# pcodec/pcodec

Measured on AMD Instinct MI355X. Metric: encode+decode GB/s (uncompressed) per chunk, u64/f64 2^18-elem, higher is better.
Workload: dtype u64

## Files before the change

### include/pco_gfx.h

```cpp
#ifndef PCO_GFX_H
#define PCO_GFX_H

#include <stddef.h>
#include <stdint.h>

#if defined(__cplusplus)
extern "C" {
#endif


#define PCO_TYPE_U32 1
#define PCO_TYPE_U64 2
#define PCO_TYPE_I32 3
#define PCO_TYPE_I64 4
#define PCO_TYPE_F32 5
#define PCO_TYPE_F64 6
#define PCO_TYPE_U16 7
#define PCO_TYPE_I16 8
#define PCO_TYPE_F16 9
#define PCO_TYPE_U8 10
#define PCO_TYPE_I8 11

typedef enum PcoError {
  PcoSuccess,
  PcoInvalidType,
  PcoCompressionError,
  PcoDecompressionError,
} PcoError;

typedef struct PcoChunkConfig {
  unsigned int compression_level;
  size_t max_page_n;
} PcoChunkConfig;

size_t pco_standalone_guarantee_file_size(size_t n, unsigned char dtype);

enum PcoError pco_standalone_simple_compress_into(const void* nums, size_t n, unsigned char dtype,
                                                  const struct PcoChunkConfig* config, void* dst,
                                                  size_t dst_cap, size_t* n_written);

enum PcoError pco_standalone_simple_decompress_into(const void* compressed, size_t compressed_len,
                                                    unsigned char dtype, void* dst, size_t dst_cap,
                                                    size_t* n_written);


enum PcoModeSpecKind {
  PCO_MODE_AUTO = 0,
  PCO_MODE_CLASSIC = 1,
  PCO_MODE_TRY_FLOAT_MULT = 2,
  PCO_MODE_TRY_FLOAT_QUANT = 3,
  PCO_MODE_TRY_INT_MULT = 4,
  PCO_MODE_TRY_DICT = 5,
};
enum PcoDeltaSpecKind {
  PCO_DELTA_AUTO = 0,
  PCO_DELTA_NOOP = 1,
  PCO_DELTA_TRY_CONSECUTIVE = 2,
  PCO_DELTA_TRY_LOOKBACK = 3,
  PCO_DELTA_TRY_CONV1 = 4,
};
typedef struct PcoChunkConfigEx {
  uint32_t compression_level;
  uint32_t mode_kind;
  double mode_f64;
  uint64_t mode_u64;
  uint32_t delta_kind;
  uint32_t delta_order;
  uint64_t max_page_n;
  uint32_t enable_8_bit;
  uint32_t flags;
} PcoChunkConfigEx;
#define PCO_GFX_CFG_STRICT_HISTOGRAM 1u
#define PCO_GFX_CFG_CONV1 2u
#define PCO_GFX_CFG_DICT 4u

enum PcoGfxStatus {
  PCO_GFX_OK = 0,
  PCO_GFX_CORRUPTION = 1,
  PCO_GFX_INSUFFICIENT_DATA = 2,
  PCO_GFX_INVALID_ARGUMENT = 3,
  PCO_GFX_UNSUPPORTED = 4,
  PCO_GFX_DEVICE_ERROR = 5,
};
int pco_gfx_last_status(void);
const char* pco_gfx_last_error(void);
int pco_gfx_device_count(void);

enum PcoError pco_gfx_simple_compress_into_ex(const void* nums, size_t n, unsigned char dtype,
                                              const PcoChunkConfigEx* config, int uniform_type,
                                              void* dst, size_t dst_cap, size_t* n_written);
enum PcoError pco_gfx_simple_compress_into_exact(const void* nums, size_t n, unsigned char dtype, const PcoChunkConfigEx* config,
                                                 int uniform_type, const size_t* page_sizes, size_t n_pages, void* dst,
                                                 size_t dst_cap, size_t* n_written);
size_t pco_gfx_guarantee_file_size(size_t n, unsigned char dtype, uint64_t max_page_n);
size_t pco_gfx_guarantee_chunk_size(size_t n, unsigned char dtype);


typedef struct PcoGfxEncodeTask {
  const void* src;
  uint64_t n;
  void* dst;
  uint64_t dst_cap;
  uint32_t dtype;
  uint32_t reserved;
} PcoGfxEncodeTask;

typedef struct PcoGfxDecodeTask {
  const void* src;
  uint64_t src_len;
  void* dst;
  uint64_t dst_cap;
  uint32_t dtype;
  uint32_t flags;
} PcoGfxDecodeTask;
#define PCO_GFX_TASK_HAS_FILE_HEADER 1u
#define PCO_GFX_TASK_WRAPPED_PAGE 2u
#define PCO_GFX_TASK_META_ONLY 4u
#define PCO_GFX_TASK_ONE_CHUNK 8u

typedef struct PcoGfxTaskResult {
  uint64_t n_out;
  uint64_t consumed;
  uint32_t status;
  uint32_t aux;
} PcoGfxTaskResult;

enum PcoError pco_gfx_compress_chunks(size_t n_tasks, const PcoGfxEncodeTask* tasks,
                                      const PcoChunkConfigEx* config, PcoGfxTaskResult* results,
                                      PcoGfxTaskResult* d_results, void* stream);
enum PcoError pco_gfx_decompress_chunks(size_t n_tasks, const PcoGfxDecodeTask* tasks,
                                        PcoGfxTaskResult* results, PcoGfxTaskResult* d_results,
                                        void* stream);

enum PcoError pco_gfx_compact_chunks(size_t n_tasks, const PcoGfxEncodeTask* tasks, const PcoGfxTaskResult* d_results, void* d_dst,
                                     uint64_t dst_cap, uint64_t dst_offset, uint64_t* d_offsets, uint64_t* total, void* stream);

size_t pco_gfx_write_standalone_header(void* dst, size_t dst_cap, uint64_t n_hint, unsigned char uniform_dtype);
size_t pco_gfx_write_standalone_footer(void* dst, size_t dst_cap);

void pco_gfx_release_workspace(void);
size_t pco_gfx_workspace_bytes(void);
unsigned long long pco_gfx_strict_histogram_fallbacks(void);
unsigned long long pco_gfx_trail_givebacks(void);
unsigned long long pco_gfx_trail_marked(void);

void pco_gfx_profile_begin(void);
int pco_gfx_profile_end(char* names, size_t names_cap, float* ms, int cap);

typedef struct PcoGfxChunkCompressor PcoGfxChunkCompressor;
typedef struct PcoGfxChunkDecompressor PcoGfxChunkDecompressor;

size_t pco_wrapped_write_header(void* dst, size_t dst_cap);
enum PcoError pco_wrapped_read_header(const void* src, size_t len, size_t* consumed,
                                      uint8_t* major, uint8_t* minor);
enum PcoError pco_chunk_compressor_new(const void* nums, size_t n, unsigned char dtype,
                                       const PcoChunkConfigEx* config,
                                       PcoGfxChunkCompressor** out);
enum PcoError pco_chunk_compressor_new_exact(const void* nums, size_t n, unsigned char dtype, const PcoChunkConfigEx* config,
                                             const size_t* page_sizes, size_t n_pages, PcoGfxChunkCompressor** out);
size_t pco_chunk_compressor_n_pages(const PcoGfxChunkCompressor*);
size_t pco_chunk_compressor_meta_size(const PcoGfxChunkCompressor*);
size_t pco_chunk_compressor_page_size(const PcoGfxChunkCompressor*, size_t page_idx);
size_t pco_chunk_compressor_page_n(const PcoGfxChunkCompressor*, size_t page_idx);
size_t pco_chunk_compressor_meta_size_hint(const PcoGfxChunkCompressor*);
size_t pco_chunk_compressor_page_size_hint(const PcoGfxChunkCompressor*, size_t page_idx);
enum PcoError pco_chunk_compressor_write_meta(const PcoGfxChunkCompressor*, void* dst, size_t dst_cap, size_t* n_written);
enum PcoError pco_chunk_compressor_write_page(const PcoGfxChunkCompressor*, size_t page_idx, void* dst, size_t dst_cap, size_t* n_written);
void pco_chunk_compressor_free(PcoGfxChunkCompressor*);

enum PcoError pco_chunk_decompressor_new(const void* src, size_t len, unsigned char dtype,
                                         uint8_t format_major, PcoGfxChunkDecompressor** out,
                                         size_t* consumed);
enum PcoError pco_chunk_decompressor_read_page(PcoGfxChunkDecompressor*, const void* src, size_t len,
                                               size_t page_n, void* dst, size_t dst_cap,
                                               size_t* n_processed, size_t* consumed);
void pco_chunk_decompressor_free(PcoGfxChunkDecompressor*);

typedef struct PcoGfxPageDecompressor PcoGfxPageDecompressor;
enum PcoError pco_page_decompressor_new(PcoGfxChunkDecompressor*, const void* src, size_t len, size_t page_n, PcoGfxPageDecompressor** out);
enum PcoError pco_page_decompressor_read(PcoGfxPageDecompressor*, void* dst, size_t dst_len, size_t* n_processed, int* finished);
size_t pco_page_decompressor_consumed(const PcoGfxPageDecompressor*);
void pco_page_decompressor_free(PcoGfxPageDecompressor*);

typedef struct PcoGfxPageInfo {
  uint64_t offset;
  uint64_t len;
  uint64_t n;
  uint32_t status;
  uint32_t aux;
} PcoGfxPageInfo;
size_t pco_gfx_wrapped_n_pages(size_t n, uint64_t max_page_n);
size_t pco_gfx_wrapped_chunk_cap(size_t n, unsigned char dtype, const PcoChunkConfigEx* config);
enum PcoError pco_gfx_compress_wrapped_chunks(size_t n_tasks, const PcoGfxEncodeTask* tasks, const PcoChunkConfigEx* config,
                                              PcoGfxPageInfo* infos, void* stream);

typedef struct PcoGfxWrappedTask {
  const void* src;
  uint64_t n;
  void* dst;
  uint64_t dst_cap;
  uint32_t dtype;
  uint32_t n_pages;
  const uint64_t* page_sizes;
} PcoGfxWrappedTask;
size_t pco_gfx_wrapped_chunk_cap_exact(const uint64_t* page_sizes, size_t n_pages, unsigned char dtype, const PcoChunkConfigEx* config);
enum PcoError pco_gfx_compress_wrapped_chunks_ex(size_t n_tasks, const PcoGfxWrappedTask* tasks, const PcoChunkConfigEx* config,
                                                 PcoGfxPageInfo* infos, PcoGfxPageInfo* d_infos, void* stream);
size_t pco_gfx_wrapped_scratch_estimate(size_t n_tasks, const PcoGfxWrappedTask* tasks, const PcoChunkConfigEx* config);
enum PcoError pco_gfx_compact_wrapped_chunks(size_t n_tasks, const PcoGfxWrappedTask* tasks, const PcoChunkConfigEx* config,
                                             const PcoGfxPageInfo* d_infos, uint32_t gap, void* d_dst, uint64_t dst_cap, uint64_t dst_offset,
                                             uint64_t* d_offsets, uint64_t* total, void* stream);

typedef struct PcoGfxPageTask {
  const void* meta;
  uint64_t meta_len;
  const void* page;
  uint64_t page_len;
  void* dst;
  uint64_t page_n;
  uint32_t dtype;
  uint32_t format_major;
} PcoGfxPageTask;
enum PcoError pco_gfx_decompress_pages(size_t n_tasks, const PcoGfxPageTask* tasks, PcoGfxTaskResult* results,
                                       PcoGfxTaskResult* d_results, void* stream);

typedef struct PcoGfxPageRangeTask {
  const void* meta;
  uint64_t meta_len;
  const void* page;
  uint64_t page_len;
  void* dst;
  uint64_t page_n;
  uint64_t first, count;
  uint32_t dtype;
  uint32_t format_major;
} PcoGfxPageRangeTask;
enum PcoError pco_gfx_decompress_page_ranges(size_t n_tasks, const PcoGfxPageRangeTask* tasks, PcoGfxTaskResult* results,
                                             PcoGfxTaskResult* d_results, void* stream);

typedef struct PcoGfxChunkMetaInfo {
  uint32_t mode_kind;
  uint32_t mode_k;
  uint64_t mode_base_latent;
  uint32_t delta_kind;
  uint32_t delta_order;
  uint32_t window_n_log, state_n_log;
  uint32_t secondary_uses_delta;
  uint32_t n_vars_parsed;
  uint32_t present[3], ans_size_log[3], n_bins[3];
  uint64_t meta_bytes;
} PcoGfxChunkMetaInfo;
enum PcoError pco_gfx_chunk_meta_info(const void* meta, size_t len, unsigned char dtype, uint8_t format_major, PcoGfxChunkMetaInfo* out);
enum PcoError pco_chunk_compressor_meta_info(const PcoGfxChunkCompressor*, unsigned char dtype, PcoGfxChunkMetaInfo* out);
enum PcoError pco_chunk_decompressor_meta_info(const PcoGfxChunkDecompressor*, PcoGfxChunkMetaInfo* out);
enum PcoError pco_gfx_chunk_meta_conv1(const void* meta, size_t len, unsigned char dtype, uint8_t format_major, uint32_t* quantization,
                                       int64_t* bias, int32_t* weights, uint32_t* order);
enum PcoError pco_gfx_chunk_meta_dict(const void* meta, size_t len, unsigned char dtype, uint8_t format_major, uint32_t* n_unique, void* values,
                                      size_t cap);

typedef struct PcoGfxComm PcoGfxComm;
enum PcoError pco_gfx_comm_unique_id(void* id128);
enum PcoError pco_gfx_comm_init(const void* id128, int n_ranks, int rank, PcoGfxComm** out);
void pco_gfx_comm_free(PcoGfxComm*);
int pco_gfx_comm_rank(const PcoGfxComm*);
int pco_gfx_comm_size(const PcoGfxComm*);
enum PcoError pco_gfx_gather_chunks(PcoGfxComm*, int root, const void* d_stream, uint64_t n_bytes, void* d_file, uint64_t file_cap,
                                    uint64_t file_offset, uint64_t* offsets, void* stream);
enum PcoError pco_gfx_scatter_chunks(PcoGfxComm*, int root, const void* d_file, uint64_t file_offset, const uint64_t* offsets,
                                     void* d_stream, uint64_t stream_cap, uint64_t* n_bytes, void* stream);

int pco_gfx_debug_float_screen(const void* values, size_t n, uint32_t dtype, uint32_t* out);
int64_t pco_gfx_debug_lookback_routes(uint8_t* out, size_t cap);

#if defined(__cplusplus)
}
#endif
#endif
```

### pcodec_amd/_lib.py

```python
import ctypes as C
import os

HERE = os.path.dirname(os.path.abspath(__file__))
LIB_PATH = os.environ.get("PCO_GFX_LIB", os.path.join(HERE, "libpco_gfx.so"))

PcoSuccess, PcoInvalidType, PcoCompressionError, PcoDecompressionError = range(4)
ST_OK, ST_CORRUPTION, ST_INSUFFICIENT_DATA, ST_INVALID_ARGUMENT, ST_UNSUPPORTED, ST_DEVICE_ERROR = range(6)
TASK_HAS_FILE_HEADER = 1

MODE_AUTO, MODE_CLASSIC, MODE_TRY_FLOAT_MULT, MODE_TRY_FLOAT_QUANT, MODE_TRY_INT_MULT, MODE_TRY_DICT = range(6)
DELTA_AUTO, DELTA_NOOP, DELTA_TRY_CONSECUTIVE, DELTA_TRY_LOOKBACK, DELTA_TRY_CONV1 = range(5)

CFG_STRICT_HISTOGRAM = 1
CFG_CONV1 = 2
CFG_DICT = 4

DTYPE_BYTE = {"uint32": 1, "uint64": 2, "int32": 3, "int64": 4, "float32": 5, "float64": 6,
              "uint16": 7, "int16": 8, "float16": 9, "uint8": 10, "int8": 11}
DTYPE_BYTES = {1: 4, 2: 8, 3: 4, 4: 8, 5: 4, 6: 8, 7: 2, 8: 2, 9: 2, 10: 1, 11: 1}


class PcoChunkConfig(C.Structure):
    _fields_ = [("compression_level", C.c_uint), ("max_page_n", C.c_size_t)]


class PcoChunkConfigEx(C.Structure):
    _fields_ = [("compression_level", C.c_uint32), ("mode_kind", C.c_uint32), ("mode_f64", C.c_double),
                ("mode_u64", C.c_uint64), ("delta_kind", C.c_uint32), ("delta_order", C.c_uint32),
                ("max_page_n", C.c_uint64), ("enable_8_bit", C.c_uint32), ("flags", C.c_uint32)]


class EncodeTask(C.Structure):
    _fields_ = [("src", C.c_void_p), ("n", C.c_uint64), ("dst", C.c_void_p), ("dst_cap", C.c_uint64),
                ("dtype", C.c_uint32), ("reserved", C.c_uint32)]


class DecodeTask(C.Structure):
    _fields_ = [("src", C.c_void_p), ("src_len", C.c_uint64), ("dst", C.c_void_p), ("dst_cap", C.c_uint64),
                ("dtype", C.c_uint32), ("flags", C.c_uint32)]


class TaskResult(C.Structure):
    _fields_ = [("n_out", C.c_uint64), ("consumed", C.c_uint64), ("status", C.c_uint32), ("aux", C.c_uint32)]


KIND_NAMES = {ST_CORRUPTION: "Corruption", ST_INSUFFICIENT_DATA: "InsufficientData", ST_INVALID_ARGUMENT: "InvalidArgument",
              ST_UNSUPPORTED: "Unsupported", ST_DEVICE_ERROR: "DeviceError"}


class PageInfo(C.Structure):
    _fields_ = [("offset", C.c_uint64), ("len", C.c_uint64), ("n", C.c_uint64), ("status", C.c_uint32), ("aux", C.c_uint32)]


class PageTask(C.Structure):
    _fields_ = [("meta", C.c_void_p), ("meta_len", C.c_uint64), ("page", C.c_void_p), ("page_len", C.c_uint64),
                ("dst", C.c_void_p), ("page_n", C.c_uint64), ("dtype", C.c_uint32), ("format_major", C.c_uint32)]


class PageRangeTask(C.Structure):
    _fields_ = [("meta", C.c_void_p), ("meta_len", C.c_uint64), ("page", C.c_void_p), ("page_len", C.c_uint64),
                ("dst", C.c_void_p), ("page_n", C.c_uint64), ("first", C.c_uint64), ("count", C.c_uint64),
                ("dtype", C.c_uint32), ("format_major", C.c_uint32)]


class WrappedTask(C.Structure):
    _fields_ = [("src", C.c_void_p), ("n", C.c_uint64), ("dst", C.c_void_p), ("dst_cap", C.c_uint64),
                ("dtype", C.c_uint32), ("n_pages", C.c_uint32), ("page_sizes", C.c_void_p)]


class PcoGfxError(RuntimeError):

    def __init__(self, code, status, msg):
        super().__init__(f"pco error: pco {KIND_NAMES.get(status, status)} error: {msg} (libpco_gfx code={code} status={status})")
        self.code, self.status = code, status


_lib = None


def lib():
    global _lib
    if _lib is None:
        if not os.path.exists(LIB_PATH):
            raise ImportError(f"{LIB_PATH} is missing: build it with `python -m pcodec_amd.build` (needs hipcc). "
                              "pcodec_amd has no CPU fallback.")
        try:
            import torch
        except Exception:
            pass
        L = C.CDLL(LIB_PATH)
        L.pco_gfx_last_error.restype = C.c_char_p
        L.pco_standalone_guarantee_file_size.restype = C.c_size_t
        L.pco_standalone_guarantee_file_size.argtypes = [C.c_size_t, C.c_ubyte]
        L.pco_gfx_guarantee_file_size.restype = C.c_size_t
        L.pco_gfx_guarantee_file_size.argtypes = [C.c_size_t, C.c_ubyte, C.c_uint64]
        L.pco_gfx_guarantee_chunk_size.restype = C.c_size_t
        L.pco_gfx_workspace_bytes.restype = C.c_size_t
        L.pco_gfx_workspace_bytes.argtypes = []
        L.pco_gfx_strict_histogram_fallbacks.restype = C.c_ulonglong
        L.pco_gfx_strict_histogram_fallbacks.argtypes = []
        L.pco_gfx_debug_lookback_routes.restype = C.c_int64
        L.pco_gfx_debug_lookback_routes.argtypes = [C.c_void_p, C.c_size_t]
        L.pco_gfx_trail_givebacks.restype = C.c_ulonglong
        L.pco_gfx_trail_givebacks.argtypes = []
        L.pco_gfx_trail_marked.restype = C.c_ulonglong
        L.pco_gfx_trail_marked.argtypes = []
        L.pco_gfx_guarantee_chunk_size.argtypes = [C.c_size_t, C.c_ubyte]
        L.pco_standalone_simple_compress_into.argtypes = [C.c_void_p, C.c_size_t, C.c_ubyte, C.c_void_p, C.c_void_p,
                                                          C.c_size_t, C.POINTER(C.c_size_t)]
        L.pco_standalone_simple_decompress_into.argtypes = [C.c_void_p, C.c_size_t, C.c_ubyte, C.c_void_p, C.c_size_t,
                                                            C.POINTER(C.c_size_t)]
        L.pco_gfx_simple_compress_into_ex.argtypes = [C.c_void_p, C.c_size_t, C.c_ubyte, C.c_void_p, C.c_int,
                                                      C.c_void_p, C.c_size_t, C.POINTER(C.c_size_t)]
        L.pco_gfx_compress_chunks.argtypes = [C.c_size_t, C.c_void_p, C.c_void_p, C.c_void_p, C.c_void_p, C.c_void_p]
        L.pco_gfx_decompress_chunks.argtypes = [C.c_size_t, C.c_void_p, C.c_void_p, C.c_void_p, C.c_void_p]
        L.pco_gfx_write_standalone_header.restype = C.c_size_t
        L.pco_gfx_write_standalone_header.argtypes = [C.c_void_p, C.c_size_t, C.c_uint64, C.c_ubyte]
        L.pco_gfx_write_standalone_footer.restype = C.c_size_t
        L.pco_gfx_write_standalone_footer.argtypes = [C.c_void_p, C.c_size_t]
        L.pco_wrapped_write_header.restype = C.c_size_t
        L.pco_wrapped_write_header.argtypes = [C.c_void_p, C.c_size_t]
        L.pco_gfx_wrapped_n_pages.restype = C.c_size_t
        L.pco_gfx_wrapped_n_pages.argtypes = [C.c_size_t, C.c_uint64]
        L.pco_gfx_wrapped_chunk_cap.restype = C.c_size_t
        L.pco_gfx_wrapped_chunk_cap.argtypes = [C.c_size_t, C.c_ubyte, C.c_void_p]
        L.pco_gfx_compress_wrapped_chunks.argtypes = [C.c_size_t, C.c_void_p, C.c_void_p, C.c_void_p, C.c_void_p]
        L.pco_gfx_decompress_pages.argtypes = [C.c_size_t, C.c_void_p, C.c_void_p, C.c_void_p, C.c_void_p]
        L.pco_gfx_decompress_page_ranges.argtypes = [C.c_size_t, C.c_void_p, C.c_void_p, C.c_void_p, C.c_void_p]
        L.pco_gfx_wrapped_chunk_cap_exact.restype = C.c_size_t
        L.pco_gfx_wrapped_chunk_cap_exact.argtypes = [C.c_void_p, C.c_size_t, C.c_ubyte, C.c_void_p]
        L.pco_gfx_compress_wrapped_chunks_ex.argtypes = [C.c_size_t, C.c_void_p, C.c_void_p, C.c_void_p, C.c_void_p, C.c_void_p]
        L.pco_gfx_wrapped_scratch_estimate.restype = C.c_size_t
        L.pco_gfx_wrapped_scratch_estimate.argtypes = [C.c_size_t, C.c_void_p, C.c_void_p]
        L.pco_gfx_compact_wrapped_chunks.argtypes = [C.c_size_t, C.c_void_p, C.c_void_p, C.c_void_p, C.c_uint32, C.c_void_p, C.c_uint64, C.c_uint64,
                                                     C.c_void_p, C.c_void_p, C.c_void_p]
        _lib = L
    return _lib


def check(code):
    if code != PcoSuccess:
        L = lib()
        raise PcoGfxError(code, L.pco_gfx_last_status(), (L.pco_gfx_last_error() or b"").decode())


def make_config(level=8, mode=MODE_AUTO, mode_f64=0.0, mode_u64=0, delta=DELTA_AUTO, delta_order=0, max_page_n=0,
                enable_8_bit=False, strict_histogram=False, conv1=False, dict=False):
    return PcoChunkConfigEx(level, mode, mode_f64, mode_u64, delta, delta_order, max_page_n, 1 if enable_8_bit else 0,
                            (CFG_STRICT_HISTOGRAM if strict_histogram else 0) | (CFG_CONV1 if conv1 else 0) | (CFG_DICT if dict else 0))


def chunk_meta_conv1(meta, dtype_byte, format_major=4):
    buf = (C.c_uint8 * max(len(meta), 1)).from_buffer_copy(bytes(meta) or b"\0")
    q, b, order, w = C.c_uint32(), C.c_int64(), C.c_uint32(), (C.c_int32 * 32)()
    rc = lib().pco_gfx_chunk_meta_conv1(buf, C.c_size_t(len(meta)), C.c_ubyte(dtype_byte), C.c_uint8(format_major), C.byref(q), C.byref(b), w,
                                        C.byref(order))
    if rc != 0:
        raise PcoGfxError(rc, lib().pco_gfx_last_status(), lib().pco_gfx_last_error().decode())
    return None if order.value == 0 else (q.value, b.value, list(w[:order.value]))


def chunk_meta_dict(meta, dtype_byte, format_major=4):
    import numpy as np
    buf = (C.c_uint8 * max(len(meta), 1)).from_buffer_copy(bytes(meta) or b"\0")
    width = {1: 4, 2: 8, 3: 4, 4: 8, 5: 4, 6: 8, 7: 2, 8: 2, 9: 2, 10: 1, 11: 1}[dtype_byte]
    cap = max(len(meta) // width, 1)
    out = np.zeros(cap, dtype={1: np.uint8, 2: np.uint16, 4: np.uint32, 8: np.uint64}[width])
    k = C.c_uint32()
    rc = lib().pco_gfx_chunk_meta_dict(buf, C.c_size_t(len(meta)), C.c_ubyte(dtype_byte), C.c_uint8(format_major), C.byref(k),
                                       out.ctypes.data_as(C.c_void_p), C.c_size_t(cap))
    if rc != 0:
        raise PcoGfxError(rc, lib().pco_gfx_last_status(), lib().pco_gfx_last_error().decode())
    return None if k.value == 0 else out[:k.value].copy()
```

### pcodec_amd/csrc/decode_fast.hip

```cpp
#include "decode_kernel.hip"

namespace pcogfx {

constexpr uint32_t kGrpWinOff = 0;
constexpr uint32_t kGrpVarOff = 448;
constexpr uint32_t kGrpTblOff = 640;
template <uint32_t KQ> struct WalkCfg {
  static constexpr uint32_t kGrpBytes = KQ == 8 ? 4912u : 9904u;
  static constexpr uint32_t kGrpTblBytes = kGrpBytes - kGrpTblOff;
  static constexpr uint32_t kWalkTmpOff = KQ * kGrpBytes;
  static constexpr uint32_t kWalkTmpObOff = kWalkTmpOff + 1056;
  static constexpr uint32_t kWalkLdsBytes = kWalkTmpObOff + 256;
  static constexpr uint32_t kRetryStatus = KQ == 8 ? 101u : 100u;
  static_assert(kGrpBytes % 16 == 0, "chunk slices must stay 16-byte aligned");
  static_assert(kWalkLdsBytes < 65536, "walk entries hold 16-bit LDS addresses");
};
template <uint32_t KQ> __device__ __forceinline__ uint8_t PCO_LDS* walk_lds() { return lds_base() + uni((uint32_t)(threadIdx.x >> 6)) * WalkCfg<KQ>::kWalkLdsBytes; }
__device__ __forceinline__ uint32_t walk_block_id() { return blockIdx.x * (blockDim.x >> 6) + uni((uint32_t)(threadIdx.x >> 6)); }
constexpr uint32_t kTrailDead = 0xffffffffu;
constexpr uint32_t kTrailDoneWord = 8;
constexpr uint32_t kTrailProgressStride = 32;
constexpr bool kTrailDefer = true;
constexpr uint32_t kTrailMaxBins = 64;
constexpr uint32_t kFastMaxBins = 256;
// ... 63 lines not shown
  if (n_bins == 0) { if (lane == 0) entries[0] = make_wentry(0, 0, 0, 0); wave_sync_lds(); return true; }
  if (carry != T) { status = PCO_GFX_CORRUPTION; return false; }
  wave_sync_lds();
  uint32_t stride = (3 * T) / 5; if ((stride & 1) == 0) stride += 1;
  for (uint32_t t = lane; t < T; t += 64) {
    uint32_t lo = 0, hi = n_bins;
    while (hi - lo > 1) { const uint32_t mid = (lo + hi) >> 1; if (cum[mid] <= t) lo = mid; else hi = mid; }
    entries[(stride * t) & (T - 1)] = lo;
  }
  wave_sync_lds();
  for (uint32_t b0 = 0; b0 < n_bins; b0 += 64) {
    const uint32_t b = b0 + lane;
    uint32_t w = 0;
    if (b < n_bins) w = cum[b + 1] - cum[b];
    wave_sync_lds();
    if (b < n_bins) cum[b] = w;
    wave_sync_lds();
  }
  const uint32_t sym_bits = 32 - clz_u32(n_bins - 1 > 0 ? n_bins - 1 : 1);
  for (uint32_t i0 = 0; i0 < T; i0 += 64) {
    const uint32_t i = i0 + lane;
    const bool act = i < T;
    const uint32_t s = act ? entries[i] : 0xffffffffu;
    uint64_t m = __ballot(act);
    for (uint32_t bit = 0; bit < sym_bits; bit++) { const uint64_t bm = __ballot((s >> bit) & 1); m &= ((s >> bit) & 1) ? bm : ~bm; }
    const uint64_t lt = ((uint64_t)1 << lane) - 1;
    const uint32_t rank = __popcll(m & lt), gcount = __popcll(m);
    const uint32_t basec = act ? cum[s] : 0;
    wave_sync_lds();
    if (act && rank == 0) cum[s] = basec + gcount;
    wave_sync_lds();
    if (act) { const uint32_t x_s = basec + rank; const uint32_t btr = clz_u32(x_s) - clz_u32(T); entries[i] = make_wentry((x_s << btr) - T, s, btr, obs[s]); }
  }
  wave_sync_lds();
  return true;
}

template <class LV, uint32_t KQ>
__device__ __noinline__ bool fast_build_var(uint32_t q, uint32_t vi, MetaReader& mr, uint8_t PCO_GLOBAL* bins_out, uint32_t& status) { return fast_build_var_impl<LV, KQ>(q, vi, mr, bins_out, status); }

struct FrontOut {
  uint32_t status, n, mode_kind;
  uint64_t bitpos;
  uint32_t states[3][4];
  uint64_t moments[2][2];
};

template <class L, uint32_t KQ, bool kInline, bool kRange = false>
__device__ __forceinline__ void fast_front_impl(const PcoGfxDecodeTask& task, uint32_t q, DecPlan PCO_GLOBAL* plan, uint8_t PCO_GLOBAL* bins_out, FrontOut& out,
                                                gcptr_u8 meta_p, uint64_t meta_len) {
  constexpr uint32_t kGrpBytes = WalkCfg<KQ>::kGrpBytes, kGrpTblBytes = WalkCfg<KQ>::kGrpTblBytes;
  const uint32_t lane = lane_id();
  gcptr_u8 src = (gcptr_u8)task.src;
  const uint64_t src_len = uni((uint64_t)task.src_len);
  const uint32_t dtype = uni(task.dtype), flags = uni(task.flags);
  const uint64_t dst_cap = uni((uint64_t)task.dst_cap);
  constexpr uint32_t LB = LBits<L>::v;
  const bool wrapped = (flags & PCO_GFX_TASK_WRAPPED_PAGE) != 0;
  MetaReader mr{src, src_len, 0};
  if (wrapped && meta_p != nullptr) mr = MetaReader{meta_p, meta_len, 0};
  uint32_t status = PCO_GFX_OK, format_major = 4, uniform_type = 0;
  out.status = PCO_GFX_OK; out.n = 0; out.bitpos = 0;
  for (int v = 0; v < 3; v++) for (int j = 0; j < 4; j++) out.states[v][j] = 0;
  out.mode_kind = kClassic;
  VarInfo PCO_LDS* vinfo = (VarInfo PCO_LDS*)(walk_lds<KQ>() + q * kGrpBytes + kGrpVarOff);
  auto fail = [&](uint32_t s) { if (wrapped && s != kStatusRetryK4) s = kStatusRetryLegacy; out.status = s; if (lane == 0) { plan->status = s; plan->consumed = mr.bit >> 3; plan->n = 0; plan->fused = 0; plan->more = 0; } };
  out.moments[0][0] = out.moments[0][1] = out.moments[1][0] = out.moments[1][1] = 0;
  if (dtype_bits(dtype) != (int)LB) { fail(PCO_GFX_INVALID_ARGUMENT); return; }
  if (flags & PCO_GFX_TASK_META_ONLY) { fail(kStatusRetryLegacy); return; }
  uint32_t n = 0;
  if (wrapped) {
    format_major = (flags >> 8) & 0xffu;
    if (dst_cap == 0 || dst_cap > kMaxEntries || format_major > 4) { fail(kStatusRetryLegacy); return; }
    n = (uint32_t)dst_cap;
  } else
  if (flags & PCO_GFX_TASK_HAS_FILE_HEADER) {
    const uint32_t magic = (uint32_t)mr.read(32);
    if (!mr.in_bounds()) status = PCO_GFX_INSUFFICIENT_DATA; else if (magic != 0x216f6370u) status = PCO_GFX_CORRUPTION;
    if (!status) {
      const uint32_t sv = (uint32_t)mr.read(8);
      if (sv < 2) mr.bit -= 8;
      else {
        if (sv >= 3) { const uint32_t ub = (uint32_t)mr.read(8); if (ub != 0) { if (dtype_bits(ub) == 0) status = PCO_GFX_CORRUPTION; uniform_type = ub; } }
        if (!status) { const uint32_t power = 1 + (uint32_t)mr.read(kBitsVarintPower); mr.read(power); if (!mr.drain_empty_byte() && mr.in_bounds()) status = PCO_GFX_CORRUPTION; }
      }
      if (!status && !mr.in_bounds()) status = PCO_GFX_INSUFFICIENT_DATA;
      if (!status && sv > 3) status = PCO_GFX_CORRUPTION;
      if (!status) {
        format_major = (uint32_t)mr.read(8);
        if (format_major >= 4) mr.read(8);
        if (format_major > 4) status = PCO_GFX_CORRUPTION; else if (!mr.in_bounds()) status = PCO_GFX_INSUFFICIENT_DATA;
      }
    }
    if (status) { fail(status); return; }
  } else if (src_len == 0) { fail(kStatusRetryLegacy); return; }
  else if ((flags & PCO_GFX_TASK_ONE_CHUNK) && ((flags >> 8) & 0xffu) != 0) format_major = (flags >> 8) & 0xffu;
  if (!wrapped) {
    const uint32_t tb = (uint32_t)mr.read(8);
    if (!mr.in_bounds()) { fail(PCO_GFX_INSUFFICIENT_DATA); return; }
    if (tb == 0) { fail(kStatusRetryLegacy); return; }
    if ((uniform_type && uniform_type != tb) || tb != dtype) { fail(PCO_GFX_CORRUPTION); return; }
    n = (uint32_t)mr.read(kBitsNEntries) + 1;
    if (!mr.in_bounds()) { fail(PCO_GFX_INSUFFICIENT_DATA); return; }
    if (n > dst_cap) { fail(PCO_GFX_INVALID_ARGUMENT); return; }
  }
  const uint32_t num_kind = dtype_kind(dtype);
  const uint32_t mode_kind = (uint32_t)mr.read(kBitsModeVariant);
  L mode_base = 0; uint32_t mode_k = 0;
  if (mode_kind == kIntMult) { if (format_major == 0) { fail(PCO_GFX_CORRUPTION); return; } mode_base = (L)mr.read(LB); }
  else if (mode_kind == kFloatMult) mode_base = (L)mr.read(LB);
  else if (mode_kind == kFloatQuant) mode_k = (uint32_t)mr.read(kBitsQuantK);
  else if (mode_kind == kDict) { fail(mr.in_bounds() ? kStatusRetryLegacy : PCO_GFX_INSUFFICIENT_DATA); return; }
  else if (mode_kind != kClassic) { fail(mr.in_bounds() ? PCO_GFX_CORRUPTION : PCO_GFX_INSUFFICIENT_DATA); return; }
  if (!mr.in_bounds()) { fail(PCO_GFX_INSUFFICIENT_DATA); return; }
  uint32_t dkind = kDeltaNone, dorder = 0, wlog = 0, slog = 0; bool sec_uses_delta = false;
  if (format_major < 3) { dorder = (uint32_t)mr.read(kBitsDeltaOrder); if (dorder) dkind = kDeltaConsecutive; }
  else {
    const uint32_t variant = (uint32_t)mr.read(kBitsDeltaVariant);
    if (variant == 1) { dorder = (uint32_t)mr.read(kBitsDeltaOrder); if (dorder == 0) { fail(PCO_GFX_CORRUPTION); return; } dkind = kDeltaConsecutive; sec_uses_delta = mr.read(1) != 0; }
    else if (variant == 2) {
      wlog = 1 + (uint32_t)mr.read(kBitsLookbackWindowLog); slog = (uint32_t)mr.read(kBitsLookbackStateLog);
      if (wlog > kMaxLookbackWindowLog || slog > wlog) { fail(PCO_GFX_CORRUPTION); return; }
      dkind = kDeltaLookback; sec_uses_delta = mr.read(1) != 0;
    } else if (variant == 3) { fail(mr.in_bounds() ? kStatusRetryLegacy : PCO_GFX_INSUFFICIENT_DATA); return; }
    else if (variant != 0) { fail(PCO_GFX_CORRUPTION); return; }
  }
  if (!mr.in_bounds()) { fail(PCO_GFX_INSUFFICIENT_DATA); return; }
  const uint32_t present[3] = {dkind == kDeltaLookback ? 1u : 0u, 1u, (mode_kind == kIntMult || mode_kind == kFloatMult || mode_kind == kFloatQuant) ? 1u : 0u};
  uint32_t total_tbl = 0; bool too_big = false;
  {
    MetaReader peek = mr;
#pragma unroll
    for (int vi = 0; vi < 3; vi++) {
      VarInfo v{};
      v.present = present[vi]; v.latent_bits = vi == 0 ? 32u : LB;
      if (vi == 1 || (vi == 2 && sec_uses_delta)) { v.delta_kind = dkind; v.delta_order = dorder; v.window_n_log = wlog; v.state_n_log = slog; }
      if (present[vi]) {
        const uint32_t a = (uint32_t)peek.read(kBitsAnsSizeLog), nb = (uint32_t)peek.read(kBitsNBins);
        if (!peek.in_bounds()) { fail(PCO_GFX_INSUFFICIENT_DATA); return; }
        if ((1u << a) < nb || (nb == 1 && a > 0) || a > kMaxAnsBits) { fail(PCO_GFX_CORRUPTION); return; }
        v.ans_size_log = a; v.n_bins = nb;
        v.off_nodes = total_tbl; v.off_lower = 0; v.off_ob = total_tbl + (4u << a);
        total_tbl += (4u << a) + 8u;
        if (nb > kFastMaxBins || a > 12) too_big = true;
        peek.bit += (uint64_t)nb * (a + v.latent_bits + offset_bits_bits(v.latent_bits));
      }
      if (lane == 0) { uint32_t PCO_LDS* p = (uint32_t PCO_LDS*)(vinfo + vi); const uint32_t* qq = (const uint32_t*)&v; for (int w = 0; w < 16; w++) p[w] = qq[w]; }
    }
  }
  wave_sync_lds();
  if (too_big || total_tbl > WalkCfg<4>::kGrpTblBytes) { fail(kStatusRetryLegacy); return; }
  if (total_tbl > kGrpTblBytes) { fail(WalkCfg<KQ>::kRetryStatus); return; }
  if (dkind == kDeltaLookback && (mode_kind != kClassic || sec_uses_delta)) { fail(kStatusRetryLegacy); return; }
  if constexpr (kRange) { if (dkind == kDeltaLookback) { fail(kStatusRetryLegacy); return; } }
#pragma unroll
  for (int vi = 0; vi < 3; vi++) {
    if (!present[vi]) continue;
    mr.bit += kBitsAnsSizeLog + kBitsNBins;
    bool ok;
    if constexpr (kInline) ok = vi == 0 ? fast_build_var_impl<uint32_t, KQ>(q, vi, mr, bins_out, status) : fast_build_var_impl<L, KQ>(q, vi, mr, bins_out, status);
    else ok = vi == 0 ? fast_build_var<uint32_t, KQ>(q, vi, mr, bins_out, status) : fast_build_var<L, KQ>(q, vi, mr, bins_out, status);
    if (!ok) { fail(status); return; }
  }
  if (!mr.drain_empty_byte()) { if (mr.in_bounds()) { fail(PCO_GFX_CORRUPTION); return; } }
  if (!mr.in_bounds()) { fail(PCO_GFX_INSUFFICIENT_DATA); return; }
  if (wrapped && meta_p != nullptr) mr = MetaReader{src, src_len, 0};
  if (dkind == kDeltaLookback) {
    const uint32_t nb0 = uni(vinfo[0].n_bins);
    const uint64_t PCO_GLOBAL* lw = (const uint64_t PCO_GLOBAL*)bins_out;
    uint32_t bad = 0;
    __builtin_amdgcn_fence(__ATOMIC_ACQ_REL, "workgroup");
    for (uint32_t b = lane; b < nb0; b += 64) { const uint64_t x = __hip_atomic_load(&lw[b], __ATOMIC_RELAXED, __HIP_MEMORY_SCOPE_AGENT); if (x < 1 || x > (1ull << wlog)) bad = 1; }
    if (uni(wave_or_u32(bad))) { fail(PCO_GFX_CORRUPTION); return; }
  }
  {
    bool valid = true;
    if (mode_kind == kIntMult) valid = num_kind != kFloat && mode_base > 0;
    else if (mode_kind == kFloatQuant) { const uint32_t prec = LB == 64 ? 52 : (LB == 32 ? 23 : 10); valid = num_kind == kFloat && mode_k > 0 && mode_k <= prec; }
    else if (mode_kind == kFloatMult) {
      if (num_kind != kFloat) valid = false;
      else if constexpr (sizeof(L) >= 4) { typedef typename FloatOf<L>::F F; const F b = bits_to_float(from_latent_ordered<L>(mode_base, kFloat)); valid = isfinite(b) && b != (F)0; }
      else if constexpr (sizeof(L) == 2) { const uint32_t hb = (uint32_t)from_latent_ordered<L>(mode_base, kFloat); valid = (hb & 0x7c00u) != 0x7c00u && (hb & 0x7fffu) != 0; }
      else valid = false;
    }
    if (!valid) { fail(PCO_GFX_CORRUPTION); return; }
  }
  uint32_t nlps[3];
#pragma unroll
  for (int vi = 0; vi < 3; vi++) {
    const uint32_t dk = uni(vinfo[vi].delta_kind);
    nlps[vi] = dk == kDeltaConsecutive ? uni(vinfo[vi].delta_order) : (dk == kDeltaLookback ? (1u << uni(vinfo[vi].state_n_log)) : 0u);
  }
  L PCO_GLOBAL* dst = (L PCO_GLOBAL*)task.dst;
#pragma unroll
  for (int vi = 0; vi < 3; vi++) {
    if (!present[vi]) continue;
    const uint32_t lbits = vi == 0 ? 32u : LB;
    const uint32_t dk = uni(vinfo[vi].delta_kind);
    for (uint32_t i = 0; i < nlps[vi]; i++) {
      const L x = (L)mr.read(lbits);
      if (dk == kDeltaConsecutive) { if (lane == 0 && i < 8) plan->moments[vi == 2 ? 1 : 0][i] = (uint64_t)x; if (i < 2) out.moments[vi == 2 ? 1 : 0][i] = (uint64_t)x; }
      else if (vi == 1 && i < n && mr.in_bounds()) { if (lane == 0) dst[i] = from_latent_ordered<L>(x, num_kind); }
    }
    const uint32_t asl = uni(vinfo[vi].ans_size_log);
    for (uint32_t j = 0; j < 4; j++) out.states[vi][j] = (uint32_t)mr.read(asl);
  }
  if (!mr.drain_empty_byte()) { if (mr.in_bounds()) { fail(PCO_GFX_CORRUPTION); return; } }
  if (!mr.in_bounds()) { fail(PCO_GFX_INSUFFICIENT_DATA); return; }
  const uint32_t n_in_body = n > nlps[1] ? n - nlps[1] : 0;
  if (n_in_body > 0) for (int vi = 0; vi < 3; vi++) if (present[vi] && uni(vinfo[vi].n_bins) == 0) { fail(PCO_GFX_CORRUPTION); return; }
  out.mode_kind = mode_kind;
  if (lane == 0) {
    plan->status = PCO_GFX_OK; plan->n = n; plan->mode_kind = mode_kind; plan->mode_k = mode_k; plan->mode_base = (uint64_t)mode_base;
    plan->num_kind = num_kind; plan->dtype = dtype; plan->window_n_log = wlog; plan->state_n_log = slog; plan->consumed = 0; plan->fused = 0; plan->more = 0;
    for (int vi = 0; vi < 3; vi++) {
      plan->present[vi] = present[vi]; plan->n_bins[vi] = vinfo[vi].n_bins; plan->max_ob[vi] = vinfo[vi].max_ob;
      plan->delta_kind[vi] = vinfo[vi].delta_kind; plan->delta_order[vi] = vinfo[vi].delta_order; plan->nlps[vi] = nlps[vi];
    }
  }
  out.n = n; out.bitpos = mr.bit;
}

template <class L, uint32_t KQ>
__device__ __noinline__ void fast_front(const PcoGfxDecodeTask& task, uint32_t q, DecPlan PCO_GLOBAL* plan, uint8_t PCO_GLOBAL* bins_out, FrontOut& out, gcptr_u8 meta_p, uint64_t meta_len) { fast_front_impl<L, KQ, false>(task, q, plan, bins_out, out, meta_p, meta_len); }
template <class L, uint32_t KQ>
__device__ __noinline__ void fast_front_range(const PcoGfxDecodeTask& task, uint32_t q, DecPlan PCO_GLOBAL* plan, uint8_t PCO_GLOBAL* bins_out, FrontOut& out, gcptr_u8 meta_p, uint64_t meta_len) { fast_front_impl<L, KQ, false, true>(task, q, plan, bins_out, out, meta_p, meta_len); }

struct WalkRegs {
  uint32_t saddr;
  uint32_t e;
  uint32_t bitaddr;
  uint32_t d0, d1, d2;
  uint32_t obsum, symacc;
};

__device__ __forceinline__ void walk_window(WalkRegs& r, uint32_t tot) {
  r.bitaddr += tot;
  const uint32_t PCO_LDS* w = (const uint32_t PCO_LDS*)(uintptr_t)((r.bitaddr >> 3) & ~3u);
  r.d0 = w[0]; r.d1 = w[1]; r.d2 = w[2];
}

template <bool kAgent>
__device__ __forceinline__ void store_syms(uint8_t PCO_GLOBAL* p, uint32_t __attribute__((ext_vector_type(4))) acc) {
  typedef uint32_t u32x4 __attribute__((ext_vector_type(4)));
  if constexpr (kAgent) {
    __asm__ volatile("global_store_dwordx4 %0, %1, off sc1" : : "v"(p), "v"(acc) : "memory");
  } else *(u32x4 PCO_GLOBAL*)p = acc;
}

struct QuadMasks { uint32_t m1, m2, m3, c63; };

template <int K, bool kTail>
__device__ __forceinline__ void walk_step(WalkRegs& r, const QuadMasks& m, uint32_t tbl_addr, bool chain_on) {
  uint32_t e = r.e;
  if (kTail) e = chain_on ? e : 0u;
  const uint32_t p = ((uint32_t)__builtin_amdgcn_update_dpp(0, (int)e, 0x111, 0xf, 0xf, true) & m.m1) +
                     ((uint32_t)__builtin_amdgcn_update_dpp(0, (int)e, 0x112, 0xf, 0xf, true) & m.m2) +
                     ((uint32_t)__builtin_amdgcn_update_dpp(0, (int)e, 0x113, 0xf, 0xf, true) & m.m3);
  const uint32_t x0 = __builtin_amdgcn_alignbit(r.d1, r.d0, r.bitaddr), x1 = __builtin_amdgcn_alignbit(r.d2, r.d1, r.bitaddr);
  const uint64_t xs = (((uint64_t)x1 << 32) | x0) >> (p & 63u);
  const uint32_t v = __builtin_amdgcn_ubfe((uint32_t)xs, 0u, e);
  const uint32_t next = tbl_addr + (((e >> 21) + v) << 2);
  if (kTail) r.saddr = chain_on ? next : r.saddr; else r.saddr = next;
  r.e = *(const uint32_t PCO_LDS*)(uintptr_t)r.saddr;
  __builtin_amdgcn_sched_barrier(0);
  const uint32_t t = p + e;
  walk_window(r, (uint32_t)__builtin_amdgcn_update_dpp(0, (int)t, 0xFF, 0xf, 0xf, true) & m.c63);
  if (K == 0) r.symacc = __builtin_amdgcn_ubfe(e, 13u, 8u); else r.symacc |= __builtin_amdgcn_ubfe(e, 13u, 8u) << (8 * K);
  r.obsum += __builtin_amdgcn_ubfe(e, 6u, 7u);
  __builtin_amdgcn_sched_barrier(0);
}

__device__ __forceinline__ uint32_t block_trail_kinds(const PcoGfxDecodeTask* tasks, const uint32_t* task_ids, uint32_t n_ids, uint32_t wb, const MetaRef* metas) {
  const uint32_t lane = lane_id(), bi = wb * 8 + (lane & 7u);
  bool one = false, two = false;
  if (lane < 8 && bi < n_ids) {
    const uint32_t ti = task_ids ? task_ids[bi] : bi;
    const PcoGfxDecodeTask t = tasks[ti];
    const bool wrapped = (t.flags & PCO_GFX_TASK_WRAPPED_PAGE) != 0;
    const uint32_t fmt = wrapped ? (t.flags >> 8) & 0xffu : ((t.flags & PCO_GFX_TASK_ONE_CHUNK) && ((t.flags >> 8) & 0xffu) ? (t.flags >> 8) & 0xffu : 4u);
    gcptr_u8 mp = (gcptr_u8)t.src + 4; uint64_t mlen = t.src_len >= 4 ? t.src_len - 4 : 0;
    if (wrapped) { if (metas != nullptr && metas[ti].p != nullptr) { mp = (gcptr_u8)metas[ti].p; mlen = metas[ti].len; } else { mp = (gcptr_u8)t.src; mlen = t.src_len; } }
    if ((t.flags & (PCO_GFX_TASK_META_ONLY | PCO_GFX_TASK_HAS_FILE_HEADER)) == 0 && mlen >= 20 && fmt >= 3 && fmt <= 4) {
      const uint64_t w = load_u64_le(mp);
      const uint32_t mode = (uint32_t)w & 15u;
      if (mode == kClassic) {
        const uint32_t dv = (uint32_t)(w >> 4) & 15u;
        const uint32_t n_bins = (uint32_t)(w >> (dv == kDeltaConsecutive ? 16 : 12)) & 0x7fffu;
        one = (dv == kDeltaNone || dv == kDeltaConsecutive) && n_bins > 1 && n_bins <= kTrailMaxBins;
      } else if (mode == kIntMult || mode == kFloatMult || mode == kFloatQuant) {
        const uint32_t at = 4u + (mode == kFloatQuant ? kBitsQuantK : (uint32_t)dtype_bits(t.dtype));
        const uint64_t w2 = load_u64_le(mp + (at >> 3));
        const uint32_t dv = (uint32_t)(w2 >> (at & 7u)) & 15u;
        two = dv == kDeltaNone || dv == kDeltaConsecutive;
      }
    }
  }
  return (uni((uint32_t)__any(one)) ? 1u : 0u) | (uni((uint32_t)__any(two)) ? 2u : 0u);
}
__device__ __forceinline__ bool block_has_trail_candidate(const PcoGfxDecodeTask* tasks, const uint32_t* task_ids, uint32_t n_ids, uint32_t wb, const MetaRef* metas) {
  return block_trail_kinds(tasks, task_ids, n_ids, wb, metas) != 0;
}

template <class L, uint32_t kWQ, bool kTrail, bool kRange = false>
__device__ __forceinline__ void dec_walk_body(const PcoGfxDecodeTask* tasks, const uint32_t* task_ids, uint32_t n_ids, DecPlan* plans,
                                              uint8_t* bins_area, uint8_t* sym_area, uint64_t sym_stride, uint64_t* offpos_area, uint64_t offpos_stride,
                                              uint32_t accept_status, PcoGfxTaskResult* results, uint32_t* progress, const MetaRef* metas,
                                              const RangeRef* ranges = nullptr) {
  static_assert(!kTrail || !kRange, "range tasks never take the publishing walker");
  static_assert(!kTrail || kWQ == 8, "the trailing expanders follow the eight-chunk walker");
  const uint32_t wb = walk_block_id();
  if ((uint64_t)wb * kWQ >= n_ids) return;
  constexpr uint32_t kGrpBytes = WalkCfg<kWQ>::kGrpBytes;
  if constexpr (kTrail) __builtin_amdgcn_s_setprio(3);
  const uint32_t lane = lane_id();
  const uint32_t slot = lane >> 2, j = lane & 3;
  if constexpr (kTrail) {
    if (!block_has_trail_candidate(tasks, task_ids, n_ids, wb, metas)) {
      if (lane < 8) __hip_atomic_store(progress + (uint64_t)wb * kTrailProgressStride + lane, kTrailDead, __ATOMIC_RELAXED, __HIP_MEMORY_SCOPE_AGENT);
      return;
    }
  } else if constexpr (kWQ == 8) {
    if (progress != nullptr && accept_status == 0 && block_has_trail_candidate(tasks, task_ids, n_ids, wb, metas)) return;
  }
  uint32_t my_ti = 0xffffffffu, my_active = 0, my_front_ok = 0, my_n = 0, my_flags = 0, my_mode = kClassic;
  uint32_t my_bend = 0xffffffffu;
  uint32_t st0 = 0, st1 = 0, st2 = 0;
  uint64_t my_bitpos = 0, my_len = 0;
  uint64_t my_mom[2][2] = {{0, 0}, {0, 0}};
  gcptr_u8 my_src = nullptr;
  for (uint32_t q = 0; q < kWQ; q++) {
    const uint32_t bi = wb * kWQ + q;
    if (bi >= n_ids) break;
    const uint32_t ti = task_ids ? task_ids[bi] : bi;
    if (accept_status != 0 && uni(((const DecPlan PCO_GLOBAL*)plans + ti)->status) != accept_status) continue;
    if constexpr (kRange) {
      if (uni(ranges[ti].count) == 0) { if (lane == 0) { DecPlan PCO_GLOBAL* pl = (DecPlan PCO_GLOBAL*)plans + ti; pl->status = kStatusEmptyRange; pl->consumed = 0; pl->n = 0; pl->fused = 0; pl->more = 0; } continue; }
    }
    const PcoGfxDecodeTask task = tasks[ti];
    FrontOut fo;
    gcptr_u8 meta_p = metas != nullptr ? (gcptr_u8)metas[ti].p : (gcptr_u8) nullptr;
    const uint64_t meta_len = metas != nullptr ? uni((uint64_t)metas[ti].len) : 0;
    if constexpr (kRange) fast_front_range<L, kWQ>(task, q, (DecPlan PCO_GLOBAL*)plans + ti, (uint8_t PCO_GLOBAL*)bins_area + (uint64_t)ti * kBinsAreaPerTask, fo, meta_p, meta_len);
    else if constexpr (kTrail) fast_front_impl<L, kWQ, true>(task, q, (DecPlan PCO_GLOBAL*)plans + ti, (uint8_t PCO_GLOBAL*)bins_area + (uint64_t)ti * kBinsAreaPerTask, fo, meta_p, meta_len);
    else fast_front<L, kWQ>(task, q, (DecPlan PCO_GLOBAL*)plans + ti, (uint8_t PCO_GLOBAL*)bins_area + (uint64_t)ti * kBinsAreaPerTask, fo, meta_p, meta_len);
    if (slot == q) {
      my_ti = ti; my_active = fo.status == PCO_GFX_OK ? 1u : 0u; my_front_ok = my_active; my_n = fo.n; my_bitpos = fo.bitpos; my_mode = fo.mode_kind;
      my_len = task.src_len; my_flags = task.flags; my_src = (gcptr_u8)task.src;
      if constexpr (kRange) my_bend = (uint32_t)range_end_batch(ranges[ti].first, ranges[ti].count);
      my_mom[0][0] = fo.moments[0][0]; my_mom[0][1] = fo.moments[0][1]; my_mom[1][0] = fo.moments[1][0]; my_mom[1][1] = fo.moments[1][1];
      st0 = j == 0 ? fo.states[0][0] : (j == 1 ? fo.states[0][1] : (j == 2 ? fo.states[0][2] : fo.states[0][3]));
      st1 = j == 0 ? fo.states[1][0] : (j == 1 ? fo.states[1][1] : (j == 2 ? fo.states[1][2] : fo.states[1][3]));
      st2 = j == 0 ? fo.states[2][0] : (j == 1 ? fo.states[2][1] : (j == 2 ? fo.states[2][2] : fo.states[2][3]));
    }
    wave_sync_lds();
  }
  const uint32_t slice = (slot < kWQ ? slot : 0u) * kGrpBytes;
  uint8_t PCO_LDS* gbase = walk_lds<kWQ>() + slice;
  const uint32_t lds0 = (uint32_t)(uintptr_t)walk_lds<kWQ>();
  uint64_t PCO_LDS* win = (uint64_t PCO_LDS*)(gbase + kGrpWinOff);
  VarInfo PCO_LDS* vinfo = (VarInfo PCO_LDS*)(gbase + kGrpVarOff);
  uint32_t n_rem = my_n, batch = 0, cur_v = 0, status = PCO_GFX_OK, present_mask = 0, nlps1 = 0;
  if (my_active) {
    present_mask = (vinfo[0].present ? 1u : 0u) | 2u | (vinfo[2].present ? 4u : 0u);
    nlps1 = vinfo[1].delta_kind == kDeltaConsecutive ? vinfo[1].delta_order : (vinfo[1].delta_kind == kDeltaLookback ? (1u << vinfo[1].state_n_log) : 0u);
    cur_v = (present_mask & 1u) ? 0u : 1u;
    if (n_rem == 0) my_active = 0;
    st0 = lds0 + slice + kGrpTblOff + vinfo[0].off_nodes + 4u * st0;
    st1 = lds0 + slice + kGrpTblOff + vinfo[1].off_nodes + 4u * st1;
    st2 = lds0 + slice + kGrpTblOff + vinfo[2].off_nodes + 4u * st2;
  }
  bool my_fused = false;
  uint32_t my_fused_kind = 0;
  uint32_t PCO_GLOBAL* my_progress = nullptr;
  if constexpr (kTrail) {
    if (my_active && slot < kWQ) {
      const bool prim_ok = vinfo[0].present == 0 && vinfo[1].n_bins >= 1 && vinfo[1].n_bins <= kTrailMaxBins && vinfo[1].max_ob <= 16 &&
                           (vinfo[1].delta_kind == kDeltaConsecutive ? vinfo[1].delta_order <= 2 : vinfo[1].delta_kind == kDeltaNone);
      if (vinfo[2].present == 0) { if (prim_ok && my_mode == kClassic && vinfo[1].n_bins > 1) my_fused_kind = 1; }
      else if (prim_ok && (my_mode == kIntMult || my_mode == kFloatMult || my_mode == kFloatQuant) && vinfo[2].n_bins >= 1 && vinfo[2].n_bins <= kTrailMaxBins &&
               vinfo[2].max_ob <= 16 && vinfo[2].delta_kind == kDeltaNone && (vinfo[1].n_bins > 1 || vinfo[2].n_bins > 1)) my_fused_kind = 2;
      my_fused = my_fused_kind != 0;
    }
    if (slot < kWQ) my_progress = (uint32_t PCO_GLOBAL*)progress + (uint64_t)wb * kTrailProgressStride + slot;
    if (j == 0 && my_fused) ((DecPlan PCO_GLOBAL*)plans + my_ti)->fused = my_fused_kind;
    __builtin_amdgcn_fence(__ATOMIC_RELEASE, "agent");
    if (j == 0 && slot < kWQ) __hip_atomic_store((uint32_t*)my_progress, my_fused ? 1u : kTrailDead, __ATOMIC_RELAXED, __HIP_MEMORY_SCOPE_AGENT);
  }

  typedef uint32_t u32x4 __attribute__((ext_vector_type(4)));
  QuadMasks qm = {j >= 1 ? ~0u : 0u, j >= 2 ? ~0u : 0u, j >= 3 ? ~0u : 0u, 63u};
  asm volatile("" : "+v"(qm.m1), "+v"(qm.m2), "+v"(qm.m3), "+v"(qm.c63));
  u32x4 d_acc[4] = {{0u, 0u, 0u, 0u}, {0u, 0u, 0u, 0u}, {0u, 0u, 0u, 0u}, {0u, 0u, 0u, 0u}};
  uint32_t d_ngrp = 0, issued_batches = 0; uint8_t PCO_GLOBAL* d_sym_out = nullptr;
  uint64_t d_off_val = 0; uint64_t* d_off_ptr = nullptr;
  auto flush_deferred = [&]() {
#pragma unroll
    for (int g = 0; g < 4; g++) if ((uint32_t)g < d_ngrp) store_syms<true>(d_sym_out + 64 * g, d_acc[g]);
    d_ngrp = 0;
    if (d_off_ptr) __hip_atomic_store(d_off_ptr, d_off_val, __ATOMIC_RELAXED, __HIP_MEMORY_SCOPE_AGENT);
    d_off_ptr = nullptr;
  };
  uint64_t touch_prev = my_bitpos >> 3; uint32_t touch_r0 = 0, touch_r1 = 0;
  while (__any(my_active != 0)) {
    uint32_t cnt = 0, nb = 0, asl = 0, off_ob = 0, off_nodes = 0;
    bool walk = false;
    if (my_active) {
      const VarInfo PCO_LDS* vi = vinfo + cur_v;
      nb = vi->n_bins; asl = vi->ans_size_log; off_ob = vi->off_ob; off_nodes = vi->off_nodes;
      const uint32_t batch_n = n_rem < kBatchN ? n_rem : kBatchN;
      if (cur_v == 0) { const uint32_t lim = n_rem > nlps1 ? n_rem - nlps1 : 0; cnt = lim < batch_n ? lim : batch_n; }
      else {
        const uint32_t nl = cur_v == 1 ? nlps1 : (vi->delta_kind == kDeltaConsecutive ? vi->delta_order : (vi->delta_kind == kDeltaLookback ? (1u << vi->state_n_log) : 0u));
        const uint32_t rem = n_rem > nl ? n_rem - nl : 0; cnt = rem < kBatchN ? rem : kBatchN;
      }
      walk = cnt > 0 && nb > 1;
    }
    const uint64_t q0 = my_bitpos >> 6;
    WalkRegs r;
    r.saddr = cur_v == 0 ? st0 : (cur_v == 1 ? st1 : st2);
    const uint32_t win_addr = lds0 + slice + kGrpWinOff, rel0 = (uint32_t)(my_bitpos & 63);
    r.bitaddr = 8u * win_addr + rel0; r.obsum = 0; r.symacc = 0; r.e = 0; r.d0 = r.d1 = r.d2 = 0;
    if (walk) {
      const uint32_t nq = ((((rel0 + cnt * asl + 63u) >> 6) + 3u) + 1u) & ~1u;
      uint64_t lo[7], hi[7];
      if ((q0 + nq) * 8 <= my_len + 16) {
#pragma unroll
        for (int k = 0; k < 7; k++) {
          const uint32_t qi = 2 * j + 8 * k, qc = qi < nq ? qi : nq - 2;
          lo[k] = load_u64_le(my_src + (q0 + qc) * 8); hi[k] = load_u64_le(my_src + (q0 + qc) * 8 + 8);
        }
      } else {
#pragma unroll
        for (int k = 0; k < 7; k++) {
          const uint32_t qi = 2 * j + 8 * k;
          lo[k] = 0; hi[k] = 0;
          if (qi < nq) { lo[k] = load_u64_le_safe(my_src, (q0 + qi) * 8, my_len + 16); hi[k] = load_u64_le_safe(my_src, (q0 + qi + 1) * 8, my_len + 16); }
        }
      }
#pragma unroll
      for (int k = 0; k < 7; k++) { const uint32_t qi = 2 * j + 8 * k; if (qi < nq) { win[qi] = lo[k]; win[qi + 1] = hi[k]; } }
    }
    wave_sync_lds();
    if constexpr (kTrail) {
      __asm__ volatile("s_waitcnt vmcnt(0)" ::: "memory");
      if (my_fused && j == 0 && status == PCO_GFX_OK) __hip_atomic_store((uint32_t*)my_progress, 1u + issued_batches, __ATOMIC_RELAXED, __HIP_MEMORY_SCOPE_AGENT);
      if constexpr (kTrailDefer) { flush_deferred(); issued_batches = batch; }
      else issued_batches = batch;
    }
    ((uint32_t PCO_LDS*)(walk_lds<kWQ>() + WalkCfg<kWQ>::kWalkTmpOff))[lane] = touch_r0 ^ touch_r1;
    if (walk) {
      const uint64_t cur = q0 * 8, pred = cur + (cur - touch_prev);
      touch_prev = cur;
      const uint64_t line0 = (pred & ~(uint64_t)127) - (pred >= 128 ? 128u : 0u);
      const uint64_t a0 = line0 + 128u * j, a1 = a0 + 512u;
      touch_r0 = load_u32_le(my_src + (a0 + 4 <= my_len ? a0 : 0));
      touch_r1 = load_u32_le(my_src + (a1 + 4 <= my_len ? a1 : 0));
    }
    const uint32_t obs_addr = lds0 + slice + kGrpTblOff + off_ob, tbl_addr = lds0 + slice + kGrpTblOff + off_nodes;
    uint8_t PCO_GLOBAL* sym_out = (uint8_t PCO_GLOBAL*)sym_area + ((uint64_t)(my_ti == 0xffffffffu ? 0u : my_ti) * 3 + cur_v) * sym_stride + (uint64_t)batch * kBatchN + 16 * j;
    if (walk) {
      r.e = *(const uint32_t PCO_LDS*)(uintptr_t)r.saddr;
      walk_window(r, 0u);
      constexpr bool defer = kTrail && kTrailDefer;
      if constexpr (defer) d_sym_out = sym_out;
      if (__all(!walk || cnt == kBatchN)) {
#pragma unroll
        for (uint32_t grp = 0; grp < 4; grp++) {
          u32x4 acc;
#pragma unroll
          for (int b = 0; b < 4; b++) {
            walk_step<0, false>(r, qm, tbl_addr, true);
            walk_step<1, false>(r, qm, tbl_addr, true);
            walk_step<2, false>(r, qm, tbl_addr, true);
            walk_step<3, false>(r, qm, tbl_addr, true);
            acc[b] = r.symacc;
          }
          if constexpr (defer) d_acc[grp] = acc; else store_syms<kTrail>(sym_out + 64 * grp, acc);
        }
        if constexpr (defer) d_ngrp = 4;
      } else {
        const uint32_t steps = (cnt + 3) >> 2;
        if constexpr (defer) d_ngrp = (steps + 15) >> 4;
#pragma unroll
        for (uint32_t grp = 0; grp < 4; grp++) {
          if (grp * 16 >= steps) break;
          u32x4 acc = {0u, 0u, 0u, 0u};
#pragma unroll
          for (int b = 0; b < 4; b++) {
            const uint32_t g = grp * 16 + b * 4;
            if (g < steps) {
              r.symacc = 0;
              if (g + 0 < steps) walk_step<0, true>(r, qm, tbl_addr, 4 * (g + 0) + j < cnt);
              if (g + 1 < steps) walk_step<1, true>(r, qm, tbl_addr, 4 * (g + 1) + j < cnt);
              if (g + 2 < steps) walk_step<2, true>(r, qm, tbl_addr, 4 * (g + 2) + j < cnt);
              if (g + 3 < steps) walk_step<3, true>(r, qm, tbl_addr, 4 * (g + 3) + j < cnt);
              acc[b] = r.symacc;
            }
          }
          if constexpr (defer) d_acc[grp] = acc; else store_syms<kTrail>(sym_out + 64 * grp, acc);
        }
      }
      if (cur_v == 0) st0 = r.saddr; else if (cur_v == 1) st1 = r.saddr; else st2 = r.saddr;
    }
    if (my_active) {
      uint32_t obq = r.obsum;
      obq += (uint32_t)__builtin_amdgcn_update_dpp(0, (int)obq, 0xB1, 0xf, 0xf, false);
      obq += (uint32_t)__builtin_amdgcn_update_dpp(0, (int)obq, 0x4E, 0xf, 0xf, false);
      const uint64_t ans_end = walk ? (q0 << 6) + (r.bitaddr - 8u * win_addr) : my_bitpos;
      uint64_t ob_total = 0;
      if (cnt > 0) ob_total = walk ? (uint64_t)obq : (nb == 1 ? (uint64_t)cnt * *(const uint8_t PCO_LDS*)(uintptr_t)obs_addr : 0ull);
      if (cnt > 0 && j == 0) {
        uint64_t* op = offpos_area + ((uint64_t)my_ti * 3 + cur_v) * offpos_stride + batch;
        if constexpr (kTrail && kTrailDefer) { d_off_ptr = op; d_off_val = ans_end; }
        else if constexpr (kTrail) __hip_atomic_store(op, ans_end, __ATOMIC_RELAXED, __HIP_MEMORY_SCOPE_AGENT);
        else *op = ans_end;
      }
      my_bitpos = ans_end + ob_total;
      if (my_bitpos > my_len * 8) { status = PCO_GFX_INSUFFICIENT_DATA; my_active = 0; }
      uint32_t nv = cur_v + 1;
      while (nv < 3 && !((present_mask >> nv) & 1u)) nv++;
      if (nv >= 3) {
        const uint32_t batch_n = n_rem < kBatchN ? n_rem : kBatchN;
        n_rem -= batch_n; batch++;
        nv = (present_mask & 1u) ? 0u : 1u;
        if (n_rem == 0) my_active = 0;
        if constexpr (kRange) { if (batch >= my_bend) my_active = 0; }
      }
      cur_v = nv;
    }
    wave_sync_lds();
  }
  if constexpr (kTrail) {
    flush_deferred();
    __asm__ volatile("s_waitcnt vmcnt(0)" ::: "memory");
    if (my_fused && j == 0) __hip_atomic_store((uint32_t*)my_progress, status == PCO_GFX_OK ? 1u + batch : kTrailDead, __ATOMIC_RELAXED, __HIP_MEMORY_SCOPE_AGENT);
  }
  if (my_ti != 0xffffffffu && j == 0 && slot < kWQ) {
    DecPlan PCO_GLOBAL* plan = (DecPlan PCO_GLOBAL*)plans + my_ti;
    if (my_front_ok) {
      uint64_t bit = my_bitpos;
      bool open_end = false;
      if constexpr (kRange) open_end = status == PCO_GFX_OK && n_rem != 0;
      if (status == PCO_GFX_OK && !open_end) {
        const uint32_t sh = (uint32_t)(bit & 7);
        if (sh) { const uint64_t byte = bit >> 3; const uint32_t b = byte < my_len ? my_src[byte] : 0u; if ((b >> sh) != 0) status = PCO_GFX_CORRUPTION; bit += 8 - sh; }
        if (bit > my_len * 8) status = PCO_GFX_INSUFFICIENT_DATA;
      }
      if ((my_flags & PCO_GFX_TASK_WRAPPED_PAGE) && status != PCO_GFX_OK) status = kStatusRetryLegacy;
      if (status == PCO_GFX_OK) {
        uint64_t byte = bit >> 3;
        if (my_flags & PCO_GFX_TASK_WRAPPED_PAGE) { }
        else if (my_flags & PCO_GFX_TASK_ONE_CHUNK) {
          if (byte < my_len && my_src[byte] != 0) plan->more = 1u;
          else if (byte < my_len) { byte += 1; plan->more = 2u; }
          else if (my_flags & PCO_GFX_TASK_HAS_FILE_HEADER) status = PCO_GFX_INSUFFICIENT_DATA;
        } else if (my_flags & PCO_GFX_TASK_HAS_FILE_HEADER) {
          if (byte >= my_len) status = PCO_GFX_INSUFFICIENT_DATA;
          else if (my_src[byte] != 0) status = kStatusRetryLegacy;
          else byte += 1;
        } else if (byte < my_len) status = kStatusRetryLegacy;
        plan->consumed = open_end ? 0 : byte;
      }
      plan->status = status;
      if constexpr (kTrail) {
        if (my_fused && status != kStatusRetryLegacy) {
          PcoGfxTaskResult r; r.n_out = status == PCO_GFX_OK ? my_n : 0; r.consumed = plan->consumed; r.status = status; r.aux = plan->more;
          results[my_ti] = r;
        }
      }
    }
  }
}

template <class L, uint32_t kWQ>
__global__ __launch_bounds__(256) void dec_walk_kernel(const PcoGfxDecodeTask* tasks, const uint32_t* task_ids, uint32_t n_ids, DecPlan* plans,
                                                      uint8_t* bins_area, uint8_t* sym_area, uint64_t sym_stride, uint64_t* offpos_area, uint64_t offpos_stride,
                                                      uint32_t accept_status, PcoGfxTaskResult* results, uint32_t* split, const MetaRef* metas) {
  dec_walk_body<L, kWQ, false>(tasks, task_ids, n_ids, plans, bins_area, sym_area, sym_stride, offpos_area, offpos_stride, accept_status, results, split, metas);
}
#define PCO_TRAIL_WALK_ATTR __attribute__((amdgpu_waves_per_eu(4, 4)))
template <class L>
__global__ __launch_bounds__(256) PCO_TRAIL_WALK_ATTR void dec_walk_trail_kernel(const PcoGfxDecodeTask* tasks, const uint32_t* task_ids, uint32_t n_ids, DecPlan* plans,
                                                      uint8_t* bins_area, uint8_t* sym_area, uint64_t sym_stride, uint64_t* offpos_area, uint64_t offpos_stride,
                                                      PcoGfxTaskResult* results, uint32_t* progress, const MetaRef* metas) {
  dec_walk_body<L, 8, true>(tasks, task_ids, n_ids, plans, bins_area, sym_area, sym_stride, offpos_area, offpos_stride, 0u, results, progress, metas);
}

__device__ __forceinline__ void store_u64_batch(unsigned long long PCO_GLOBAL* batch_base, const unsigned long long (&x)[4]) {
  typedef uint32_t u32x4 __attribute__((ext_vector_type(4)));
  const uint32_t lane = lane_id();
  const uint32_t from = 4u * (((lane & 1u) << 5) + (lane >> 1));
  const uint32_t a[4] = {(uint32_t)x[0], (uint32_t)(x[0] >> 32), (uint32_t)x[1], (uint32_t)(x[1] >> 32)};
  const uint32_t b[4] = {(uint32_t)x[2], (uint32_t)(x[2] >> 32), (uint32_t)x[3], (uint32_t)(x[3] >> 32)};
  u32x4 s1, s2;
#pragma unroll
  for (int j = 0; j < 4; j++) {
    const auto r = __builtin_amdgcn_permlane32_swap(a[j], b[j], false, false);
    s1[j] = (uint32_t)__builtin_amdgcn_ds_bpermute((int)from, (int)r[0]); s2[j] = (uint32_t)__builtin_amdgcn_ds_bpermute((int)from, (int)r[1]);
  }
  u32x4 PCO_GLOBAL* o = (u32x4 PCO_GLOBAL*)batch_base + lane;
  __builtin_nontemporal_store(s1, o); __builtin_nontemporal_store(s2, o + 64);
}

constexpr uint32_t kExpWaves = 4;
constexpr uint32_t kExpLowOff = 0;
constexpr uint32_t kExpObOff = 3 * 2048;
constexpr uint32_t kExpMomOff = kExpObOff + 768;
constexpr uint32_t kExpTurnOff = kExpMomOff + 128;
constexpr uint32_t kExpWaveOff = kExpTurnOff + 16;
constexpr uint32_t kExpWaveBytes = 4096;
constexpr uint32_t kExpLdsBytes = kExpWaveOff + kExpWaves * kExpWaveBytes;
constexpr uint32_t kExpRing = 8;
constexpr uint32_t kExpRingOff = kExpLdsBytes;
constexpr uint32_t kExpLbLdsBytes = kExpRingOff + kExpRing * 256 * 8;

struct ExpPre { uint32_t syms; uint32_t sec[8]; };
constexpr uint32_t kExpStgDwords = 528;

__device__ __forceinline__ void expand_prefetch(ExpPre& pre, gcptr_u8 src, uint64_t src_len, uint64_t start_bit, uint32_t need_bits,
                                                const uint8_t PCO_GLOBAL* syms, uint32_t cnt, bool single_bin) {
  const uint32_t lane = lane_id();
  typedef uint32_t u32x4 __attribute__((ext_vector_type(4)));
  typedef u32x4 __attribute__((aligned(1))) u32x4_unaligned;
  pre.syms = (!single_bin && 64 * (lane >> 4) < cnt) ? *(const uint32_t PCO_GLOBAL*)(syms + 4 * lane) : 0u;
  const uint64_t byte0 = (start_bit >> 5) * 4;
  const uint32_t need_bytes = need_bits == 0 ? 0u : (((uint32_t)(start_bit & 31) + need_bits + 31u) / 32u) * 4u + 8u;
  const uint32_t off = 32 * lane;
#pragma unroll
  for (int k = 0; k < 8; k++) pre.sec[k] = 0;
  if (off < need_bytes) {
    if (byte0 + off + 32 <= src_len + 16) {
      const u32x4 a = *(const u32x4_unaligned PCO_GLOBAL*)(src + byte0 + off), b = *(const u32x4_unaligned PCO_GLOBAL*)(src + byte0 + off + 16);
      pre.sec[0] = a.x; pre.sec[1] = a.y; pre.sec[2] = a.z; pre.sec[3] = a.w; pre.sec[4] = b.x; pre.sec[5] = b.y; pre.sec[6] = b.z; pre.sec[7] = b.w;
    } else {
#pragma unroll
      for (int k = 0; k < 4; k++) { const uint64_t w = load_u64_le_safe(src, byte0 + off + 8 * k, src_len + 16); pre.sec[2 * k] = (uint32_t)w; pre.sec[2 * k + 1] = (uint32_t)(w >> 32); }
    }
  }
}

template <class LV>
__device__ __forceinline__ void expand_item(const ExpPre& pre, uint32_t PCO_LDS* stg, gcptr_u8 src, uint64_t src_len, uint64_t start_bit, uint32_t need_bits, uint32_t cnt,
                                            const uint64_t PCO_LDS* lowers, const uint8_t PCO_LDS* obs, bool single_bin, uint32_t max_ob, LV out[4]) {
  const uint32_t lane = lane_id();
  typedef uint32_t u32x4 __attribute__((ext_vector_type(4)));
  if (need_bits != 0) {
    const uint32_t need_bytes = (((uint32_t)(start_bit & 31) + need_bits + 31u) / 32u) * 4u + 8u;
    if (32 * lane < need_bytes) {
      u32x4 a, b; a.x = pre.sec[0]; a.y = pre.sec[1]; a.z = pre.sec[2]; a.w = pre.sec[3]; b.x = pre.sec[4]; b.y = pre.sec[5]; b.z = pre.sec[6]; b.w = pre.sec[7];
      *(u32x4 PCO_LDS*)(stg + 8 * lane) = a; *(u32x4 PCO_LDS*)(stg + 8 * lane + 4) = b;
    }
    if (need_bytes > 2048 && lane < 2) {
      const uint64_t w = load_u64_le_safe(src, (start_bit >> 5) * 4 + 2048 + 8 * lane, src_len + 16);
      stg[512 + 2 * lane] = (uint32_t)w; stg[513 + 2 * lane] = (uint32_t)(w >> 32);
    }
  }
  wave_sync_lds();
  const uint32_t mine = (uint32_t)__builtin_amdgcn_ds_bpermute((int)(4u * ((lane & 48u) + 4u * (lane & 3u) + ((lane >> 2) & 3u))), (int)pre.syms);
  const uint32_t syms = single_bin ? 0u : quad_transpose_u8(mine, lane & 3);
  uint32_t ob[4]; LV low[4]; uint32_t t = 0;
#pragma unroll
  for (int k = 0; k < 4; k++) {
    const bool act = 4 * lane + k < cnt;
    const uint32_t s = (syms >> (8 * k)) & 0xffu;
    ob[k] = act ? (uint32_t)obs[s] : 0u;
    low[k] = act ? (LV)lowers[s] : (LV)0;
    t += ob[k];
  }
  const uint32_t incl = wave_incl_scan(t);
  uint32_t r = (uint32_t)(start_bit & 31) + incl - t;
  if (need_bits != 0 && max_ob <= 16) {
    const uint32_t d = r >> 5;
    const uint32_t w0 = stg[d], w1 = stg[d + 1], w2 = stg[d + 2];
    uint64_t v64 = (uint64_t)__builtin_amdgcn_alignbit(w1, w0, r) | ((uint64_t)__builtin_amdgcn_alignbit(w2, w1, r) << 32);
#pragma unroll
    for (int k = 0; k < 4; k++) {
      out[k] = (LV)(low[k] + (LV)__builtin_amdgcn_ubfe((uint32_t)v64, 0u, ob[k]));
      v64 >>= ob[k];
    }
    wave_sync_lds();
    return;
  }
#pragma unroll
  for (int k = 0; k < 4; k++) {
    LV val = 0;
    if (need_bits != 0) {
      const uint32_t d = r >> 5;
      const uint32_t w0 = stg[d], w1 = stg[d + 1];
      if constexpr (sizeof(LV) == 8) {
        const uint32_t w2 = stg[d + 2];
        const uint64_t v64 = (uint64_t)__builtin_amdgcn_alignbit(w1, w0, r) | ((uint64_t)__builtin_amdgcn_alignbit(w2, w1, r) << 32);
        val = ob[k] >= 64 ? v64 : (v64 & (((uint64_t)1 << ob[k]) - 1));
      } else {
        val = (LV)__builtin_amdgcn_ubfe(__builtin_amdgcn_alignbit(w1, w0, r), 0u, ob[k]);
        if (ob[k] >= 32) val = (LV)__builtin_amdgcn_alignbit(w1, w0, r);
      }
    }
    out[k] = (LV)(low[k] + val);
    r += ob[k];
  }
  wave_sync_lds();
}

template <class L, bool kLb, bool kRange>
__device__ __forceinline__ void dec_expand_body(const PcoGfxDecodeTask* tasks, PcoGfxTaskResult* results, const uint32_t* task_ids, uint32_t n_ids,
                                                const DecPlan* plans, const uint8_t* bins_area, const uint8_t* sym_area, uint64_t sym_stride,
                                                const uint64_t* offpos_area, uint64_t offpos_stride,
                                                const uint32_t* progress , uint32_t* givebacks,
                                                const RangeRef* ranges) {
  static_assert(!(kLb && kRange), "lookback ranges are decoded into scratch");
  const uint32_t lane = lane_id(), tid = threadIdx.x, wave = tid >> 6;
  uint8_t PCO_LDS* smem = lds_base();
  for (uint32_t bi = blockIdx.x; bi < n_ids; bi += gridDim.x) {
    const uint32_t ti = task_ids ? task_ids[bi] : bi;
    const DecPlan PCO_GLOBAL* plan = (const DecPlan PCO_GLOBAL*)plans + ti;
    const uint32_t pstatus = uni(plan->status);
    if constexpr (kRange) {
      if (pstatus == kStatusRetryLegacy || pstatus == kStatusEmptyRange) {
        if (tid == 0) { PcoGfxTaskResult r; r.n_out = 0; r.consumed = 0; r.status = pstatus == kStatusEmptyRange ? (uint32_t)PCO_GFX_OK : pstatus; r.aux = 0; results[ti] = r; }
        continue;
      }
    }
    if (pstatus == kStatusRetryLegacy) continue;
    if (uni(plan->fused)) {
      const bool done = progress != nullptr && uni(progress[(uint64_t)(bi >> 3) * kTrailProgressStride + kTrailDoneWord + (bi & 7u)]) != 0;
      if (!kLb && tid == 0 && givebacks != nullptr) atomicAdd(givebacks + 1, 1u);
      if (done) continue;
      if (!kLb && tid == 0 && givebacks != nullptr && pstatus == PCO_GFX_OK) atomicAdd(givebacks, 1u);
    }
    if ((uni(plan->delta_kind[1]) == kDeltaLookback) != kLb) continue;
    if (pstatus != PCO_GFX_OK) {
      if (tid == 0) { PcoGfxTaskResult r; r.n_out = 0; r.consumed = plan->consumed; r.status = pstatus; r.aux = 0; results[ti] = r; }
      continue;
    }
    const PcoGfxDecodeTask task = tasks[ti];
    gcptr_u8 src = (gcptr_u8)task.src;
    const uint64_t src_len = uni((uint64_t)task.src_len);
    L PCO_GLOBAL* dst = (L PCO_GLOBAL*)task.dst;
    const uint32_t n = uni(plan->n), mode_kind = uni(plan->mode_kind), mode_k = uni(plan->mode_k), num_kind = uni(plan->num_kind);
    const L mode_base = (L)uni((uint64_t)plan->mode_base);
    uint32_t present[3], n_bins[3], max_ob[3], dk[3], dord[3], nlps[3];
#pragma unroll
    for (int v = 0; v < 3; v++) {
      present[v] = uni(plan->present[v]); n_bins[v] = uni(plan->n_bins[v]); max_ob[v] = uni(plan->max_ob[v]);
      dk[v] = uni(plan->delta_kind[v]); dord[v] = uni(plan->delta_order[v]); nlps[v] = uni(plan->nlps[v]);
    }
    const uint32_t window_n_log = uni(plan->window_n_log);
    const uint32_t state_n = dk[1] == kDeltaLookback ? nlps[1] : 0u;
    uint64_t PCO_LDS* lowers = (uint64_t PCO_LDS*)(smem + kExpLowOff);
    uint8_t PCO_LDS* obs = smem + kExpObOff;
    uint64_t PCO_LDS* mom64 = (uint64_t PCO_LDS*)(smem + kExpMomOff);
    uint32_t PCO_LDS* turn = (uint32_t PCO_LDS*)(smem + kExpTurnOff);
    uint8_t PCO_LDS* wsm = smem + kExpWaveOff + wave * kExpWaveBytes;
    uint32_t PCO_LDS* dlat = (uint32_t PCO_LDS*)wsm;
    L PCO_LDS* scratch = (L PCO_LDS*)(wsm + 1024);
    uint32_t PCO_LDS* parent = (uint32_t PCO_LDS*)(wsm + 3072);
    uint32_t PCO_LDS* stg = (uint32_t PCO_LDS*)(wsm + 1024);
    L PCO_LDS* moments0 = (L PCO_LDS*)mom64; L PCO_LDS* moments1 = (L PCO_LDS*)(mom64 + 8);
    L PCO_LDS* hring = (L PCO_LDS*)(smem + kExpRingOff);
    __syncthreads();
    const uint8_t PCO_GLOBAL* bins = (const uint8_t PCO_GLOBAL*)bins_area + (uint64_t)ti * kBinsAreaPerTask;
#pragma unroll
    for (int v = 0; v < 3; v++) {
      if (!present[v]) continue;
      const uint64_t PCO_GLOBAL* gl = (const uint64_t PCO_GLOBAL*)(bins + (uint64_t)v * kBinsAreaPerVar);
      const uint8_t PCO_GLOBAL* go = bins + (uint64_t)v * kBinsAreaPerVar + kFastMaxBins * 8;
      for (uint32_t b = tid; b < n_bins[v]; b += 256) { lowers[v * 256 + b] = gl[b]; obs[v * 256 + b] = go[b]; }
    }
    if (tid < 8) { moments0[tid] = (L)plan->moments[0][tid]; moments1[tid] = (L)plan->moments[1][tid]; }
    if (tid == 0) { turn[0] = 0; turn[1] = 0; }
    __syncthreads();
    const bool ordered = dk[1] != kDeltaNone || (present[2] && dk[2] == kDeltaConsecutive);
    uint32_t n_batches = (n + kBatchN - 1) / kBatchN;
    uint64_t r_first = 0, r_end = 0;
    uint32_t b_begin = 0;
    if constexpr (kRange) {
      r_first = uni(ranges[ti].first); r_end = r_first + uni(ranges[ti].count);
      const uint32_t b_end = (uint32_t)range_end_batch(r_first, r_end - r_first);
      n_batches = b_end < n_batches ? b_end : n_batches;
      b_begin = ordered ? 0u : (uint32_t)(r_first >> 8);
    }
    uint32_t lb_oob = 0;
    auto cnt_of = [&](uint32_t batch, int v) -> uint32_t {
      const uint32_t n_remaining = n - batch * kBatchN;
      const uint32_t batch_n = n_remaining < kBatchN ? n_remaining : kBatchN;
      if (v == 0) { const uint32_t lim = n_remaining > nlps[1] ? n_remaining - nlps[1] : 0; return lim < batch_n ? lim : batch_n; }
      const uint32_t rem = n_remaining > nlps[v] ? n_remaining - nlps[v] : 0; return rem < kBatchN ? rem : kBatchN;
    };
    const int other = present[0] ? 0 : 2;
    const bool has_other = present[0] || present[2];
    const uint32_t wave_u = kRange ? b_begin + ((uni(wave) + kExpWaves - (b_begin & (kExpWaves - 1))) & (kExpWaves - 1)) : uni(wave);
    ExpPre pre[2], nxt[2];
    uint64_t st_cur[2] = {0, 0}, st_nxt[2] = {0, 0}, st_raw[2] = {0, 0};
    auto var_of = [&](int slot) -> int { return slot == 1 ? 1 : other; };
    auto issue_starts = [&](uint32_t batch, uint64_t (&st)[2]) {
#pragma unroll
      for (int sl = 0; sl < 2; sl++) {
        const int v = var_of(sl);
        st[sl] = ((sl == 1 || has_other) && batch < n_batches && cnt_of(batch, v) > 0) ? offpos_area[((uint64_t)ti * 3 + v) * offpos_stride + batch] : 0ull;
      }
    };
    auto prefetch = [&](uint32_t batch, const uint64_t (&st)[2], ExpPre (&dstp)[2]) {
#pragma unroll
      for (int sl = 0; sl < 2; sl++) {
        const int v = var_of(sl);
        if (sl == 0 && !has_other) continue;
        const uint32_t cnt = cnt_of(batch, v);
        if (cnt == 0) continue;
        const uint8_t PCO_GLOBAL* syms = (const uint8_t PCO_GLOBAL*)sym_area + ((uint64_t)ti * 3 + v) * sym_stride + (uint64_t)batch * kBatchN;
        expand_prefetch(dstp[sl], src, src_len, st[sl], cnt * max_ob[v], syms, cnt, n_bins[v] <= 1);
      }
    };
    if (wave_u < n_batches) {
      issue_starts(wave_u, st_cur); issue_starts(wave_u + kExpWaves, st_nxt);
      for (int sl = 0; sl < 2; sl++) { st_cur[sl] = uni(st_cur[sl]); st_nxt[sl] = uni(st_nxt[sl]); }
      prefetch(wave_u, st_cur, pre);
    }
    for (uint32_t batch = wave_u; batch < n_batches; batch += kExpWaves) {
      const uint32_t j0 = batch * kBatchN, n_remaining = n - j0;
      const uint32_t batch_n = n_remaining < kBatchN ? n_remaining : kBatchN;
      L prim[4] = {0, 0, 0, 0}, sec[4] = {0, 0, 0, 0};
      uint32_t prim_cnt = 0;
      issue_starts(batch + 2 * kExpWaves, st_raw);
      if (batch + kExpWaves < n_batches) prefetch(batch + kExpWaves, st_nxt, nxt);
#pragma unroll
      for (int sl = 0; sl < 2; sl++) {
        if (sl == 0 && !has_other) continue;
        const int v = var_of(sl);
        const uint32_t cnt = cnt_of(batch, v);
        if (cnt == 0) continue;
        const bool single_bin = n_bins[v] <= 1;
        if (v == 0) {
          uint32_t tmp[4];
          if (max_ob[0] != 0 || !single_bin) expand_item<uint32_t>(pre[0], stg, src, src_len, st_cur[0], cnt * max_ob[0], cnt, lowers, obs, single_bin, max_ob[0], tmp);
          else { const uint32_t l0 = (uint32_t)lowers[0]; for (int k = 0; k < 4; k++) tmp[k] = l0; }
          for (int k = 0; k < 4; k++) dlat[4 * lane + k] = 4 * lane + k < cnt ? tmp[k] : 0u;
        } else {
          L tmp[4];
          if (max_ob[v] != 0 || !single_bin) expand_item<L>(pre[sl], stg, src, src_len, st_cur[sl], cnt * max_ob[v], cnt, lowers + v * 256, obs + v * 256, single_bin, max_ob[v], tmp);
          else { const L l0 = (L)lowers[v * 256]; for (int k = 0; k < 4; k++) tmp[k] = 4 * lane + k < cnt ? l0 : (L)0; }
          if (v == 1) { for (int k = 0; k < 4; k++) prim[k] = tmp[k]; prim_cnt = cnt; } else { for (int k = 0; k < 4; k++) sec[k] = tmp[k]; }
        }
      }
#pragma unroll
      for (int sl = 0; sl < 2; sl++) { pre[sl] = nxt[sl]; st_cur[sl] = st_nxt[sl]; st_nxt[sl] = uni(st_raw[sl]); }
      L far_val[4] = {0, 0, 0, 0};
      if constexpr (kLb) {
        wave_sync_lds();
#pragma unroll
        for (int k = 0; k < 4; k++) {
          const uint32_t i = 4 * lane + k;
          const uint32_t lb = i < prim_cnt ? dlat[i] : 0u;
          const int64_t q = (int64_t)(state_n + j0 + i) - (int64_t)lb;
          const bool far = lb > i && lb <= (1u << window_n_log) && q >= 0 && (q < (int64_t)state_n || batch - (uint32_t)((q - state_n) >> 8) >= kExpRing);
          if (far) far_val[k] = to_latent_ordered<L>(__hip_atomic_load(&dst[q], __ATOMIC_RELAXED, __HIP_MEMORY_SCOPE_AGENT), num_kind);
        }
      }
      if (ordered) {
        while (__hip_atomic_load((uint32_t*)turn, __ATOMIC_RELAXED, __HIP_MEMORY_SCOPE_WORKGROUP) != batch) __builtin_amdgcn_s_sleep(1);
        __builtin_amdgcn_fence(__ATOMIC_ACQUIRE, "workgroup");
        if (dk[1] == kDeltaConsecutive) consecutive_decode<L>(prim, dord[1], moments0);
        if (present[2] && dk[2] == kDeltaConsecutive) consecutive_decode<L>(sec, dord[2], moments1);
        if constexpr (kLb) {
          __builtin_amdgcn_wave_barrier();
          const uint32_t window_n = 1u << window_n_log;
          const uint64_t kbase = (uint64_t)j0;
          for (int k = 0; k < 4; k++) {
            const uint32_t i = 4 * lane + k;
            L val = (L)(prim[k] + lmid<L>());
            uint32_t par = 0xffffffffu;
            if (i < prim_cnt) {
              uint32_t lb = dlat[i];
              if (lb > window_n) { lb_oob = 1; lb = 1; val = (L)(prim[k] + lmid<L>()); }
              if (lb == 0) { }
              else if (lb <= i) par = i - lb;
              else {
                const int64_t q = (int64_t)(state_n + kbase + i) - (int64_t)lb;
                if (q >= 0) {
                  const bool ring_hit = q >= (int64_t)state_n && batch - (uint32_t)((q - state_n) >> 8) < kExpRing;
                  if (ring_hit) val = (L)(val + hring[(uint32_t)(q - state_n) & (kExpRing * 256 - 1)]);
                  else if (dlat[i] <= window_n) val = (L)(val + far_val[k]);
                  else val = (L)(val + to_latent_ordered<L>(__hip_atomic_load(&dst[q], __ATOMIC_RELAXED, __HIP_MEMORY_SCOPE_AGENT), num_kind));
                }
              }
            }
            scratch[i] = val; parent[i] = par;
          }
          wave_sync_lds();
// ... 129 lines not shown
```

### pcodec_amd/csrc/decode_kernel.hip

```cpp
#pragma once
#include <type_traits>

#include "pco_dev.h"

namespace pcogfx {

#define PCO_LDS __attribute__((address_space(3)))
template <bool kLds, class T> using tptr = std::conditional_t<kLds, T PCO_LDS*, T PCO_GLOBAL*>;

struct MetaRef { const void* p; uint64_t len; };
struct RangeRef { uint64_t first, count; };
__host__ __device__ inline uint64_t range_end_batch(uint64_t first, uint64_t count) { return (first + count + 255) >> 8; }

struct VarInfo {
  uint32_t present, latent_bits, ans_size_log, n_bins, max_ob;
  uint32_t delta_kind, delta_order, window_n_log, state_n_log;
  uint32_t off_nodes, off_lower, off_ob, off_cum;
  uint32_t pad[3];
};
static_assert(sizeof(VarInfo) == 64, "VarInfo");

constexpr uint32_t kLdsWinOff = 0;
constexpr uint32_t kLdsSymOff = 544;
constexpr uint32_t kLdsMomOff = kLdsSymOff + 512;
constexpr uint32_t kLdsVarOff = kLdsMomOff + 128;
constexpr uint32_t kLdsDlatOff = kLdsVarOff + 192;
constexpr uint32_t kLdsScratchOff = kLdsDlatOff + 1024;
constexpr uint32_t kLdsParentOff = kLdsScratchOff + 2048;
constexpr uint32_t kLdsFixed = kLdsParentOff + 1024;
static_assert(kLdsFixed % 16 == 0, "LDS carve must stay 16-byte aligned");
constexpr uint64_t kTblWsBytesPerVar = (4ull << kMaxAnsBits) + (1ull << kMaxAnsBits) * (8 + 1 + 4) + 256;
constexpr uint64_t kTblWsBytes = 3 * kTblWsBytesPerVar;

__device__ __forceinline__ uint8_t PCO_LDS* lds_base() {
  extern __shared__ __attribute__((aligned(16))) uint8_t pco_lds[];
  return (uint8_t PCO_LDS*)pco_lds;
}
__device__ __forceinline__ void wave_sync_lds() {
  __builtin_amdgcn_fence(__ATOMIC_RELEASE, "workgroup");
  __builtin_amdgcn_wave_barrier();
}

__device__ __forceinline__ uint32_t var_table_bytes(uint32_t ans_size_log, uint32_t n_bins, uint32_t latent_bytes) {
  uint32_t b = (4u << ans_size_log);
  b += ((n_bins * latent_bytes + 7u) & ~7u);
  b += ((n_bins + 7u) & ~7u);
  b += (((n_bins + 1) * 4u + 7u) & ~7u);
  return b;
}

__device__ __forceinline__ uint32_t make_node(uint32_t base, uint32_t btr, uint32_t sym) { return base | (btr << 14) | (sym << 18); }

template <class LV, bool kLds>
__device__ __noinline__ bool build_var_tables(tptr<kLds, uint8_t> tbl, uint32_t vi, MetaReader& mr, uint32_t& status) {
  const uint32_t lane = lane_id();
  VarInfo PCO_LDS* vinfo = (VarInfo PCO_LDS*)(lds_base() + kLdsVarOff) + vi;
  const uint32_t asl = uni(vinfo->ans_size_log), n_bins = uni(vinfo->n_bins), latent_bits = uni(vinfo->latent_bits);
  const uint32_t T = 1u << asl;
  tptr<kLds, uint32_t> nodes = (tptr<kLds, uint32_t>)(tbl + uni(vinfo->off_nodes));
  tptr<kLds, LV> lowers = (tptr<kLds, LV>)(tbl + uni(vinfo->off_lower));
  tptr<kLds, uint8_t> obs = tbl + uni(vinfo->off_ob);
  tptr<kLds, uint32_t> cum = (tptr<kLds, uint32_t>)(tbl + uni(vinfo->off_cum));
  const uint32_t obb = offset_bits_bits(latent_bits);
  const uint32_t bin_bits = asl + latent_bits + obb;
  const uint64_t bins_start = mr.bit;
  uint32_t bad = 0, max_ob = 0, carry = 0;
  for (uint32_t b0 = 0; b0 < n_bins; b0 += 64) {
    const uint32_t b = b0 + lane;
    uint32_t w = 0;
    if (b < n_bins) {
      const uint64_t at = bins_start + (uint64_t)b * bin_bits;
      w = (uint32_t)mr.peek(at, asl) + 1;
      const uint64_t lower = mr.peek(at + asl, latent_bits);
      const uint32_t ob = (uint32_t)mr.peek(at + asl + latent_bits, obb);
      if (ob > latent_bits) bad = 1;
      lowers[b] = (LV)lower; obs[b] = (uint8_t)ob;
      max_ob = max_ob > ob ? max_ob : ob;
    }
    const uint32_t incl = wave_incl_scan(w);
    if (b < n_bins) cum[b] = carry + incl - w;
    carry += wave_last(incl);
  }
  if (lane == 0) { cum[n_bins] = carry; }
  mr.bit = bins_start + (uint64_t)n_bins * bin_bits;
  max_ob = uni(wave_max_u32(max_ob));
  if (lane == 0) vinfo->max_ob = max_ob;
  if (!mr.in_bounds()) { status = PCO_GFX_INSUFFICIENT_DATA; return false; }
  if (uni(wave_or_u32(bad))) { status = PCO_GFX_CORRUPTION; return false; }
  if (n_bins == 0) {
    if (lane == 0) nodes[0] = make_node(0, 0, 0);
    wave_sync_lds();
    return true;
  }
  if (carry != T) { status = PCO_GFX_CORRUPTION; return false; }
  wave_sync_lds();
  uint32_t stride = (3 * T) / 5; if ((stride & 1) == 0) stride += 1;
  for (uint32_t t = lane; t < T; t += 64) {
    uint32_t lo = 0, hi = n_bins;
    while (hi - lo > 1) { const uint32_t mid = (lo + hi) >> 1; if (cum[mid] <= t) lo = mid; else hi = mid; }
    nodes[(stride * t) & (T - 1)] = lo;
  }
  wave_sync_lds();
  for (uint32_t b0 = 0; b0 < n_bins; b0 += 64) {
    const uint32_t b = b0 + lane;
    uint32_t w = 0;
    if (b < n_bins) w = cum[b + 1] - cum[b];
    wave_sync_lds();
    if (b < n_bins) cum[b] = w;
    wave_sync_lds();
  }
  const uint32_t sym_bits = 32 - clz_u32(n_bins - 1 > 0 ? n_bins - 1 : 1);
  for (uint32_t i0 = 0; i0 < T; i0 += 64) {
    const uint32_t i = i0 + lane;
    const bool act = i < T;
    const uint32_t s = act ? nodes[i] : 0xffffffffu;
    uint64_t m = __ballot(act);
    for (uint32_t bit = 0; bit < sym_bits; bit++) {
      const uint64_t bm = __ballot((s >> bit) & 1);
      m &= ((s >> bit) & 1) ? bm : ~bm;
    }
    const uint64_t lt = ((uint64_t)1 << lane) - 1;
    const uint32_t rank = __popcll(m & lt), gcount = __popcll(m);
    const uint32_t basec = act ? cum[s] : 0;
    wave_sync_lds();
    if (act && rank == 0) cum[s] = basec + gcount;
    wave_sync_lds();
    if (act) {
      const uint32_t x_s = basec + rank;
      const uint32_t btr = clz_u32(x_s) - clz_u32(T);
      nodes[i] = make_node((x_s << btr) - T, btr, s);
    }
  }
  wave_sync_lds();
  return true;
}

template <bool kLds>
__device__ __forceinline__ uint64_t walk_ans(gcptr_u8 src, uint64_t src_len, uint64_t bitpos, uint32_t cnt,
                                              tptr<kLds, uint32_t> nodes, uint32_t& st) {
  const uint32_t lane = lane_id();
  uint32_t PCO_LDS* win = (uint32_t PCO_LDS*)(lds_base() + kLdsWinOff);
  uint16_t PCO_LDS* sym_stage = (uint16_t PCO_LDS*)(lds_base() + kLdsSymOff);
  const uint64_t dw0 = bitpos >> 5;
  {
    const uint64_t w = load_u64_le_safe(src, dw0 * 4 + (uint64_t)lane * 8, src_len + 16);
    win[2 * lane] = (uint32_t)w; win[2 * lane + 1] = (uint32_t)(w >> 32);
    if (lane < 4) {
      const uint64_t w2 = load_u64_le_safe(src, dw0 * 4 + 512 + (uint64_t)lane * 8, src_len + 16);
      win[128 + 2 * lane] = (uint32_t)w2; win[128 + 2 * lane + 1] = (uint32_t)(w2 >> 32);
    }
  }
  wave_sync_lds();
  uint32_t rel = (uint32_t)(bitpos & 31);
  if (lane < 4) {
    const uint32_t steps = (cnt + 3) >> 2;
    for (uint32_t g = 0; g < steps; g++) {
      const bool act = 4 * g + lane < cnt;
      const uint32_t node = nodes[st];
      const uint32_t d = rel >> 5;
      const uint32_t w0 = win[d], w1 = win[d + 1], w2 = win[d + 2], w3 = win[d + 3];
      const uint32_t btr = act ? ((node >> 14) & 15u) : 0u;
      uint32_t p1 = (uint32_t)__builtin_amdgcn_mov_dpp((int)btr, 0x90 , 0xf, 0xf, false);
      p1 = lane >= 1 ? p1 : 0;
      uint32_t incl = btr + p1;
      uint32_t p2 = (uint32_t)__builtin_amdgcn_mov_dpp((int)incl, 0x40 , 0xf, 0xf, false);
      p2 = lane >= 2 ? p2 : 0;
      incl += p2;
      const uint32_t excl = incl - btr;
      const uint32_t tot = (uint32_t)__builtin_amdgcn_mov_dpp((int)incl, 0xff , 0xf, 0xf, false);
      const uint32_t sh = (rel & 31) + excl;
      const uint32_t sel = sh >> 5;
      const uint32_t lo = sel == 0 ? w0 : (sel == 1 ? w1 : w2);
      const uint32_t hi = sel == 0 ? w1 : (sel == 1 ? w2 : w3);
      const uint32_t bits = __builtin_amdgcn_alignbit(hi, lo, sh & 31);
      const uint32_t val = bits & ((1u << btr) - 1u);
      if (act) {
        sym_stage[4 * g + lane] = (uint16_t)(node >> 18);
        st = (node & 0x3fffu) + val;
      }
      rel += tot;
    }
  }
  const uint32_t rel_end = uni(rel);
  wave_sync_lds();
  return (dw0 << 5) + rel_end;
}

template <class LV, bool kLds>
__device__ __forceinline__ uint64_t unpack_offsets(gcptr_u8 src, uint64_t src_len, uint64_t bitpos, uint32_t cnt,
                                                    tptr<kLds, LV> lowers, tptr<kLds, uint8_t> obs, bool single_bin, LV out[4]) {
  const uint32_t lane = lane_id();
  uint16_t PCO_LDS* sym_stage = (uint16_t PCO_LDS*)(lds_base() + kLdsSymOff);
  uint32_t ob[4]; LV low[4];
#pragma unroll
  for (int k = 0; k < 4; k++) {
    const uint32_t i = 4 * lane + k;
    const bool act = i < cnt;
    const uint32_t s = (single_bin || !act) ? 0u : (uint32_t)sym_stage[i];
    ob[k] = act ? (uint32_t)obs[s] : 0u;
    low[k] = act ? lowers[s] : (LV)0;
  }
  const uint32_t t = ob[0] + ob[1] + ob[2] + ob[3];
  const uint32_t incl = wave_incl_scan(t);
  const uint32_t total = wave_last(incl);
  uint64_t b = bitpos + (incl - t);
#pragma unroll
  for (int k = 0; k < 4; k++) {
    uint64_t val = 0;
    if (ob[k] != 0) {
      const uint64_t byte = b >> 3; const uint32_t sh = (uint32_t)(b & 7);
      val = load_u64_le_safe(src, byte, src_len + 16) >> sh;
      if (sh + ob[k] > 64) val |= load_u64_le_safe(src, byte + 8, src_len + 16) << (64 - sh);
      if (ob[k] < 64) val &= ((uint64_t)1 << ob[k]) - 1;
    }
    out[k] = (LV)(low[k] + (LV)val);
    b += ob[k];
  }
  return bitpos + total;
}

template <class L>
__device__ __forceinline__ void consecutive_decode(L x[4], uint32_t order, L PCO_LDS* moments) {
  const uint32_t lane = lane_id();
#pragma unroll
  for (int k = 0; k < 4; k++) x[k] = (L)(x[k] + lmid<L>());
  for (uint32_t m = order; m-- > 0;) {
    const L mom = moments[m];
    const L e1 = x[0], e2 = (L)(e1 + x[1]), e3 = (L)(e2 + x[2]), t = (L)(e3 + x[3]);
    const L incl = wave_incl_scan(t);
    const L base = (L)(mom + (L)(incl - t));
    x[0] = base; x[1] = (L)(base + e1); x[2] = (L)(base + e2); x[3] = (L)(base + e3);
    const L total = wave_last(incl);
    wave_sync_lds();
    if (lane == 0) moments[m] = (L)(mom + total);
    wave_sync_lds();
  }
}

template <class L>
__device__ __forceinline__ L join_one(uint32_t mode_kind, uint32_t num_kind, L base_latent, uint32_t k, L p, L s) {
  switch (mode_kind) {
    case kClassic: return from_latent_ordered<L>(p, num_kind);
    case kIntMult: return from_latent_ordered<L>((L)((L)(p * base_latent) + s), num_kind);
    case kFloatQuant: {
      const L sign_cutoff = (L)(lmid<L>() >> k);
      const L lowmax = (L)(((L)1 << k) - 1);
      const L low = p >= sign_cutoff ? s : (L)(lowmax - s);
      return from_latent_ordered<L>((L)((L)(p << k) + low), kFloat);
    }
    default: {
      if constexpr (sizeof(L) >= 4) {
        typedef typename FloatOf<L>::F F;
        const F base = bits_to_float(from_latent_ordered<L>(base_latent, kFloat));
        const F unadjusted = int_float_from_latent<L>(p) * base;
        const L l = (L)(to_latent_ordered<L>(float_to_bits(unadjusted), kFloat) + s + lmid<L>());
        return from_latent_ordered<L>(l, kFloat);
      } else if constexpr (sizeof(L) == 2) {
        const uint32_t base = (uint32_t)from_latent_ordered<L>(base_latent, kFloat);
        const uint32_t unadjusted = half_mul(half_int_float_from_latent((uint32_t)p), base);
        const L l = (L)(to_latent_ordered<L>((L)unadjusted, kFloat) + s + lmid<L>());
        return from_latent_ordered<L>(l, kFloat);
      } else return 0;
    }
  }
}

struct PageParams {
  uint32_t mode_kind, mode_k, num_kind, n;
  uint64_t mode_base;
  uint64_t dict_byte; uint32_t dict_n;
  uint32_t conv_order, conv_quant;
  void PCO_GLOBAL* sec_hist;
  gcptr_u8 dict_src = nullptr;
  uint32_t limit = 0;
  uint32_t* progress = nullptr;
};
constexpr uint32_t kLdsConvOff = kLdsParentOff;

template <class L>
__device__ __forceinline__ void conv1_decode(L x[4], uint32_t dst_n, uint32_t order, uint32_t quant) {
  const uint32_t lane = lane_id();
  uint32_t PCO_LDS* res = (uint32_t PCO_LDS*)(lds_base() + kLdsScratchOff);
  const int64_t PCO_LDS* cw = (const int64_t PCO_LDS*)(lds_base() + kLdsConvOff);
  constexpr int kConvBits = LBits<L>::v == 32 ? 64 : 2 * (int)LBits<L>::v;
  auto wrap = [&](uint64_t v) -> int64_t { return kConvBits == 64 ? (int64_t)v : (int64_t)(v << (64 - kConvBits)) >> (64 - kConvBits); };
#pragma unroll
  for (int k = 0; k < 4; k++) res[order + 4 * lane + k] = (uint32_t)(L)(x[k] + lmid<L>());
  wave_sync_lds();
  if (lane == 0) {
    const int64_t bias = wrap((uint64_t)cw[0]);
    for (uint32_t i = 0; i < dst_n; i++) {
      uint64_t sum = (uint64_t)bias;
      for (uint32_t k = 0; k < order; k++) sum += (uint64_t)wrap((uint64_t)cw[1 + k]) * (uint64_t)res[i + k];
      int64_t sc = wrap(sum);
      if (sc < 0) sc = 0;
      res[order + i] = (uint32_t)(L)((L)res[order + i] + (L)(uint64_t)(sc >> quant));
    }
  }
  wave_sync_lds();
#pragma unroll
  for (int k = 0; k < 4; k++) x[k] = (L)res[4 * lane + k];
  wave_sync_lds();
  if (lane == 0) for (uint32_t j = 0; j < order; j++) res[j] = res[dst_n + j];
  wave_sync_lds();
}

template <class L, bool kLds, bool kRange = false>
__device__ __noinline__ void decode_page_body(gcptr_u8 src, uint64_t src_len, MetaReader& mr, tptr<kLds, uint8_t> tbl,
                                             const PageParams& pp, L PCO_GLOBAL* dst, uint32_t& status) {
  const uint32_t lane = lane_id();
  uint8_t PCO_LDS* smem = lds_base();
  uint64_t PCO_LDS* mom64 = (uint64_t PCO_LDS*)(smem + kLdsMomOff);
  uint32_t PCO_LDS* dlat = (uint32_t PCO_LDS*)(smem + kLdsDlatOff);
  L PCO_LDS* scratch = (L PCO_LDS*)(smem + kLdsScratchOff);
  uint32_t PCO_LDS* parent = (uint32_t PCO_LDS*)(smem + kLdsParentOff);
  VarInfo PCO_LDS* vinfo = (VarInfo PCO_LDS*)(smem + kLdsVarOff);
  L PCO_LDS* moments0 = (L PCO_LDS*)(mom64);
  L PCO_LDS* moments1 = (L PCO_LDS*)(mom64 + 8);
  const uint32_t mode_kind = pp.mode_kind, mode_k = pp.mode_k, num_kind = pp.num_kind, n = pp.n;
  const L mode_base = (L)pp.mode_base;

// ... 581 lines not shown
```

### pcodec_amd/csrc/pco_gfx.hip

```cpp
#include "pco_host.h"
#include "pco_half.h"

#include <algorithm>
#include <atomic>
#include <chrono>
#include <thread>
#include <mutex>
#include <condition_variable>
#include <functional>
#include <sched.h>
#include <pthread.h>
#include <sys/syscall.h>
#include <unistd.h>
#include <cstdlib>
#include <cstring>
#include <memory>
#include <unordered_map>

#include "pco_auto_host.inc"
#include "decode_kernel.hip"
#include "decode_trail.hip"
#include "encode_kernels.hip"
#include "encode_lookback.hip"
#include "encode_conv1.hip"
#include "encode_dict.hip"
#include "encode_hist_select.hip"
#include "encode_hist_literal.hip"
#include "auto_mode_kernels.hip"
#include "encode_fast.hip"
#include "encode_walkseg.hip"
#include "encode_walkpack.hip"
#include "stream_kernels.hip"
#include "stream_wrapped.hip"

namespace pcogfx {

static thread_local HostError g_err{PCO_GFX_OK, ""};
void set_error(int status, const std::string& msg) { g_err.status = status; g_err.msg = msg; }
void clear_error() { g_err.status = PCO_GFX_OK; g_err.msg.clear(); }

struct WorkspaceHolder {
  std::unordered_map<int, std::unique_ptr<Workspace>> by_device;
  ~WorkspaceHolder() {
    const bool worker = (long)syscall(SYS_gettid) != (long)getpid();
    for (auto& kv : by_device) {
      if (worker) { int cur = 0; const bool sw = hipGetDevice(&cur) == hipSuccess && cur != kv.first && hipSetDevice(kv.first) == hipSuccess; kv.second->release_all(); if (kv.second->last_event) (void)hipEventDestroy(kv.second->last_event); if (sw) (void)hipSetDevice(cur); }
      else (void)kv.second.release();
    }
  }
};
static thread_local WorkspaceHolder g_ws_holder;
Workspace& workspace() {
  int dev = 0;
  hipError_t e = hipGetDevice(&dev);
  if (e != hipSuccess) throw HostError{PCO_GFX_DEVICE_ERROR, std::string("no HIP device: ") + hipGetErrorString(e)};
  std::unique_ptr<Workspace>& slot = g_ws_holder.by_device[dev];
  if (!slot) { slot.reset(new Workspace()); slot->device = dev; }
  return *slot;
}

static void require_device() {
  int n = 0;
  hipError_t e = hipGetDeviceCount(&n);
  if (e != hipSuccess || n <= 0)
    throw HostError{PCO_GFX_DEVICE_ERROR, "libpco_gfx: no MI355X/HIP device visible; this library has no CPU fallback"};
}

static size_t baseline_meta_max_size(int latent_bits) {
  const size_t delta_max_bits = 4 + 5 + 5 + 64 + 32 * 32;
  const size_t var_bits = kBitsAnsSizeLog + kBitsNBins + (0 + (size_t)latent_bits + offset_bits_bits(latent_bits));
  return (kBitsModeVariant + delta_max_bits + var_bits + 7) / 8;
}
size_t guarantee_wrapped_chunk_size(int latent_bits, size_t n) { return baseline_meta_max_size(latent_bits) + (n * (size_t)latent_bits + 7) / 8; }
size_t guarantee_standalone_chunk_size(int latent_bits, size_t n) { return 1 + 3 + guarantee_wrapped_chunk_size(latent_bits, n); }
size_t guarantee_standalone_header_size() { return 4 + 1 + (kBitsVarintPower + 64 + 8 + 7) / 8 + 2; }
bool n_per_page(uint64_t max_page_n, size_t n, std::vector<size_t>& out) {
  out.clear();
  if (max_page_n == 0) max_page_n = 1u << 18;
  if (n == 0) return true;
  size_t n_pages = (n + max_page_n - 1) / max_page_n;
  size_t low = n / n_pages, r = n % n_pages;
  out.assign(n_pages, low);
  for (size_t i = 0; i < r; i++) out[i] = low + 1;
  return true;
}

static PcoError fail_with(const HostError& e, PcoError code) { set_error(e.status, e.msg); return code; }

struct KernelProfile {
  bool on = false;
  struct Rec { const char* name; hipEvent_t a, b; };
  std::vector<Rec> recs;
  std::vector<hipEvent_t> pool;
  bool take(hipEvent_t& e) { if (!pool.empty()) { e = pool.back(); pool.pop_back(); return true; } return hipEventCreate(&e) == hipSuccess; }
  void give(hipEvent_t e) { pool.push_back(e); }
};
static thread_local KernelProfile g_prof;
struct ScopedKernelTimer {
  hipStream_t s; hipEvent_t b{}; bool live = false;
  ScopedKernelTimer(const char* name, hipStream_t stream) : s(stream) {
    if (!g_prof.on) return;
    hipEvent_t a;
    if (!g_prof.take(a)) return;
    if (!g_prof.take(b)) { g_prof.give(a); return; }
    (void)hipEventRecord(a, s);
    g_prof.recs.push_back({name, a, b}); live = true;
  }
  ~ScopedKernelTimer() { if (live) (void)hipEventRecord(b, s); }
};
hipEvent_t profile_span_begin(const char* name, hipStream_t stream) {
  if (!g_prof.on) return nullptr;
  hipEvent_t a, b;
  if (!g_prof.take(a)) return nullptr;
  if (!g_prof.take(b)) { g_prof.give(a); return nullptr; }
  (void)hipEventRecord(a, stream);
  g_prof.recs.push_back({name, a, b});
  return b;
}
#define PCO_TIMED_LAUNCH(name, stream, ...) do { ScopedKernelTimer _t(name, stream); hipLaunchKernelGGL(__VA_ARGS__); } while (0)

static uint32_t g_decode_lds_bytes = 16 * 1024;
static bool g_decode_trail = env_not_zero("PCO_GFX_DEC_TRAIL");
static char g_trail_debug = env_char("PCO_GFX_TRAIL_DEBUG");
static bool g_trail_always = env_first_is("PCO_GFX_DEC_TRAIL", '2');

static void ensure_side_stream(Workspace& ws) {
  if (!ws.side_stream) PCO_HIP_CHECK(hipStreamCreateWithFlags(&ws.side_stream, hipStreamNonBlocking));
  if (!ws.side_stream2) PCO_HIP_CHECK(hipStreamCreateWithFlags(&ws.side_stream2, hipStreamNonBlocking));
  if (!ws.join_event2) PCO_HIP_CHECK(hipEventCreateWithFlags(&ws.join_event2, hipEventDisableTiming));
  if (!ws.fork_event) PCO_HIP_CHECK(hipEventCreateWithFlags(&ws.fork_event, hipEventDisableTiming));
  if (!ws.join_event) PCO_HIP_CHECK(hipEventCreateWithFlags(&ws.join_event, hipEventDisableTiming));
  if (!ws.n_cus) { hipDeviceProp_t prop; PCO_HIP_CHECK(hipGetDeviceProperties(&prop, ws.device)); ws.n_cus = prop.multiProcessorCount > 0 ? prop.multiProcessorCount : 256; }
}

static void launch_decode(size_t n_tasks, const PcoGfxDecodeTask* tasks, PcoGfxTaskResult* results,
                          PcoGfxTaskResult* d_results_user, hipStream_t stream, const MetaRef* metas = nullptr) {
  if (n_tasks == 0) return;
  Workspace& ws = workspace();
  std::vector<uint32_t> ids[4];
  bool any_bad = false;
  for (size_t i = 0; i < n_tasks; i++) {
    const int b = dtype_bits(tasks[i].dtype);
    if (b == 64) ids[0].push_back((uint32_t)i); else if (b == 32) ids[1].push_back((uint32_t)i); else if (b == 16) ids[2].push_back((uint32_t)i); else if (b == 8) ids[3].push_back((uint32_t)i); else any_bad = true;
  }
  if (any_bad) throw HostError{PCO_GFX_INVALID_ARGUMENT, "decode: invalid number type"};
  const size_t task_bytes = n_tasks * sizeof(PcoGfxDecodeTask);
  const size_t ids_off = (task_bytes + 15) & ~(size_t)15, metas_off = (ids_off + n_tasks * sizeof(uint32_t) + 15) & ~(size_t)15;
  uint8_t* d_base = (uint8_t*)ws.tasks.ensure(metas_off + (metas ? n_tasks * sizeof(MetaRef) : 0) + 64);
  PcoGfxDecodeTask* d_tasks = (PcoGfxDecodeTask*)d_base;
  uint32_t* d_ids = (uint32_t*)(d_base + ids_off);
  const MetaRef* d_metas = nullptr;
  if (metas) { PCO_HIP_CHECK(hipMemcpyAsync(d_base + metas_off, metas, n_tasks * sizeof(MetaRef), hipMemcpyHostToDevice, stream)); d_metas = (const MetaRef*)(d_base + metas_off); }
  PcoGfxTaskResult* d_results = d_results_user ? d_results_user : (PcoGfxTaskResult*)ws.results.ensure(n_tasks * sizeof(PcoGfxTaskResult));
  PCO_HIP_CHECK(hipMemcpyAsync(d_tasks, tasks, task_bytes, hipMemcpyHostToDevice, stream));
  const bool mixed = (ids[0].size() != n_tasks) && (ids[1].size() != n_tasks) && (ids[2].size() != n_tasks) && (ids[3].size() != n_tasks);
  std::vector<uint32_t> flat;
  size_t id_off[4] = {0, 0, 0, 0};
  if (mixed) {
    for (int g = 0; g < 4; g++) { id_off[g] = flat.size(); flat.insert(flat.end(), ids[g].begin(), ids[g].end()); }
    PCO_HIP_CHECK(hipMemcpyAsync(d_ids, flat.data(), flat.size() * sizeof(uint32_t), hipMemcpyHostToDevice, stream));
  }
  const uint32_t budget = g_decode_lds_bytes - kLdsFixed;
  size_t max_grid = 0;
  constexpr size_t kGeneralGrid = 4096;
  for (int g = 0; g < 4; g++) max_grid = std::max(max_grid, std::min<size_t>(ids[g].size(), kGeneralGrid));
  uint8_t* tbl = results ? nullptr : (uint8_t*)ws.tbl_ws.ensure(max_grid * kTblWsBytes);
  uint64_t max_cap = 0; bool plain = true;
  for (size_t i = 0; i < n_tasks; i++) { max_cap = std::max<uint64_t>(max_cap, tasks[i].dst_cap); if (tasks[i].flags & PCO_GFX_TASK_META_ONLY) plain = false; }
  const uint64_t sym_stride = ((max_cap + 255) & ~(uint64_t)255) + 256, offpos_stride = sym_stride / 256 + 2;
  const bool fast = plain && n_tasks * 3 * sym_stride <= ((size_t)48 << 30);
  DecPlan* d_plans = nullptr; uint8_t* d_bins = nullptr; uint8_t* d_sym = nullptr; uint64_t* d_offpos = nullptr;
  if (fast) {
    d_plans = (DecPlan*)ws.dec_plans.ensure(n_tasks * sizeof(DecPlan));
    d_bins = (uint8_t*)ws.dec_bins.ensure(n_tasks * kBinsAreaPerTask);
    d_sym = (uint8_t*)ws.dec_sym.ensure(n_tasks * 3 * sym_stride + 64);
    d_offpos = (uint64_t*)ws.dec_offpos.ensure(n_tasks * 3 * offpos_stride * 8);
  }
  const uint32_t need_hist = results ? kStatusNeedHist : (uint32_t)PCO_GFX_UNSUPPORTED;
  for (int g = 0; g < 4; g++) {
    if (ids[g].empty()) continue;
    const uint32_t cnt = (uint32_t)ids[g].size();
    const uint32_t grid = (uint32_t)std::min<size_t>(cnt, kGeneralGrid);
    const uint32_t* idp = mixed ? d_ids + id_off[g] : nullptr;
    const uint32_t* filt = fast ? (const uint32_t*)d_plans : nullptr;
    const uint32_t fstride = (uint32_t)(sizeof(DecPlan) / 4);
    if (fast) {
      const uint32_t n_wb = (cnt + 7) / 8;
      uint32_t* d_progress = nullptr;
      uint32_t* d_givebacks = nullptr;
      constexpr uint32_t kTrailMinChunks = 1024;
      const bool use_trail = g_decode_trail && (cnt >= kTrailMinChunks || g_trail_debug != '\0' || g_trail_always);
      if (use_trail) {
        ensure_side_stream(ws);
        d_progress = (uint32_t*)ws.dec_progress.ensure((size_t)n_wb * kTrailProgressStride * sizeof(uint32_t));
        PCO_HIP_CHECK(hipMemsetAsync(d_progress, 0, (size_t)n_wb * kTrailProgressStride * sizeof(uint32_t), stream));
        if (!ws.dec_stats.p) { ws.dec_stats.ensure(256); PCO_HIP_CHECK(hipMemsetAsync(ws.dec_stats.p, 0, 256, stream)); }
        d_givebacks = (uint32_t*)ws.dec_stats.p;
      }
      const uint32_t trail_grid = use_trail ? std::min<uint32_t>(n_wb, (uint32_t)ws.n_cus * 4u) : 0u;
#define PCO_FAST_DECODE(L, name)                                                                                                                          \
      {                                                                                                                                                   \
        static const bool _walk_ok = hipFuncSetAttribute((const void*)dec_walk_kernel<L, 8>, hipFuncAttributeMaxDynamicSharedMemorySize, (int)(4 * WalkCfg<8>::kWalkLdsBytes)) == hipSuccess && \
                                     hipFuncSetAttribute((const void*)dec_walk_kernel<L, 4>, hipFuncAttributeMaxDynamicSharedMemorySize, (int)(4 * WalkCfg<4>::kWalkLdsBytes)) == hipSuccess;   \
        if (!_walk_ok) throw HostError{PCO_GFX_DEVICE_ERROR, "cannot reserve LDS for dec_walk_kernel"};                                                   \
      }                                                                                                                                                   \
      if (use_trail) {                                                                                                                                    \
        ScopedKernelTimer _span("dec_walk+trail<" name ">", stream);                                                                                      \
        if (g_trail_debug == 'd') {    \
          hipLaunchKernelGGL((dec_trail_kernel<L, false>), dim3(trail_grid), dim3(64 * kTrailWaves), 0, stream, d_tasks, idp, cnt, d_plans, d_bins, d_sym, sym_stride, d_offpos, offpos_stride, d_progress, n_wb, d_metas); \
          hipLaunchKernelGGL((dec_trail_kernel<L, true>), dim3(trail_grid), dim3(64 * kTrailWaves), 0, stream, d_tasks, idp, cnt, d_plans, d_bins, d_sym, sym_stride, d_offpos, offpos_stride, d_progress, n_wb, d_metas);  \
        }                                                                                                                                                 \
        PCO_HIP_CHECK(hipEventRecord(ws.fork_event, stream));                                                                                             \
                              \
        static const bool _quad_ok = hipFuncSetAttribute((const void*)dec_walk_trail_kernel<L>, hipFuncAttributeMaxDynamicSharedMemorySize, (int)(4 * WalkCfg<8>::kWalkLdsBytes)) == hipSuccess; \
        if (!_quad_ok) throw HostError{PCO_GFX_DEVICE_ERROR, "cannot reserve LDS for dec_walk_trail_kernel"};                                             \
        PCO_TIMED_LAUNCH("~dec_walk_kernel<" name ">", stream, (dec_walk_trail_kernel<L>), dim3((n_wb + 3) / 4), dim3(256), 4 * WalkCfg<8>::kWalkLdsBytes, stream, \
                         d_tasks, idp, cnt, d_plans, d_bins, d_sym, sym_stride, d_offpos, offpos_stride, d_results, d_progress, d_metas);                 \
                  \
        PCO_HIP_CHECK(hipStreamWaitEvent(ws.side_stream2, ws.fork_event, 0));                                                                             \
        PCO_TIMED_LAUNCH("~dec_walk_kernel(rest)<" name ">", ws.side_stream2, (dec_walk_kernel<L, 8>), dim3((n_wb + 3) / 4), dim3(256), 4 * WalkCfg<8>::kWalkLdsBytes, ws.side_stream2, \
                         d_tasks, idp, cnt, d_plans, d_bins, d_sym, sym_stride, d_offpos, offpos_stride, 0u, d_results, d_progress, d_metas);             \
        PCO_HIP_CHECK(hipEventRecord(ws.join_event2, ws.side_stream2));                                                                                   \
        hipStream_t ts = g_trail_debug == 's' ? stream : ws.side_stream;                                                                                  \
        PCO_HIP_CHECK(hipStreamWaitEvent(ws.side_stream, ws.fork_event, 0));                                                                              \
                                                                 \
        if (g_trail_debug != 'n' && g_trail_debug != 'd') PCO_TIMED_LAUNCH("~dec_trail_kernel<" name ">", ts, (dec_trail_kernel<L, false>), dim3(trail_grid), dim3(64 * kTrailWaves), 0, ts, \
                         d_tasks, idp, cnt, d_plans, d_bins, d_sym, sym_stride, d_offpos, offpos_stride, d_progress, n_wb, d_metas);                               \
        if (g_trail_debug != 'n' && g_trail_debug != 'd') PCO_TIMED_LAUNCH("~dec_trail2_kernel<" name ">", ts, (dec_trail_kernel<L, true>), dim3(trail_grid), dim3(64 * kTrailWaves), 0, ts, \
                         d_tasks, idp, cnt, d_plans, d_bins, d_sym, sym_stride, d_offpos, offpos_stride, d_progress, n_wb, d_metas);                               \
        PCO_HIP_CHECK(hipEventRecord(ws.join_event, ws.side_stream));                                                                                     \
        PCO_HIP_CHECK(hipStreamWaitEvent(stream, ws.join_event, 0));                                                                                      \
        PCO_HIP_CHECK(hipStreamWaitEvent(stream, ws.join_event2, 0));                                                                                     \
      } else PCO_TIMED_LAUNCH("dec_walk_kernel<" name ">", stream, (dec_walk_kernel<L, 8>), dim3((n_wb + 3) / 4), dim3(256), 4 * WalkCfg<8>::kWalkLdsBytes, stream, \
                       d_tasks, idp, cnt, d_plans, d_bins, d_sym, sym_stride, d_offpos, offpos_stride, 0u, d_results, (uint32_t*)nullptr, d_metas);       \
      PCO_TIMED_LAUNCH("dec_walk4_kernel<" name ">", stream, (dec_walk_kernel<L, 4>), dim3((cnt + 15) / 16), dim3(256), 4 * WalkCfg<4>::kWalkLdsBytes, stream, \
                       d_tasks, idp, cnt, d_plans, d_bins, d_sym, sym_stride, d_offpos, offpos_stride, kStatusRetryK4, d_results, (uint32_t*)nullptr, d_metas); \
      PCO_TIMED_LAUNCH("dec_expand_kernel<" name ">", stream, (dec_expand_kernel<L, false>), dim3(grid), dim3(256), kExpLdsBytes, stream,               \
                       d_tasks, d_results, idp, cnt, d_plans, d_bins, d_sym, sym_stride, d_offpos, offpos_stride, (const uint32_t*)d_progress, d_givebacks);    \
      PCO_TIMED_LAUNCH("dec_expand_lb_kernel<" name ">", stream, (dec_expand_kernel<L, true>), dim3(grid), dim3(256), kExpLbLdsBytes, stream,           \
                       d_tasks, d_results, idp, cnt, d_plans, d_bins, d_sym, sym_stride, d_offpos, offpos_stride, (const uint32_t*)d_progress, d_givebacks);
      if (g == 0) { PCO_FAST_DECODE(uint64_t, "u64") } else if (g == 1) { PCO_FAST_DECODE(uint32_t, "u32") } else if (g == 2) { PCO_FAST_DECODE(uint16_t, "u16") } else { PCO_FAST_DECODE(uint8_t, "u8") }
#undef PCO_FAST_DECODE
    }
    if (g == 0) PCO_TIMED_LAUNCH("pco_decode_kernel<u64>", stream, pco_decode_kernel<uint64_t>, dim3(grid), dim3(64), g_decode_lds_bytes, stream, d_tasks, d_results, idp, cnt, budget, tbl, filt, fstride, kStatusRetryLegacy, (uint8_t*)nullptr, (const uint64_t*)nullptr, need_hist, d_metas);
    else if (g == 1) PCO_TIMED_LAUNCH("pco_decode_kernel<u32>", stream, pco_decode_kernel<uint32_t>, dim3(grid), dim3(64), g_decode_lds_bytes, stream, d_tasks, d_results, idp, cnt, budget, tbl, filt, fstride, kStatusRetryLegacy, (uint8_t*)nullptr, (const uint64_t*)nullptr, need_hist, d_metas);
    else if (g == 2) PCO_TIMED_LAUNCH("pco_decode_kernel<u16>", stream, pco_decode_kernel<uint16_t>, dim3(grid), dim3(64), g_decode_lds_bytes, stream, d_tasks, d_results, idp, cnt, budget, tbl, filt, fstride, kStatusRetryLegacy, (uint8_t*)nullptr, (const uint64_t*)nullptr, need_hist, d_metas);
    else PCO_TIMED_LAUNCH("pco_decode_kernel<u8>", stream, pco_decode_kernel<uint8_t>, dim3(grid), dim3(64), g_decode_lds_bytes, stream, d_tasks, d_results, idp, cnt, budget, tbl, filt, fstride, kStatusRetryLegacy, (uint8_t*)nullptr, (const uint64_t*)nullptr, need_hist, d_metas);
    PCO_HIP_CHECK(hipGetLastError());
  }
  if (results) {
    PCO_HIP_CHECK(hipMemcpyAsync(results, d_results, n_tasks * sizeof(PcoGfxTaskResult), hipMemcpyDeviceToHost, stream));
    PCO_HIP_CHECK(hipStreamSynchronize(stream));
    std::vector<uint32_t> again[4]; size_t n_again = 0;
    for (size_t i = 0; i < n_tasks; i++) if (results[i].status == kStatusNeedHist) {
      const int b = dtype_bits(tasks[i].dtype);
      again[b == 64 ? 0 : (b == 32 ? 1 : (b == 16 ? 2 : 3))].push_back((uint32_t)i); n_again++;
    }
    if (n_again) {
      std::vector<uint32_t> flat_ids; std::vector<uint64_t> offs; uint64_t hist_bytes = 0;
      size_t goff[4];
      for (int g = 0; g < 4; g++) { goff[g] = flat_ids.size(); for (uint32_t i : again[g]) { flat_ids.push_back(i); offs.push_back(hist_bytes); hist_bytes += ((tasks[i].dst_cap * (uint64_t)(dtype_bits(tasks[i].dtype) / 8)) + 255) & ~(uint64_t)255; } }
      uint8_t* d_hist = (uint8_t*)ws.dec_hist.ensure(hist_bytes + n_again * 12 + 256);
      uint64_t* d_hoff = (uint64_t*)(d_hist + ((hist_bytes + 15) & ~(uint64_t)15));
      uint32_t* d_again = (uint32_t*)(d_hoff + n_again);
      PCO_HIP_CHECK(hipMemcpyAsync(d_hoff, offs.data(), n_again * 8, hipMemcpyHostToDevice, stream));
      PCO_HIP_CHECK(hipMemcpyAsync(d_again, flat_ids.data(), n_again * 4, hipMemcpyHostToDevice, stream));
      uint8_t* tbl2 = (uint8_t*)ws.tbl_ws.ensure(std::min<size_t>(n_again, kGeneralGrid) * kTblWsBytes);
      for (int g = 0; g < 4; g++) {
        if (again[g].empty()) continue;
        const uint32_t cnt = (uint32_t)again[g].size(), grid = (uint32_t)std::min<size_t>(cnt, kGeneralGrid);
        const uint32_t* idp = d_again + goff[g]; const uint64_t* hop = d_hoff + goff[g];
        if (g == 0) PCO_TIMED_LAUNCH("pco_decode_kernel<u64>", stream, pco_decode_kernel<uint64_t>, dim3(grid), dim3(64), g_decode_lds_bytes, stream, d_tasks, d_results, idp, cnt, budget, tbl2, (const uint32_t*)nullptr, 0u, 0u, d_hist, hop, (uint32_t)PCO_GFX_UNSUPPORTED, d_metas);
        else if (g == 1) PCO_TIMED_LAUNCH("pco_decode_kernel<u32>", stream, pco_decode_kernel<uint32_t>, dim3(grid), dim3(64), g_decode_lds_bytes, stream, d_tasks, d_results, idp, cnt, budget, tbl2, (const uint32_t*)nullptr, 0u, 0u, d_hist, hop, (uint32_t)PCO_GFX_UNSUPPORTED, d_metas);
        else if (g == 2) PCO_TIMED_LAUNCH("pco_decode_kernel<u16>", stream, pco_decode_kernel<uint16_t>, dim3(grid), dim3(64), g_decode_lds_bytes, stream, d_tasks, d_results, idp, cnt, budget, tbl2, (const uint32_t*)nullptr, 0u, 0u, d_hist, hop, (uint32_t)PCO_GFX_UNSUPPORTED, d_metas);
        else PCO_TIMED_LAUNCH("pco_decode_kernel<u8>", stream, pco_decode_kernel<uint8_t>, dim3(grid), dim3(64), g_decode_lds_bytes, stream, d_tasks, d_results, idp, cnt, budget, tbl2, (const uint32_t*)nullptr, 0u, 0u, d_hist, hop, (uint32_t)PCO_GFX_UNSUPPORTED, d_metas);
      }
      PCO_HIP_CHECK(hipGetLastError());
      PCO_HIP_CHECK(hipMemcpyAsync(results, d_results, n_tasks * sizeof(PcoGfxTaskResult), hipMemcpyDeviceToHost, stream));
      PCO_HIP_CHECK(hipStreamSynchronize(stream));
    }
  }
}

}

using namespace pcogfx;

extern "C" {

int pco_gfx_last_status(void) { return g_err.status; }
const char* pco_gfx_last_error(void) { return g_err.msg.c_str(); }
int pco_gfx_device_count(void) { int n = 0; if (hipGetDeviceCount(&n) != hipSuccess) return 0; return n; }
void pco_gfx_release_workspace(void) {
  try { Workspace& w = workspace(); if (w.has_last && w.last_event) (void)hipEventSynchronize(w.last_event); w.release_all(); } catch (...) {}
}

size_t pco_gfx_workspace_bytes(void) {
  try {
    static const bool trace = std::getenv("PCO_GFX_TRACE") != nullptr;
    if (trace) fprintf(stderr, "[pco_gfx trace] workspace: %s\n", workspace().device_report().c_str());
    return workspace().device_bytes();
  } catch (...) { return 0; }
}

static unsigned long long trail_stat(int which) {
  try {
    Workspace& w = workspace();
    const unsigned long long acc = which == 0 ? w.acc_givebacks : w.acc_marked;
    if (!w.dec_stats.p) return acc;
    if (w.has_last && w.last_event) (void)hipEventSynchronize(w.last_event);
    uint32_t v[2] = {0, 0};
    if (hipMemcpy(v, w.dec_stats.p, 8, hipMemcpyDeviceToHost) != hipSuccess) return acc;
    return acc + v[which];
  } catch (...) { return 0; }
}
unsigned long long pco_gfx_trail_givebacks(void) { return trail_stat(0); }
unsigned long long pco_gfx_trail_marked(void) { return trail_stat(1); }
unsigned long long pco_gfx_strict_histogram_fallbacks(void) {
  try {
    Workspace& w = workspace();
    if (!w.enc_strict.p) return w.acc_strict;
    if (w.has_last && w.last_event) (void)hipEventSynchronize(w.last_event);
    uint32_t v = 0;
    if (hipMemcpy(&v, w.enc_strict.p, 4, hipMemcpyDeviceToHost) != hipSuccess) return w.acc_strict;
    return w.acc_strict + v;
  } catch (...) { return 0; }
}

void pco_gfx_profile_begin(void) {
  for (auto& r : g_prof.recs) { g_prof.give(r.a); g_prof.give(r.b); }
  g_prof.recs.clear(); g_prof.on = true;
}
int pco_gfx_profile_end(char* names, size_t names_cap, float* ms, int cap) {
  g_prof.on = false;
  int n = 0; size_t pos = 0;
  for (auto& r : g_prof.recs) {
    float t = 0.f;
    (void)hipEventSynchronize(r.b);
    (void)hipEventElapsedTime(&t, r.a, r.b);
    if (n < cap) {
      const size_t len = std::strlen(r.name) + 1;
      if (names && pos + len <= names_cap) { std::memcpy(names + pos, r.name, len); pos += len; }
      if (ms) ms[n] = t;
      n++;
    }
    g_prof.give(r.a); g_prof.give(r.b);
  }
  g_prof.recs.clear();
  return n;
}

size_t pco_gfx_guarantee_file_size(size_t n, unsigned char dtype, uint64_t max_page_n) {
  const int bits = dtype_bits(dtype);
  if (!bits) return 0;
  std::vector<size_t> pages;
  n_per_page(max_page_n, n, pages);
  size_t res = guarantee_standalone_header_size() + 1;
  for (size_t p : pages) res += guarantee_standalone_chunk_size(bits, p);
  return res;
}
size_t pco_standalone_guarantee_file_size(size_t n, unsigned char dtype) { return pco_gfx_guarantee_file_size(n, dtype, 0); }
size_t pco_gfx_guarantee_chunk_size(size_t n, unsigned char dtype) {
  const int bits = dtype_bits(dtype);
  return bits ? guarantee_standalone_chunk_size(bits, n) : 0;
}

size_t pco_gfx_write_standalone_header(void* dst, size_t dst_cap, uint64_t n_hint, unsigned char uniform_dtype) {
  HostBitWriter w;
  w.write(0x216f6370u, 32); w.write(3, 8); w.write(uniform_dtype, 8);
  const uint32_t power = n_hint == 0 ? 1 : (64 - (uint32_t)__builtin_clzll(n_hint));
  w.write(power - 1, kBitsVarintPower); w.write(n_hint, power); w.finish_byte();
  w.write(4, 8); w.write(1, 8);
  if (w.bytes() > dst_cap) return 0;
  std::memcpy(dst, w.buf.data(), w.bytes());
  return w.bytes();
}
size_t pco_gfx_write_standalone_footer(void* dst, size_t dst_cap) {
  if (dst_cap < 1) return 0;
  *(uint8_t*)dst = 0;
  return 1;
}
size_t pco_wrapped_write_header(void* dst, size_t dst_cap) {
  if (dst_cap < 2) return 0;
  ((uint8_t*)dst)[0] = 4; ((uint8_t*)dst)[1] = 1;
  return 2;
}
enum PcoError pco_wrapped_read_header(const void* src, size_t len, size_t* consumed, uint8_t* major, uint8_t* minor) {
  clear_error();
  const uint8_t* p = (const uint8_t*)src;
  if (len < 1) { set_error(PCO_GFX_INSUFFICIENT_DATA, "empty header"); return PcoDecompressionError; }
  uint8_t mj = p[0], mn = 0; size_t used = 1;
  if (mj >= 4) { if (len < 2) { set_error(PCO_GFX_INSUFFICIENT_DATA, "short header"); return PcoDecompressionError; } mn = p[1]; used = 2; }
  if (mj > 4) { set_error(PCO_GFX_CORRUPTION, "file's format version definitely cannot be decompressed"); return PcoDecompressionError; }
  if (consumed) *consumed = used; if (major) *major = mj; if (minor) *minor = mn;
  return PcoSuccess;
}

enum PcoError pco_gfx_decompress_chunks(size_t n_tasks, const PcoGfxDecodeTask* tasks, PcoGfxTaskResult* results,
                                        PcoGfxTaskResult* d_results, void* stream) {
  clear_error();
  try {
    require_device();
    { WorkspaceUse use(workspace(), (hipStream_t)stream); launch_decode(n_tasks, tasks, results, d_results, (hipStream_t)stream); }
    if (results) for (size_t i = 0; i < n_tasks; i++) if (results[i].status != PCO_GFX_OK) {
      set_error((int)results[i].status, "decode task " + std::to_string(i) + " failed");
      return PcoDecompressionError;
    }
    return PcoSuccess;
  } catch (const HostError& e) { return fail_with(e, PcoDecompressionError); }
}

enum PcoError pco_gfx_decompress_pages(size_t n_tasks, const PcoGfxPageTask* tasks, PcoGfxTaskResult* results, PcoGfxTaskResult* d_results, void* stream) {
  clear_error();
  try {
    require_device();
    std::vector<PcoGfxDecodeTask> dt(n_tasks); std::vector<MetaRef> refs(n_tasks);
    for (size_t i = 0; i < n_tasks; i++) {
      const PcoGfxPageTask& t = tasks[i];
      if (t.format_major > 4) throw HostError{PCO_GFX_CORRUPTION, "page task " + std::to_string(i) + ": the file's format version definitely cannot be decompressed"};
      if (t.meta == nullptr || t.page == nullptr) throw HostError{PCO_GFX_INVALID_ARGUMENT, "page task " + std::to_string(i) + ": null ChunkMeta or page"};
      dt[i] = PcoGfxDecodeTask{t.page, t.page_len, t.dst, t.page_n, t.dtype, PCO_GFX_TASK_WRAPPED_PAGE | (t.format_major << 8)};
      refs[i] = MetaRef{t.meta, t.meta_len};
    }
    { WorkspaceUse use(workspace(), (hipStream_t)stream); launch_decode(n_tasks, dt.data(), results, d_results, (hipStream_t)stream, refs.data()); }
    if (results) for (size_t i = 0; i < n_tasks; i++) if (results[i].status != PCO_GFX_OK) {
      set_error((int)results[i].status, "page task " + std::to_string(i) + " failed");
      return PcoDecompressionError;
    }
    return PcoSuccess;
  } catch (const HostError& e) { return fail_with(e, PcoDecompressionError); }
}

enum PcoError pco_gfx_compact_chunks(size_t n_tasks, const PcoGfxEncodeTask* tasks, const PcoGfxTaskResult* d_results, void* d_dst,
                                     uint64_t dst_cap, uint64_t dst_offset, uint64_t* d_offsets, uint64_t* total, void* stream_) {
  clear_error();
  try {
    require_device();
    hipStream_t stream = (hipStream_t)stream_;
    if (!d_results || !d_offsets || (!d_dst && dst_cap)) throw HostError{PCO_GFX_INVALID_ARGUMENT, "compact: null device array"};
    if (n_tasks >= (1ull << 31)) throw HostError{PCO_GFX_INVALID_ARGUMENT, "compact: too many chunks"};
    Workspace& ws = workspace();
    WorkspaceUse use(ws, stream);
    uint8_t* d_base = (uint8_t*)ws.compact_tasks.ensure(n_tasks * sizeof(PcoGfxEncodeTask) + 64);
    uint32_t* d_over = (uint32_t*)d_base; PcoGfxEncodeTask* d_tasks = (PcoGfxEncodeTask*)(d_base + 64);
    uint64_t max_cap = 0;
    for (size_t i = 0; i < n_tasks; i++) max_cap = std::max<uint64_t>(max_cap, tasks[i].dst_cap);
    if (n_tasks) PCO_HIP_CHECK(hipMemcpyAsync(d_tasks, tasks, n_tasks * sizeof(PcoGfxEncodeTask), hipMemcpyHostToDevice, stream));
    PCO_TIMED_LAUNCH("compact_scan_kernel", stream, compact_scan_kernel, dim3(1), dim3(1024), 0, stream, d_results, (uint32_t)n_tasks, dst_offset, dst_cap, d_offsets, d_over);
    if (n_tasks) {
      const uint64_t slice = 64 * 1024;
      const uint32_t slices = (uint32_t)std::max<uint64_t>(1, (max_cap + slice - 1) / slice);
      if ((uint64_t)slices * n_tasks >= (1ull << 31)) throw HostError{PCO_GFX_INVALID_ARGUMENT, "compact: too many chunks for one call"};
      PCO_TIMED_LAUNCH("compact_copy_kernel", stream, compact_copy_kernel, dim3((uint32_t)(slices * n_tasks)), dim3(256), 0, stream, d_tasks, d_results, d_offsets, (uint8_t*)d_dst, d_over, (uint32_t)n_tasks, slice, slices);
    }
    PCO_HIP_CHECK(hipGetLastError());
    if (total) {
      uint32_t over = 0;
      PCO_HIP_CHECK(hipMemcpyAsync(total, d_offsets + n_tasks, 8, hipMemcpyDeviceToHost, stream));
      PCO_HIP_CHECK(hipMemcpyAsync(&over, d_over, 4, hipMemcpyDeviceToHost, stream));
      PCO_HIP_CHECK(hipStreamSynchronize(stream));
      if (over) throw HostError{PCO_GFX_INVALID_ARGUMENT, "compact: destination too small"};
    }
    return PcoSuccess;
  } catch (const HostError& e) { return fail_with(e, PcoCompressionError); }
}

static bool parse_standalone_header_host(const uint8_t* p, size_t len, unsigned char dtype, size_t& off, uint32_t& fmt_major) {
  if (len < 6 || p[0] != 'p' || p[1] != 'c' || p[2] != 'o' || p[3] != '!') return false;
  const uint32_t sv = p[4];
  if (sv < 2 || sv > 3) return false;
  size_t pos = 5;
  if (sv >= 3) { const uint32_t uniform = p[pos++]; if (uniform != 0 && uniform != dtype) return false; }
  if (pos + 9 > len) return false;
  uint64_t bits = 0; for (int i = 0; i < 9 && i < 8; i++) bits |= (uint64_t)p[pos + i] << (8 * i);
  const uint32_t power = 1 + (uint32_t)(bits & 63u);
  const uint32_t vbits = kBitsVarintPower + power, vbytes = (vbits + 7) / 8;
  if (vbits & 7) {
    const uint32_t last = p[pos + vbytes - 1];
    if ((last >> (vbits & 7)) != 0) return false;
  }
  pos += vbytes;
  if (pos >= len) return false;
  fmt_major = p[pos++];
  if (fmt_major > 4) return false;
  if (fmt_major >= 4) pos++;
  if (pos > len) return false;
  off = pos;
  return true;
}

enum PcoError pco_standalone_simple_decompress_into(const void* compressed, size_t compressed_len, unsigned char dtype,
                                                    void* dst, size_t dst_cap, size_t* n_written) {
  clear_error();
  const int bits = dtype_bits(dtype);
  if (!bits) { set_error(PCO_GFX_INVALID_ARGUMENT, "invalid dtype"); return PcoInvalidType; }
  try {
    require_device();
    Workspace& ws = workspace();
    WorkspaceUse use(ws, 0);
    uint8_t* d_in = (uint8_t*)ws.io_in.ensure(compressed_len + 64);
    const size_t esz = (size_t)(bits / 8), out_bytes = dst_cap * esz;
    uint8_t* d_out = (uint8_t*)ws.io_out.ensure(out_bytes + 64);
    PCO_HIP_CHECK(hipMemsetAsync(d_in + compressed_len, 0, 64, 0));
    if (compressed_len) PCO_HIP_CHECK(hipMemcpyAsync(d_in, compressed, compressed_len, hipMemcpyHostToDevice, 0));
    size_t off = 0, done = 0; uint32_t fmt_major = 4;
    const bool by_chunk = parse_standalone_header_host((const uint8_t*)compressed, compressed_len, dtype, off, fmt_major);
    if (!by_chunk) {
      PcoGfxDecodeTask task{d_in, compressed_len, d_out, dst_cap, dtype, PCO_GFX_TASK_HAS_FILE_HEADER};
      PcoGfxTaskResult res{};
      launch_decode(1, &task, &res, nullptr, 0);
      if (res.status != PCO_GFX_OK) {
        set_error((int)res.status, "decompression failed");
        return PcoDecompressionError;
      }
      done = res.n_out;
    } else {
      for (;;) {
        if (off >= compressed_len) { set_error(PCO_GFX_INSUFFICIENT_DATA, "decompression failed: the file ends without its terminator"); return PcoDecompressionError; }
        if (((const uint8_t*)compressed)[off] == 0) break;
        PcoGfxDecodeTask task{d_in + off, compressed_len - off, d_out + done * esz, std::min<size_t>(dst_cap - done, kMaxEntries), dtype, PCO_GFX_TASK_ONE_CHUNK | (fmt_major << 8)};
        PcoGfxTaskResult res{};
        launch_decode(1, &task, &res, nullptr, 0);
        if (res.status != PCO_GFX_OK) { set_error((int)res.status, "decompression failed"); return PcoDecompressionError; }
        done += res.n_out; off += res.consumed;
        if (res.aux & 1u) { if (res.consumed == 0) break; continue; }
        if (!(res.aux & 2u)) { set_error(PCO_GFX_INSUFFICIENT_DATA, "decompression failed: the file ends without its terminator"); return PcoDecompressionError; }
        break;
      }
    }
    if (done) PCO_HIP_CHECK(hipMemcpy(dst, d_out, done * esz, hipMemcpyDeviceToHost));
    if (n_written) *n_written = done;
    return PcoSuccess;
  } catch (const HostError& e) { return fail_with(e, PcoDecompressionError); }
}

}

#include "pco_gfx_encode_api.inc"
#include "pco_gfx_comm.inc"

extern "C" int pco_gfx_debug_float_screen(const void* values, size_t n, uint32_t dtype, uint32_t* out) {
  using namespace pcogfx;
  if (n == 0 || n > kAutoCap || dtype_kind(dtype) != kFloat || dtype_bits(dtype) < 32) return PCO_GFX_INVALID_ARGUMENT;
  const size_t eb = dtype_bits(dtype) / 8;
  void* d_vals = nullptr; void* d_sbuf = nullptr; uint32_t* d_idx = nullptr; FloatStatsTask* d_task = nullptr; FloatStatsResult* d_res = nullptr;
  std::vector<uint32_t> idx(n); for (size_t i = 0; i < n; i++) idx[i] = (uint32_t)i;
  int rc = PCO_GFX_OK;
  if (hipFuncSetAttribute((const void*)auto_float_stats_kernel, hipFuncAttributeMaxDynamicSharedMemorySize, (int)kAutoStage1LdsBytes) != hipSuccess) return PCO_GFX_DEVICE_ERROR;
  if (hipMalloc(&d_vals, n * eb) != hipSuccess || hipMalloc(&d_sbuf, kAutoCap * 8) != hipSuccess || hipMalloc((void**)&d_idx, n * 4) != hipSuccess || hipMalloc((void**)&d_task, sizeof(FloatStatsTask)) != hipSuccess || hipMalloc((void**)&d_res, sizeof(FloatStatsResult)) != hipSuccess) rc = PCO_GFX_DEVICE_ERROR;
  if (rc == PCO_GFX_OK) {
    const FloatStatsTask t{d_vals, d_idx, d_sbuf, (uint32_t)n, dtype};
    static FloatStatsResult r;
    if (hipMemcpy(d_vals, values, n * eb, hipMemcpyHostToDevice) != hipSuccess || hipMemcpy(d_idx, idx.data(), n * 4, hipMemcpyHostToDevice) != hipSuccess || hipMemcpy(d_task, &t, sizeof(t), hipMemcpyHostToDevice) != hipSuccess) rc = PCO_GFX_DEVICE_ERROR;
    else {
      hipLaunchKernelGGL(auto_float_stats_kernel, dim3(1), dim3(kAutoT), kAutoStage1LdsBytes, 0, d_task, d_res);
      if (hipMemcpy(&r, d_res, sizeof(r), hipMemcpyDeviceToHost) != hipSuccess) rc = PCO_GFX_DEVICE_ERROR;
      else {
        out[0] = r.s_size; out[1] = r.tz5; out[2] = r.n_gcd; out[3] = r.sim[0]; out[4] = r.sim[1]; out[5] = r.sim[2]; for (int i = 0; i < 56; i++) out[6 + i] = r.hist[i];
        out[62] = r.has_euclid; out[63] = (uint32_t)r.k; out[64] = r.n_ints; out[65] = (uint32_t)r.base_c; out[66] = (uint32_t)(r.base_c >> 32);
      }
    }
  }
  (void)hipFree(d_vals); (void)hipFree(d_sbuf); (void)hipFree(d_idx); (void)hipFree(d_task); (void)hipFree(d_res);
  return rc;
}

extern "C" int64_t pco_gfx_debug_lookback_routes(uint8_t* out, size_t cap) {
  using namespace pcogfx;
  Workspace& w = workspace();
  const size_t n = w.lb_n;
  if (n == 0 || !w.enc_lb.p || (std::max(w.lb_redo_off, w.lb_skip_off) + n) * 4 > w.enc_lb.cap) return 0;
  if (hipDeviceSynchronize() != hipSuccess) return -(int64_t)PCO_GFX_DEVICE_ERROR;
  std::vector<uint32_t> redo(n), skip(n);
  const uint32_t* base = (const uint32_t*)w.enc_lb.p;
  if (hipMemcpy(redo.data(), base + w.lb_redo_off, n * 4, hipMemcpyDeviceToHost) != hipSuccess || hipMemcpy(skip.data(), base + w.lb_skip_off, n * 4, hipMemcpyDeviceToHost) != hipSuccess) return -(int64_t)PCO_GFX_DEVICE_ERROR;
  for (size_t k = 0; k < n && k < cap; k++) out[k] = redo[k] ? 2 : (skip[k] ? 1 : 0);
  return (int64_t)n;
}
```

### pcodec_amd/csrc/pco_host.h

```cpp
#pragma once
#include <hip/hip_runtime.h>
#include <stdint.h>

#include <algorithm>
#include <cstdlib>
#include <string>
#include <vector>

#include "../../include/pco_gfx.h"

namespace pcogfx {

struct HostError {
  int status;
  std::string msg;
  bool oom = false;
};

void set_error(int status, const std::string& msg);
void clear_error();

inline bool env_is_one(const char* name) { const char* e = std::getenv(name); return e != nullptr && e[0] == '1'; }
inline bool env_not_zero(const char* name) { const char* e = std::getenv(name); return !(e != nullptr && e[0] == '0'); }
inline char env_char(const char* name) { const char* e = std::getenv(name); return e != nullptr ? e[0] : '\0'; }
inline bool env_first_is(const char* name, char c) { const char* e = std::getenv(name); return e != nullptr && e[0] == c; }

#define PCO_HIP_CHECK(expr)                                                                   \
  do {                                                                                        \
    hipError_t _e = (expr);                                                                   \
    if (_e != hipSuccess) throw pcogfx::HostError{PCO_GFX_DEVICE_ERROR, std::string(#expr) + ": " + hipGetErrorString(_e)}; \
  } while (0)

struct DevBuf {
  void* p = nullptr;
  size_t cap = 0;
  void* ensure(size_t bytes) {
    if (bytes > cap) {
      if (p) { (void)hipFree(p); p = nullptr; cap = 0; }
      size_t want = bytes + std::min<size_t>(bytes / 8, (size_t)64 << 20) + 256;
      hipError_t e = hipMalloc(&p, want);
      if (e != hipSuccess) { p = nullptr; (void)hipGetLastError(); throw HostError{PCO_GFX_DEVICE_ERROR, std::string("hipMalloc failed: ") + hipGetErrorString(e), true}; }
      cap = want;
    }
    return p;
  }
  void release() { if (p) (void)hipFree(p); p = nullptr; cap = 0; }
};

struct HostBuf {
  void* p = nullptr;
  size_t cap = 0;
  void* ensure(size_t bytes) {
    if (bytes > cap) {
      if (p) { (void)hipHostFree(p); p = nullptr; cap = 0; }
      size_t want = bytes + bytes / 8 + 256;
      hipError_t e = hipHostMalloc(&p, want, hipHostMallocDefault);
      if (e != hipSuccess) { p = nullptr; (void)hipGetLastError(); throw HostError{PCO_GFX_DEVICE_ERROR, std::string("hipHostMalloc failed: ") + hipGetErrorString(e), true}; }
      cap = want;
    }
    return p;
  }
  void release() { if (p) (void)hipHostFree(p); p = nullptr; cap = 0; }
};

struct Workspace {
  int device = -1;
  hipStream_t last_stream = nullptr; hipEvent_t last_event = nullptr; bool has_last = false;
  DevBuf tasks, results, tbl_ws;
  DevBuf dec_plans, dec_bins, dec_sym, dec_offpos;
  DevBuf dec_progress;
  DevBuf dec_stats;
  hipStream_t side_stream = nullptr, side_stream2 = nullptr; hipEvent_t fork_event = nullptr, join_event = nullptr, join_event2 = nullptr;
  int n_cus = 0;
  DevBuf dec_hist;
  DevBuf io_in, io_out;
  DevBuf compact_tasks;
  DevBuf enc_state;
  DevBuf enc_lat, enc_lat2, enc_sort, enc_ans, enc_small, enc_lb, enc_walk;
  DevBuf enc_lbprops;
  size_t lb_n = 0, lb_redo_off = 0, lb_skip_off = 0;
  DevBuf enc_sym, enc_answ, enc_bat, enc_run, enc_fstate, enc_vlut;
  DevBuf enc_strict;
  DevBuf enc_conv;
  DevBuf enc_dict, enc_dict_hbm;
  DevBuf auto_idx, auto_samp, auto_tasks, auto_sum, auto_log2;
  HostBuf h_samp, h_sum;
#define PCO_WS_BUFS(X) X(tasks) X(results) X(tbl_ws) X(dec_plans) X(dec_bins) X(dec_sym) X(dec_offpos) X(dec_progress) X(dec_stats) X(dec_hist) X(io_in) X(io_out) X(compact_tasks) X(enc_state) \
  X(enc_lat) X(enc_lat2) X(enc_sort) X(enc_ans) X(enc_small) X(enc_lb) X(enc_lbprops) X(enc_walk) X(enc_sym) X(enc_answ) X(enc_bat) X(enc_run) X(enc_fstate) X(enc_vlut) X(enc_strict) X(enc_conv) X(enc_dict) X(enc_dict_hbm) X(auto_idx) X(auto_samp) X(auto_tasks) X(auto_sum) X(auto_log2)
  size_t device_bytes() const {
    size_t b = 0;
#define PCO_WS_ADD(name) b += name.cap;
    PCO_WS_BUFS(PCO_WS_ADD)
#undef PCO_WS_ADD
    return b;
  }
  std::string device_report() const {
    std::string r;
#define PCO_WS_REP(name) if (name.cap) r += std::string(#name) + "=" + std::to_string(name.cap) + " ";
    PCO_WS_BUFS(PCO_WS_REP)
#undef PCO_WS_REP
    return r;
  }
  unsigned long long acc_givebacks = 0, acc_marked = 0, acc_strict = 0;
  void fold_counters() {
    uint32_t v[2] = {0, 0};
    if (dec_stats.p && hipMemcpy(v, dec_stats.p, 8, hipMemcpyDeviceToHost) == hipSuccess) { acc_givebacks += v[0]; acc_marked += v[1]; }
    uint32_t f = 0;
    if (enc_strict.p && hipMemcpy(&f, enc_strict.p, 4, hipMemcpyDeviceToHost) == hipSuccess) acc_strict += f;
  }
  void release_all() {
    fold_counters();
    lb_n = 0;
    if (side_stream) { (void)hipStreamSynchronize(side_stream); (void)hipStreamDestroy(side_stream); side_stream = nullptr; }
    if (side_stream2) { (void)hipStreamSynchronize(side_stream2); (void)hipStreamDestroy(side_stream2); side_stream2 = nullptr; }
    if (fork_event) { (void)hipEventDestroy(fork_event); fork_event = nullptr; }
    if (join_event) { (void)hipEventDestroy(join_event); join_event = nullptr; }
    if (join_event2) { (void)hipEventDestroy(join_event2); join_event2 = nullptr; }
    tasks.release(); results.release(); tbl_ws.release(); dec_plans.release(); dec_bins.release(); dec_sym.release(); dec_offpos.release(); dec_progress.release(); dec_stats.release(); dec_hist.release(); io_in.release(); io_out.release(); compact_tasks.release();
    enc_state.release(); enc_lat.release(); enc_lat2.release(); enc_sort.release(); enc_ans.release(); enc_small.release(); enc_lb.release(); enc_lbprops.release(); enc_walk.release(); enc_sym.release(); enc_answ.release(); enc_bat.release(); enc_run.release(); enc_fstate.release(); enc_vlut.release(); enc_strict.release(); enc_conv.release(); enc_dict.release(); enc_dict_hbm.release(); auto_idx.release(); auto_samp.release(); auto_tasks.release(); auto_sum.release(); auto_log2.release(); h_samp.release(); h_sum.release();
  }
};
Workspace& workspace();
struct WorkspaceUse {
  Workspace& ws; hipStream_t stream;
  WorkspaceUse(Workspace& w, hipStream_t s) : ws(w), stream(s) {
    if (ws.has_last && ws.last_stream != stream && ws.last_event) (void)hipStreamWaitEvent(stream, ws.last_event, 0);
  }
  ~WorkspaceUse() {
    if (!ws.last_event && hipEventCreateWithFlags(&ws.last_event, hipEventDisableTiming) != hipSuccess) { ws.last_event = nullptr; return; }
    if (hipEventRecord(ws.last_event, stream) == hipSuccess) { ws.last_stream = stream; ws.has_last = true; }
  }
};

struct HostBitWriter {
  std::vector<uint8_t> buf;
  uint64_t bit = 0;
  void write(uint64_t v, uint32_t n) {
    if (n == 0) return;
    if (n < 64) v &= ((uint64_t)1 << n) - 1;
    size_t need = (size_t)((bit + n + 7) >> 3) + 9;
    if (buf.size() < need) buf.resize(need * 2, 0);
    for (uint32_t i = 0; i < n;) {
      size_t byte = (size_t)(bit >> 3); uint32_t sh = (uint32_t)(bit & 7);
      uint32_t take = 8 - sh; if (take > n - i) take = n - i;
      buf[byte] |= (uint8_t)(((v >> i) & ((1u << take) - 1)) << sh);
      i += take; bit += take;
    }
  }
  void finish_byte() { bit = (bit + 7) & ~(uint64_t)7; }
  size_t bytes() const { return (size_t)((bit + 7) >> 3); }
};

size_t guarantee_wrapped_chunk_size(int latent_bits, size_t n);
size_t guarantee_standalone_chunk_size(int latent_bits, size_t n);
size_t guarantee_standalone_header_size();
bool n_per_page(uint64_t max_page_n, size_t n, std::vector<size_t>& out);

}
```

Measured before the change: 1732.

## Prefetch next walk round's bitstream into registers and stage into LDS window

```diff
diff --git a/include/pco_gfx.h b/include/pco_gfx.h
--- a/include/pco_gfx.h
+++ b/include/pco_gfx.h
@@ -143,6 +143,8 @@
 unsigned long long pco_gfx_strict_histogram_fallbacks(void);
 unsigned long long pco_gfx_trail_givebacks(void);
 unsigned long long pco_gfx_trail_marked(void);
+unsigned long long pco_gfx_walk_prestaged(void);
+unsigned long long pco_gfx_walk_restaged(void);
 
 void pco_gfx_profile_begin(void);
 int pco_gfx_profile_end(char* names, size_t names_cap, float* ms, int cap);
diff --git a/pcodec_amd/_lib.py b/pcodec_amd/_lib.py
--- a/pcodec_amd/_lib.py
+++ b/pcodec_amd/_lib.py
@@ -105,6 +105,10 @@
         L.pco_gfx_trail_givebacks.argtypes = []
         L.pco_gfx_trail_marked.restype = C.c_ulonglong
         L.pco_gfx_trail_marked.argtypes = []
+        L.pco_gfx_walk_prestaged.restype = C.c_ulonglong
+        L.pco_gfx_walk_prestaged.argtypes = []
+        L.pco_gfx_walk_restaged.restype = C.c_ulonglong
+        L.pco_gfx_walk_restaged.argtypes = []
         L.pco_gfx_guarantee_chunk_size.argtypes = [C.c_size_t, C.c_ubyte]
         L.pco_standalone_simple_compress_into.argtypes = [C.c_void_p, C.c_size_t, C.c_ubyte, C.c_void_p, C.c_void_p,
                                                           C.c_size_t, C.POINTER(C.c_size_t)]
diff --git a/pcodec_amd/csrc/decode_fast.hip b/pcodec_amd/csrc/decode_fast.hip
--- a/pcodec_amd/csrc/decode_fast.hip
+++ b/pcodec_amd/csrc/decode_fast.hip
@@ -389,11 +389,13 @@
   return block_trail_kinds(tasks, task_ids, n_ids, wb, metas) != 0;
 }
 
-template <class L, uint32_t kWQ, bool kTrail, bool kRange = false>
+constexpr uint32_t kPreQ = 24;
+template <class L, uint32_t kWQ, bool kTrail, bool kRange = false, bool kPre = false>
 __device__ __forceinline__ void dec_walk_body(const PcoGfxDecodeTask* tasks, const uint32_t* task_ids, uint32_t n_ids, DecPlan* plans,
                                               uint8_t* bins_area, uint8_t* sym_area, uint64_t sym_stride, uint64_t* offpos_area, uint64_t offpos_stride,
                                               uint32_t accept_status, PcoGfxTaskResult* results, uint32_t* progress, const MetaRef* metas,
-                                              const RangeRef* ranges = nullptr) {
+                                              const RangeRef* ranges = nullptr, unsigned long long* stats = nullptr) {
+  static_assert(!kPre || !kRange, "the range kernels stage every round's section where it starts");
   static_assert(!kTrail || !kRange, "range tasks never take the publishing walker");
   static_assert(!kTrail || kWQ == 8, "the trailing expanders follow the eight-chunk walker");
   const uint32_t wb = walk_block_id();
@@ -459,7 +461,7 @@
   }
   bool my_fused = false;
   uint32_t my_fused_kind = 0;
-  uint32_t PCO_GLOBAL* my_progress = nullptr;
+  auto my_progress = [&]() { uint32_t sl = slot < kWQ ? slot : 0u; asm volatile("" : "+v"(sl)); return (uint32_t PCO_GLOBAL*)progress + (uint64_t)wb * kTrailProgressStride + sl; };
   if constexpr (kTrail) {
     if (my_active && slot < kWQ) {
       const bool prim_ok = vinfo[0].present == 0 && vinfo[1].n_bins >= 1 && vinfo[1].n_bins <= kTrailMaxBins && vinfo[1].max_ob <= 16 &&
@@ -469,32 +471,48 @@
                vinfo[2].max_ob <= 16 && vinfo[2].delta_kind == kDeltaNone && (vinfo[1].n_bins > 1 || vinfo[2].n_bins > 1)) my_fused_kind = 2;
       my_fused = my_fused_kind != 0;
     }
-    if (slot < kWQ) my_progress = (uint32_t PCO_GLOBAL*)progress + (uint64_t)wb * kTrailProgressStride + slot;
     if (j == 0 && my_fused) ((DecPlan PCO_GLOBAL*)plans + my_ti)->fused = my_fused_kind;
     __builtin_amdgcn_fence(__ATOMIC_RELEASE, "agent");
-    if (j == 0 && slot < kWQ) __hip_atomic_store((uint32_t*)my_progress, my_fused ? 1u : kTrailDead, __ATOMIC_RELAXED, __HIP_MEMORY_SCOPE_AGENT);
+    if (j == 0 && slot < kWQ) __hip_atomic_store((uint32_t*)my_progress(), my_fused ? 1u : kTrailDead, __ATOMIC_RELAXED, __HIP_MEMORY_SCOPE_AGENT);
   }
 
   typedef uint32_t u32x4 __attribute__((ext_vector_type(4)));
   QuadMasks qm = {j >= 1 ? ~0u : 0u, j >= 2 ? ~0u : 0u, j >= 3 ? ~0u : 0u, 63u};
   asm volatile("" : "+v"(qm.m1), "+v"(qm.m2), "+v"(qm.m3), "+v"(qm.c63));
   u32x4 d_acc[4] = {{0u, 0u, 0u, 0u}, {0u, 0u, 0u, 0u}, {0u, 0u, 0u, 0u}, {0u, 0u, 0u, 0u}};
-  uint32_t d_ngrp = 0, issued_batches = 0; uint8_t PCO_GLOBAL* d_sym_out = nullptr;
-  uint64_t d_off_val = 0; uint64_t* d_off_ptr = nullptr;
-  auto flush_deferred = [&]() {
-#pragma unroll
-    for (int g = 0; g < 4; g++) if ((uint32_t)g < d_ngrp) store_syms<true>(d_sym_out + 64 * g, d_acc[g]);
-    d_ngrp = 0;
-    if (d_off_ptr) __hip_atomic_store(d_off_ptr, d_off_val, __ATOMIC_RELAXED, __HIP_MEMORY_SCOPE_AGENT);
-    d_off_ptr = nullptr;
+  uint32_t d_what = 0, issued_batches = 0;
+  uint64_t PCO_LDS* d_off_slot = (uint64_t PCO_LDS*)(walk_lds<kWQ>() + WalkCfg<kWQ>::kWalkTmpOff) + lane;
+  uint64_t PCO_LDS* src_slot = (uint64_t PCO_LDS*)(walk_lds<kWQ>() + WalkCfg<kWQ>::kWalkTmpOff + 512) + 2 * (slot < kWQ ? slot : 0u);
+  static_assert(512 + 16 * kWQ <= 1312, "the table-build scratch holds the parked values");
+  auto flush_deferred = [&](uint64_t d_off_val) {
+    uint32_t ti = my_ti == 0xffffffffu ? 0u : my_ti, j16 = 16 * j;
+    asm volatile("" : "+v"(ti), "+v"(j16));
+    const uint64_t item = (uint64_t)ti * 3 + ((d_what >> 4) & 3u);
+    uint8_t PCO_GLOBAL* so = (uint8_t PCO_GLOBAL*)sym_area + item * sym_stride + (uint64_t)(d_what >> 6) * kBatchN + j16;
+#pragma unroll
+    for (int g = 0; g < 4; g++) if ((uint32_t)g < (d_what & 7u)) store_syms<true>(so + 64 * g, d_acc[g]);
+    if (d_what & 8u) __hip_atomic_store(offpos_area + item * offpos_stride + (d_what >> 6), d_off_val, __ATOMIC_RELAXED, __HIP_MEMORY_SCOPE_AGENT);
+    d_what = 0;
   };
   uint64_t touch_prev = my_bitpos >> 3; uint32_t touch_r0 = 0, touch_r1 = 0;
+  typedef u32x4 __attribute__((aligned(1))) u32x4_unaligned;
+  uint32_t prev_q = 0, pre_q = 0, pre_st = 3u << 8;
+  if constexpr (kPre) {
+    if (my_front_ok && j == 0) { src_slot[0] = (uint64_t)(uintptr_t)my_src; src_slot[1] = my_len; }
+    if (my_front_ok && j < 3) { vinfo[j].pre_stride = 0; vinfo[j].pre_span = 0; vinfo[j].pre_count = 0; }
+    wave_sync_lds();
+  }
   while (__any(my_active != 0)) {
-    uint32_t cnt = 0, nb = 0, asl = 0, off_ob = 0, off_nodes = 0;
+    uint32_t cnt = 0, nb = 0, asl = 0, off_ob = 0, off_nodes = 0, h_stride = 0, h_span = 0;
     bool walk = false;
+    uint64_t d_off_now = 0;
+    gcptr_u8 r_src = my_src; uint64_t r_len = my_len;
+    if constexpr (kPre) { r_src = (gcptr_u8)(uintptr_t)src_slot[0]; r_len = src_slot[1]; }
+    if constexpr (kTrail && kTrailDefer) d_off_now = *d_off_slot;
     if (my_active) {
       const VarInfo PCO_LDS* vi = vinfo + cur_v;
       nb = vi->n_bins; asl = vi->ans_size_log; off_ob = vi->off_ob; off_nodes = vi->off_nodes;
+      if constexpr (kPre) { h_stride = vi->pre_stride; h_span = vi->pre_span; }
       const uint32_t batch_n = n_rem < kBatchN ? n_rem : kBatchN;
       if (cur_v == 0) { const uint32_t lim = n_rem > nlps1 ? n_rem - nlps1 : 0; cnt = lim < batch_n ? lim : batch_n; }
       else {
@@ -504,25 +522,33 @@
       walk = cnt > 0 && nb > 1;
     }
     const uint64_t q0 = my_bitpos >> 6;
+    const uint32_t win_addr = lds0 + slice + kGrpWinOff, rel0 = (uint32_t)(my_bitpos & 63);
+    const uint32_t obs_addr = lds0 + slice + kGrpTblOff + off_ob, tbl_addr = lds0 + slice + kGrpTblOff + off_nodes;
+    uint8_t PCO_GLOBAL* sym_out = (uint8_t PCO_GLOBAL*)sym_area + ((uint64_t)(my_ti == 0xffffffffu ? 0u : my_ti) * 3 + cur_v) * sym_stride + (uint64_t)batch * kBatchN + 16 * j;
+    uint32_t dq = 0, hit_bits = 0xffffffffu;
+    u32x4 pq[kPreQ / 8];
+    if constexpr (kPre) {
+      const uint32_t d = (uint32_t)q0 - pre_q;
+      if (walk && (pre_st & 0x80u) == 0 && d < (pre_st & 63u)) { dq = d; hit_bits = 64u * (pre_st & 63u); }
+    }
     WalkRegs r;
     r.saddr = cur_v == 0 ? st0 : (cur_v == 1 ? st1 : st2);
-    const uint32_t win_addr = lds0 + slice + kGrpWinOff, rel0 = (uint32_t)(my_bitpos & 63);
-    r.bitaddr = 8u * win_addr + rel0; r.obsum = 0; r.symacc = 0; r.e = 0; r.d0 = r.d1 = r.d2 = 0;
-    if (walk) {
+    r.bitaddr = 8u * win_addr + 64u * dq + rel0; r.obsum = 0; r.symacc = 0; r.e = 0; r.d0 = r.d1 = r.d2 = 0;
+    if (walk && hit_bits == 0xffffffffu) {
       const uint32_t nq = ((((rel0 + cnt * asl + 63u) >> 6) + 3u) + 1u) & ~1u;
       uint64_t lo[7], hi[7];
-      if ((q0 + nq) * 8 <= my_len + 16) {
+      if ((q0 + nq) * 8 <= r_len + 16) {
 #pragma unroll
         for (int k = 0; k < 7; k++) {
           const uint32_t qi = 2 * j + 8 * k, qc = qi < nq ? qi : nq - 2;
-          lo[k] = load_u64_le(my_src + (q0 + qc) * 8); hi[k] = load_u64_le(my_src + (q0 + qc) * 8 + 8);
+          lo[k] = load_u64_le(r_src + (q0 + qc) * 8); hi[k] = load_u64_le(r_src + (q0 + qc) * 8 + 8);
         }
       } else {
 #pragma unroll
         for (int k = 0; k < 7; k++) {
           const uint32_t qi = 2 * j + 8 * k;
           lo[k] = 0; hi[k] = 0;
-          if (qi < nq) { lo[k] = load_u64_le_safe(my_src, (q0 + qi) * 8, my_len + 16); hi[k] = load_u64_le_safe(my_src, (q0 + qi + 1) * 8, my_len + 16); }
+          if (qi < nq) { lo[k] = load_u64_le_safe(r_src, (q0 + qi) * 8, r_len + 16); hi[k] = load_u64_le_safe(r_src, (q0 + qi + 1) * 8, r_len + 16); }
         }
       }
 #pragma unroll
@@ -531,26 +557,38 @@
     wave_sync_lds();
     if constexpr (kTrail) {
       __asm__ volatile("s_waitcnt vmcnt(0)" ::: "memory");
-      if (my_fused && j == 0 && status == PCO_GFX_OK) __hip_atomic_store((uint32_t*)my_progress, 1u + issued_batches, __ATOMIC_RELAXED, __HIP_MEMORY_SCOPE_AGENT);
-      if constexpr (kTrailDefer) { flush_deferred(); issued_batches = batch; }
+      if (my_fused && j == 0 && status == PCO_GFX_OK) __hip_atomic_store((uint32_t*)my_progress(), 1u + issued_batches, __ATOMIC_RELAXED, __HIP_MEMORY_SCOPE_AGENT);
+      if constexpr (kTrailDefer) { flush_deferred(d_off_now); issued_batches = batch; }
       else issued_batches = batch;
     }
+    if constexpr (kPre) {
+      if (walk) {
+        const uint32_t last_v = (pre_st >> 8) & 3u, since = (uint32_t)q0 - prev_q;
+        const uint32_t stride = last_v == cur_v ? since : h_stride;
+        if (j == 0 && last_v < 3) vinfo[last_v].pre_stride = since;
+        const uint32_t margin = h_span < kPreQ ? (kPreQ - h_span) >> 1 : 0u;
+        const uint64_t p0 = q0 + (stride > margin ? stride - margin : 0u);
+        const uint64_t lim = (r_len + 16) >> 3;
+        const uint32_t nq = p0 >= lim ? 0u : (lim - p0 < (uint64_t)kPreQ ? (uint32_t)(lim - p0) & ~1u : kPreQ);
+        pre_q = (uint32_t)p0; pre_st = (pre_st & ~63u) | nq;
+#pragma unroll
+        for (int k = 0; k < (int)(kPreQ / 8); k++) { const uint32_t qi = 2 * j + 8 * k; pq[k] = *(const u32x4_unaligned PCO_GLOBAL*)(r_src + (qi < nq ? (p0 + qi) * 8 : 0)); }
+      }
+    } else {
     ((uint32_t PCO_LDS*)(walk_lds<kWQ>() + WalkCfg<kWQ>::kWalkTmpOff))[lane] = touch_r0 ^ touch_r1;
     if (walk) {
       const uint64_t cur = q0 * 8, pred = cur + (cur - touch_prev);
       touch_prev = cur;
       const uint64_t line0 = (pred & ~(uint64_t)127) - (pred >= 128 ? 128u : 0u);
       const uint64_t a0 = line0 + 128u * j, a1 = a0 + 512u;
-      touch_r0 = load_u32_le(my_src + (a0 + 4 <= my_len ? a0 : 0));
-      touch_r1 = load_u32_le(my_src + (a1 + 4 <= my_len ? a1 : 0));
-    }
-    const uint32_t obs_addr = lds0 + slice + kGrpTblOff + off_ob, tbl_addr = lds0 + slice + kGrpTblOff + off_nodes;
-    uint8_t PCO_GLOBAL* sym_out = (uint8_t PCO_GLOBAL*)sym_area + ((uint64_t)(my_ti == 0xffffffffu ? 0u : my_ti) * 3 + cur_v) * sym_stride + (uint64_t)batch * kBatchN + 16 * j;
+      touch_r0 = load_u32_le(r_src + (a0 + 4 <= r_len ? a0 : 0));
+      touch_r1 = load_u32_le(r_src + (a1 + 4 <= r_len ? a1 : 0));
+    }
+    }
     if (walk) {
       r.e = *(const uint32_t PCO_LDS*)(uintptr_t)r.saddr;
       walk_window(r, 0u);
       constexpr bool defer = kTrail && kTrailDefer;
-      if constexpr (defer) d_sym_out = sym_out;
       if (__all(!walk || cnt == kBatchN)) {
 #pragma unroll
         for (uint32_t grp = 0; grp < 4; grp++) {
@@ -565,10 +603,10 @@
           }
           if constexpr (defer) d_acc[grp] = acc; else store_syms<kTrail>(sym_out + 64 * grp, acc);
         }
-        if constexpr (defer) d_ngrp = 4;
+        if constexpr (defer) d_what = 4u | (cur_v << 4) | (batch << 6);
       } else {
         const uint32_t steps = (cnt + 3) >> 2;
-        if constexpr (defer) d_ngrp = (steps + 15) >> 4;
+        if constexpr (defer) d_what = ((steps + 15) >> 4) | (cur_v << 4) | (batch << 6);
 #pragma unroll
         for (uint32_t grp = 0; grp < 4; grp++) {
           if (grp * 16 >= steps) break;
@@ -588,23 +626,40 @@
           if constexpr (defer) d_acc[grp] = acc; else store_syms<kTrail>(sym_out + 64 * grp, acc);
         }
       }
-      if (cur_v == 0) st0 = r.saddr; else if (cur_v == 1) st1 = r.saddr; else st2 = r.saddr;
-    }
-    if (my_active) {
+    }
+    bool ran_out = false;
+    if constexpr (kPre) {
+      ran_out = walk && r.bitaddr - 8u * win_addr > hit_bits;
+      if (walk) {
+        if (!ran_out) {
+#pragma unroll
+          for (int k = 0; k < (int)(kPreQ / 8); k++) *(u32x4 PCO_LDS*)(win + 2 * j + 8 * k) = pq[k];
+          if (j == 0) {
+            (void)__hip_atomic_fetch_add(&vinfo[hit_bits != 0xffffffffu ? 0 : 1].pre_count, 1u, __ATOMIC_RELAXED, __HIP_MEMORY_SCOPE_WAVEFRONT);
+            vinfo[cur_v].pre_span = (r.bitaddr - 8u * win_addr - 64u * dq + 63u) >> 6;
+          }
+          pre_st = (pre_st & ~(3u << 8)) | (cur_v << 8); prev_q = (uint32_t)q0;
+        } else { pre_st = (pre_st & ~63u) + 64u; if constexpr (kTrail && kTrailDefer) d_what = 0; }
+      }
+    }
+    if (walk && !ran_out) { if (cur_v == 0) st0 = r.saddr; else if (cur_v == 1) st1 = r.saddr; else st2 = r.saddr; }
+    if (my_active && !ran_out) {
       uint32_t obq = r.obsum;
       obq += (uint32_t)__builtin_amdgcn_update_dpp(0, (int)obq, 0xB1, 0xf, 0xf, false);
       obq += (uint32_t)__builtin_amdgcn_update_dpp(0, (int)obq, 0x4E, 0xf, 0xf, false);
-      const uint64_t ans_end = walk ? (q0 << 6) + (r.bitaddr - 8u * win_addr) : my_bitpos;
+      const uint64_t ans_end = walk ? ((q0 - dq) << 6) + (r.bitaddr - 8u * win_addr) : my_bitpos;
       uint64_t ob_total = 0;
       if (cnt > 0) ob_total = walk ? (uint64_t)obq : (nb == 1 ? (uint64_t)cnt * *(const uint8_t PCO_LDS*)(uintptr_t)obs_addr : 0ull);
       if (cnt > 0 && j == 0) {
         uint64_t* op = offpos_area + ((uint64_t)my_ti * 3 + cur_v) * offpos_stride + batch;
-        if constexpr (kTrail && kTrailDefer) { d_off_ptr = op; d_off_val = ans_end; }
+        if constexpr (kTrail && kTrailDefer) { d_what = (d_what & 7u) | 8u | (cur_v << 4) | (batch << 6); *d_off_slot = ans_end; }
         else if constexpr (kTrail) __hip_atomic_store(op, ans_end, __ATOMIC_RELAXED, __HIP_MEMORY_SCOPE_AGENT);
         else *op = ans_end;
       }
       my_bitpos = ans_end + ob_total;
-      if (my_bitpos > my_len * 8) { status = PCO_GFX_INSUFFICIENT_DATA; my_active = 0; }
+      uint64_t end_len = my_len;
+      if constexpr (kPre) end_len = src_slot[1];
+      if (my_bitpos > end_len * 8) { status = PCO_GFX_INSUFFICIENT_DATA; my_active = 0; }
       uint32_t nv = cur_v + 1;
       while (nv < 3 && !((present_mask >> nv) & 1u)) nv++;
       if (nv >= 3) {
@@ -618,10 +673,17 @@
     }
     wave_sync_lds();
   }
+  if constexpr (kPre) { if (my_front_ok) { my_src = (gcptr_u8)(uintptr_t)src_slot[0]; my_len = src_slot[1]; } }
+  if constexpr (kPre) {
+    uint32_t c = (my_front_ok && j < 2) ? vinfo[j].pre_count : 0u;
+#pragma unroll
+    for (int m = 4; m < 64; m <<= 1) c += (uint32_t)__shfl_xor((int)c, m);
+    if (stats != nullptr && lane < 2 && c != 0) atomicAdd(stats + lane, (unsigned long long)c);
+  }
   if constexpr (kTrail) {
-    flush_deferred();
+    flush_deferred(*d_off_slot);
     __asm__ volatile("s_waitcnt vmcnt(0)" ::: "memory");
-    if (my_fused && j == 0) __hip_atomic_store((uint32_t*)my_progress, status == PCO_GFX_OK ? 1u + batch : kTrailDead, __ATOMIC_RELAXED, __HIP_MEMORY_SCOPE_AGENT);
+    if (my_fused && j == 0) __hip_atomic_store((uint32_t*)my_progress(), status == PCO_GFX_OK ? 1u + batch : kTrailDead, __ATOMIC_RELAXED, __HIP_MEMORY_SCOPE_AGENT);
   }
   if (my_ti != 0xffffffffu && j == 0 && slot < kWQ) {
     DecPlan PCO_GLOBAL* plan = (DecPlan PCO_GLOBAL*)plans + my_ti;
@@ -663,15 +725,15 @@
 template <class L, uint32_t kWQ>
 __global__ __launch_bounds__(256) void dec_walk_kernel(const PcoGfxDecodeTask* tasks, const uint32_t* task_ids, uint32_t n_ids, DecPlan* plans,
                                                       uint8_t* bins_area, uint8_t* sym_area, uint64_t sym_stride, uint64_t* offpos_area, uint64_t offpos_stride,
-                                                      uint32_t accept_status, PcoGfxTaskResult* results, uint32_t* split, const MetaRef* metas) {
-  dec_walk_body<L, kWQ, false>(tasks, task_ids, n_ids, plans, bins_area, sym_area, sym_stride, offpos_area, offpos_stride, accept_status, results, split, metas);
+                                                      uint32_t accept_status, PcoGfxTaskResult* results, uint32_t* split, const MetaRef* metas, unsigned long long* stats) {
+  dec_walk_body<L, kWQ, false, false, true>(tasks, task_ids, n_ids, plans, bins_area, sym_area, sym_stride, offpos_area, offpos_stride, accept_status, results, split, metas, nullptr, stats);
 }
 #define PCO_TRAIL_WALK_ATTR __attribute__((amdgpu_waves_per_eu(4, 4)))
 template <class L>
 __global__ __launch_bounds__(256) PCO_TRAIL_WALK_ATTR void dec_walk_trail_kernel(const PcoGfxDecodeTask* tasks, const uint32_t* task_ids, uint32_t n_ids, DecPlan* plans,
                                                       uint8_t* bins_area, uint8_t* sym_area, uint64_t sym_stride, uint64_t* offpos_area, uint64_t offpos_stride,
-                                                      PcoGfxTaskResult* results, uint32_t* progress, const MetaRef* metas) {
-  dec_walk_body<L, 8, true>(tasks, task_ids, n_ids, plans, bins_area, sym_area, sym_stride, offpos_area, offpos_stride, 0u, results, progress, metas);
+                                                      PcoGfxTaskResult* results, uint32_t* progress, const MetaRef* metas, unsigned long long* stats) {
+  dec_walk_body<L, 8, true, false, true>(tasks, task_ids, n_ids, plans, bins_area, sym_area, sym_stride, offpos_area, offpos_stride, 0u, results, progress, metas, nullptr, stats);
 }
 
 __device__ __forceinline__ void store_u64_batch(unsigned long long PCO_GLOBAL* batch_base, const unsigned long long (&x)[4]) {
diff --git a/pcodec_amd/csrc/decode_kernel.hip b/pcodec_amd/csrc/decode_kernel.hip
--- a/pcodec_amd/csrc/decode_kernel.hip
+++ b/pcodec_amd/csrc/decode_kernel.hip
@@ -16,7 +16,7 @@
   uint32_t present, latent_bits, ans_size_log, n_bins, max_ob;
   uint32_t delta_kind, delta_order, window_n_log, state_n_log;
   uint32_t off_nodes, off_lower, off_ob, off_cum;
-  uint32_t pad[3];
+  uint32_t pre_stride, pre_span, pre_count;
 };
 static_assert(sizeof(VarInfo) == 64, "VarInfo");
 
diff --git a/pcodec_amd/csrc/pco_gfx.hip b/pcodec_amd/csrc/pco_gfx.hip
--- a/pcodec_amd/csrc/pco_gfx.hip
+++ b/pcodec_amd/csrc/pco_gfx.hip
@@ -187,6 +187,8 @@
     if (fast) {
       const uint32_t n_wb = (cnt + 7) / 8;
       uint32_t* d_progress = nullptr;
+      if (!ws.dec_stats.p) { ws.dec_stats.ensure(256); PCO_HIP_CHECK(hipMemsetAsync(ws.dec_stats.p, 0, 256, stream)); }
+      unsigned long long* d_wstats = (unsigned long long*)((uint8_t*)ws.dec_stats.p + kDecStatsWalkOff);
       uint32_t* d_givebacks = nullptr;
       constexpr uint32_t kTrailMinChunks = 1024;
       const bool use_trail = g_decode_trail && (cnt >= kTrailMinChunks || g_trail_debug != '\0' || g_trail_always);
@@ -194,7 +196,6 @@
         ensure_side_stream(ws);
         d_progress = (uint32_t*)ws.dec_progress.ensure((size_t)n_wb * kTrailProgressStride * sizeof(uint32_t));
         PCO_HIP_CHECK(hipMemsetAsync(d_progress, 0, (size_t)n_wb * kTrailProgressStride * sizeof(uint32_t), stream));
-        if (!ws.dec_stats.p) { ws.dec_stats.ensure(256); PCO_HIP_CHECK(hipMemsetAsync(ws.dec_stats.p, 0, 256, stream)); }
         d_givebacks = (uint32_t*)ws.dec_stats.p;
       }
       const uint32_t trail_grid = use_trail ? std::min<uint32_t>(n_wb, (uint32_t)ws.n_cus * 4u) : 0u;
@@ -215,11 +216,11 @@
         static const bool _quad_ok = hipFuncSetAttribute((const void*)dec_walk_trail_kernel<L>, hipFuncAttributeMaxDynamicSharedMemorySize, (int)(4 * WalkCfg<8>::kWalkLdsBytes)) == hipSuccess; \
         if (!_quad_ok) throw HostError{PCO_GFX_DEVICE_ERROR, "cannot reserve LDS for dec_walk_trail_kernel"};                                             \
         PCO_TIMED_LAUNCH("~dec_walk_kernel<" name ">", stream, (dec_walk_trail_kernel<L>), dim3((n_wb + 3) / 4), dim3(256), 4 * WalkCfg<8>::kWalkLdsBytes, stream, \
-                         d_tasks, idp, cnt, d_plans, d_bins, d_sym, sym_stride, d_offpos, offpos_stride, d_results, d_progress, d_metas);                 \
+                         d_tasks, idp, cnt, d_plans, d_bins, d_sym, sym_stride, d_offpos, offpos_stride, d_results, d_progress, d_metas, d_wstats);       \
                   \
         PCO_HIP_CHECK(hipStreamWaitEvent(ws.side_stream2, ws.fork_event, 0));                                                                             \
         PCO_TIMED_LAUNCH("~dec_walk_kernel(rest)<" name ">", ws.side_stream2, (dec_walk_kernel<L, 8>), dim3((n_wb + 3) / 4), dim3(256), 4 * WalkCfg<8>::kWalkLdsBytes, ws.side_stream2, \
-                         d_tasks, idp, cnt, d_plans, d_bins, d_sym, sym_stride, d_offpos, offpos_stride, 0u, d_results, d_progress, d_metas);             \
+                         d_tasks, idp, cnt, d_plans, d_bins, d_sym, sym_stride, d_offpos, offpos_stride, 0u, d_results, d_progress, d_metas, d_wstats);   \
         PCO_HIP_CHECK(hipEventRecord(ws.join_event2, ws.side_stream2));                                                                                   \
         hipStream_t ts = g_trail_debug == 's' ? stream : ws.side_stream;                                                                                  \
         PCO_HIP_CHECK(hipStreamWaitEvent(ws.side_stream, ws.fork_event, 0));                                                                              \
@@ -232,9 +233,9 @@
         PCO_HIP_CHECK(hipStreamWaitEvent(stream, ws.join_event, 0));                                                                                      \
         PCO_HIP_CHECK(hipStreamWaitEvent(stream, ws.join_event2, 0));                                                                                     \
       } else PCO_TIMED_LAUNCH("dec_walk_kernel<" name ">", stream, (dec_walk_kernel<L, 8>), dim3((n_wb + 3) / 4), dim3(256), 4 * WalkCfg<8>::kWalkLdsBytes, stream, \
-                       d_tasks, idp, cnt, d_plans, d_bins, d_sym, sym_stride, d_offpos, offpos_stride, 0u, d_results, (uint32_t*)nullptr, d_metas);       \
+                       d_tasks, idp, cnt, d_plans, d_bins, d_sym, sym_stride, d_offpos, offpos_stride, 0u, d_results, (uint32_t*)nullptr, d_metas, d_wstats); \
       PCO_TIMED_LAUNCH("dec_walk4_kernel<" name ">", stream, (dec_walk_kernel<L, 4>), dim3((cnt + 15) / 16), dim3(256), 4 * WalkCfg<4>::kWalkLdsBytes, stream, \
-                       d_tasks, idp, cnt, d_plans, d_bins, d_sym, sym_stride, d_offpos, offpos_stride, kStatusRetryK4, d_results, (uint32_t*)nullptr, d_metas); \
+                       d_tasks, idp, cnt, d_plans, d_bins, d_sym, sym_stride, d_offpos, offpos_stride, kStatusRetryK4, d_results, (uint32_t*)nullptr, d_metas, d_wstats); \
       PCO_TIMED_LAUNCH("dec_expand_kernel<" name ">", stream, (dec_expand_kernel<L, false>), dim3(grid), dim3(256), kExpLdsBytes, stream,               \
                        d_tasks, d_results, idp, cnt, d_plans, d_bins, d_sym, sym_stride, d_offpos, offpos_stride, (const uint32_t*)d_progress, d_givebacks);    \
       PCO_TIMED_LAUNCH("dec_expand_lb_kernel<" name ">", stream, (dec_expand_kernel<L, true>), dim3(grid), dim3(256), kExpLbLdsBytes, stream,           \
@@ -306,16 +307,18 @@
 static unsigned long long trail_stat(int which) {
   try {
     Workspace& w = workspace();
-    const unsigned long long acc = which == 0 ? w.acc_givebacks : w.acc_marked;
+    const unsigned long long acc = which == 0 ? w.acc_givebacks : (which == 1 ? w.acc_marked : (which == 2 ? w.acc_prestaged : w.acc_restaged));
     if (!w.dec_stats.p) return acc;
     if (w.has_last && w.last_event) (void)hipEventSynchronize(w.last_event);
-    uint32_t v[2] = {0, 0};
-    if (hipMemcpy(v, w.dec_stats.p, 8, hipMemcpyDeviceToHost) != hipSuccess) return acc;
-    return acc + v[which];
+    DecStatsHost v;
+    if (hipMemcpy(&v, w.dec_stats.p, sizeof(v), hipMemcpyDeviceToHost) != hipSuccess) return acc;
+    return acc + (which < 2 ? v.trail[which] : v.walk[which - 2]);
   } catch (...) { return 0; }
 }
 unsigned long long pco_gfx_trail_givebacks(void) { return trail_stat(0); }
 unsigned long long pco_gfx_trail_marked(void) { return trail_stat(1); }
+unsigned long long pco_gfx_walk_prestaged(void) { return trail_stat(2); }
+unsigned long long pco_gfx_walk_restaged(void) { return trail_stat(3); }
 unsigned long long pco_gfx_strict_histogram_fallbacks(void) {
   try {
     Workspace& w = workspace();
diff --git a/pcodec_amd/csrc/pco_host.h b/pcodec_amd/csrc/pco_host.h
--- a/pcodec_amd/csrc/pco_host.h
+++ b/pcodec_amd/csrc/pco_host.h
@@ -63,6 +63,9 @@
   void release() { if (p) (void)hipHostFree(p); p = nullptr; cap = 0; }
 };
 
+struct DecStatsHost { uint32_t trail[2] = {0, 0}; uint32_t unused[2] = {0, 0}; unsigned long long walk[2] = {0, 0}; };
+constexpr size_t kDecStatsWalkOff = 16;
+static_assert(offsetof(DecStatsHost, walk) == kDecStatsWalkOff, "DecStatsHost");
 struct Workspace {
   int device = -1;
   hipStream_t last_stream = nullptr; hipEvent_t last_event = nullptr; bool has_last = false;
@@ -101,10 +104,10 @@
 #undef PCO_WS_REP
     return r;
   }
-  unsigned long long acc_givebacks = 0, acc_marked = 0, acc_strict = 0;
+  unsigned long long acc_givebacks = 0, acc_marked = 0, acc_strict = 0, acc_prestaged = 0, acc_restaged = 0;
   void fold_counters() {
-    uint32_t v[2] = {0, 0};
-    if (dec_stats.p && hipMemcpy(v, dec_stats.p, 8, hipMemcpyDeviceToHost) == hipSuccess) { acc_givebacks += v[0]; acc_marked += v[1]; }
+    DecStatsHost v;
+    if (dec_stats.p && hipMemcpy(&v, dec_stats.p, sizeof(v), hipMemcpyDeviceToHost) == hipSuccess) { acc_givebacks += v.trail[0]; acc_marked += v.trail[1]; acc_prestaged += v.walk[0]; acc_restaged += v.walk[1]; }
     uint32_t f = 0;
     if (enc_strict.p && hipMemcpy(&f, enc_strict.p, 4, hipMemcpyDeviceToHost) == hipSuccess) acc_strict += f;
   }
```

New measurement: 1757 (median of 6 runs). 1.01x the previous value.
